# lunarlab-gatech/MorphSym-HGNN

Measured on AMD Instinct MI355X. Metric: graph-windows/sec fwd+bwd, A1-C2 GRF regression, higher is better.
Workload: dtype bf16; 1 GPU; A1-C2 GRF regression (3-D), h=128, L=3, T=150, 8192 windows/GPU, fwd+MSE+bwd, all parameter gradients; global_batch=8192, parallelism=dp1, rccl_ranks=0

## Files before the change

### morphsym_hgnn_amd/csrc/mshgnn.hip

```cpp
#include "mshgnn_slab.hpp"
extern "C" const char* mshgnn_last_error(void) { return g_err.c_str(); }
extern "C" const char* mshgnn_version(void) { return "mshgnn 0.5 (gfx950)"; }
extern "C" int mshgnn_abi_version(void) { return MSHGNN_ABI_VERSION; }
extern "C" size_t mshgnn_struct_size(int which) {
    switch (which) {
        case 0: return sizeof(mshgnn_desc);
        case 1: return sizeof(mshgnn_info);
        case 2: return sizeof(mshgnn_ws_layout);
        case 3: return sizeof(mshgnn_window_desc);
        case 4: return sizeof(mshgnn_kernel_stat);
        default: return 0;
    }
}


template <typename T> __device__ __forceinline__ void prep_one(const PrepArgs& a, int idx, bool with_bias) {
    constexpr int EPC = Prec<T>::EPC, NBV = Prec<T>::NBV;
    const int vec_per_pack = H * H / EPC;
    const int npk = a.pack_n < 0 ? a.n_packs : a.pack_n;
    const int total = npk * vec_per_pack;
    if (idx < total) {
        const int pack = a.pack0 + idx / vec_per_pack, r = idx % vec_per_pack;
        const int gid = pack * vec_per_pack + r;
        const int lane = r % 64, v = (r / 64) % NBV, wv = r / (64 * NBV);
        const PackDesc pd = a.packs[pack];
        T out[EPC];
        float g[8][EPC];
#pragma unroll
        for (int i = 0; i < 8; ++i)
#pragma unroll
            for (int x = 0; x < EPC; ++x) {
                int k, col;
                const int i16 = lane & 15;
                if constexpr (sizeof(T) == 4) { k = 32 * (lane >> 4) + 4 * (v & 7) + x; col = wv * 32 + 8 * (i16 >> 2) + 4 * (v >> 3) + (i16 & 3); }
                else { k = 32 * (lane >> 4) + 8 * (v & 3) + x; col = wv * 32 + 8 * (i16 >> 2) + 4 * (v >> 2) + (i16 & 3); }
                g[i][x] = 0.f;
                if (i < pd.n_src) {
                    if (pd.orient == 0) { if (k < pd.ncols) g[i][x] = a.params[pd.src[i] + (int64_t)col * pd.ld + pd.col0 + k]; }
                    else g[i][x] = a.params[pd.src[i] + (int64_t)k * pd.ld + col];
                }
            }
#pragma unroll
        for (int x = 0; x < EPC; ++x) {
            float sum = 0.f;
#pragma unroll
            for (int i = 0; i < 8; ++i) sum += g[i][x];
            out[x] = from_f32<T>(sum);
        }
        T* dst = reinterpret_cast<T*>(a.wpack) + (size_t)gid * EPC;
#pragma unroll
        for (int x = 0; x < EPC; ++x) dst[x] = out[x];
    } else if (with_bias) {
        const int b = idx - total;
        if (b < a.n_biases * H) {
            const BiasDesc bd = a.biases[b / H];
            float s = 0.f;
            for (int i = 0; i < bd.n_src; ++i) s += a.params[bd.src[i] + (b % H)];
            a.bias[b] = s;
        }
    }
}
template <typename T> __global__ void k_prep(PrepArgs a) { prep_one<T>(a, blockIdx.x * blockDim.x + threadIdx.x, true); }


__device__ __forceinline__ u32x4 splice8(u32x4 A, u32x4 B, int n0) {
    const unsigned __int128 a = ((unsigned __int128)(((unsigned long long)A[3] << 32) | A[2]) << 64) | (((unsigned long long)A[1] << 32) | A[0]);
    const unsigned __int128 b = ((unsigned __int128)(((unsigned long long)B[3] << 32) | B[2]) << 64) | (((unsigned long long)B[1] << 32) | B[0]);
    const int sh = 16 * n0;
    const unsigned __int128 r = (a & ((((unsigned __int128)1) << sh) - 1)) | (b << sh);
    return u32x4{(unsigned)r, (unsigned)(r >> 32), (unsigned)(r >> 64), (unsigned)(r >> 96)};
}
template <typename T, bool ALIGNED, bool SERIES = false, int SRC = 0, bool NORM = false> __global__ __launch_bounds__(256) void k_enc_fwd(EncArgs a, SeriesSrc ser, WideSrc wsrc) {
    using P = Prec<T>;
    static_assert(!NORM || SERIES, "standardisation is part of the series gather");
    static_assert(!SERIES || (sizeof(T) == 2 && ALIGNED), "the series gather is a bf16 path");
    static_assert(SRC == 0 || (sizeof(T) == 2 && ALIGNED && !SERIES), "wide source rows: bf16 plan, aligned destination rows");
    constexpr int MB = P::ENC_MB;
    constexpr int VPB = P::ROWS * P::CPR, NIT = VPB / 256 > 0 ? VPB / 256 : 1, BPP = 256 / VPB > 0 ? 256 / VPB : 1;
    extern __shared__ __attribute__((aligned(16))) char smem[];
    const int tid = threadIdx.x, lane = tid & 63, wv = __builtin_amdgcn_readfirstlane(tid >> 6);
    const int lab_blocks = SERIES ? (int)((ser.lab.B + 255) / 256) : 0;
    if constexpr (SERIES) {
        if ((int)blockIdx.x < lab_blocks) {
            const int64_t b = (int64_t)blockIdx.x * 256 + tid;
            if (b < ser.lab.B) window_labels_one(ser.lab, b);
            return;
        }
    }
    const int bid = (int)blockIdx.x - lab_blocks;
    if (bid >= a.wg_prefix[a.n_types]) {
        if constexpr (sizeof(T) == 2 && ALIGNED && !SERIES) prep_one<T>(a.prep, (bid - a.wg_prefix[a.n_types]) * 256 + tid, false);
        return;
    }
    int t = 0;
    while (t + 1 < a.n_types && bid >= a.wg_prefix[t + 1]) ++t;
    const int local = bid - a.wg_prefix[t];
    const int node = a.node_list[a.node_off[t] + (ENC_ORDER ? local % a.nodes[t] : local / a.tiles)], tile = ENC_ORDER ? local / a.nodes[t] : local % a.tiles;
    const bool skip = SERIES && ((a.skip_mask >> (a.tbase[t] + node)) & 1ull) != 0;
    const int w0 = tile * MB * P::ROWS;
    const T* x = reinterpret_cast<const T*>(a.x[t]);
    const int64_t pitch = a.pitch[t];
    const int F = a.width[t], nt = a.tbase[t + 1] - a.tbase[t], nkc = a.nkc[t], vb = a.vb[t];
    const uint8_t* sg = a.signs + a.sign_off[t] + (size_t)node * nkc * H;
    const T* wpack = reinterpret_cast<const T*>(a.wpack);
    const float* bias = a.bias + (size_t)max(a.bias_idx[t], 0) * H;

    typename P::Acc acc[MB];
#pragma unroll
    for (int m = 0; m < MB; ++m) acc_init_bias<T>(acc[m], bias, wv, lane);
    const int c = tid % P::CPR, r0 = (tid % VPB) / P::CPR, sub = tid / VPB;
    typename P::BFrag bf;
    typename P::AFrag af;
    const AOff<T> ao(lane);
    u32x4 v[MB / BPP][NIT];
    u32x4 rawv[(SERIES || SRC) ? MB / BPP : 1][NIT];
    u32x2 wv8[SRC ? MB / BPP : 1][SRC ? SRC : 1];
    const bool unit_ok = SRC == 8 || (F & 1) == 0;
    const int64_t spitch = SRC ? wsrc.pitch[t] : 0;
    int srow[SERIES ? MB / BPP : 1];
    u32x4 vn[NORM ? MB / BPP : 1][2];
    RunStats rsa[NORM ? MB / BPP : 1], rsb[NORM ? MB / BPP : 1];
    int n_n0 = 8; bool n_has_a = false, n_has_b = false;
    __shared__ unsigned long long rp_s[SERIES ? 16 : 1];
    int rfirst = 0, rend = 0;
    if constexpr (SERIES) {
#pragma unroll
        for (int mi = 0; mi < MB / BPP; ++mi) srow[mi] = (int)ser.starts[min(w0 + (mi * BPP + sub) * P::ROWS + r0, a.B - 1)];
        rfirst = ser.rows[2 * (ser.row0[t] + node)]; rend = ser.rows[2 * (ser.row0[t] + node) + 1];
        if (tid < 16) rp_s[tid] = rfirst + tid < rend ? ser.run_ptr[rfirst + tid] : 0ull;
        __syncthreads();
    }
    auto fetch = [&](int kc) {
        const int k0 = kc * H + c * P::EPC;
        const int nvalid = min(P::EPC, F - k0);
        if constexpr (SERIES) {
            const int j = k0 / ser.T, off = k0 - j * ser.T, n0 = min(P::EPC, ser.T - off);
            const bool second = nvalid > n0;
            auto run_ptr_of = [&](int jj) -> unsigned long long { return jj < 16 ? rp_s[jj] : (rfirst + jj < rend ? ser.run_ptr[rfirst + jj] : 0ull); };
            const unsigned long long pa = nvalid > 0 ? run_ptr_of(j) : 0ull, pb = second ? run_ptr_of(j + 1) : 0ull;
            if constexpr (NORM) {
                n_n0 = n0; n_has_a = pa != 0ull; n_has_b = pb != 0ull;
                const u32x4 ones32 = u32x4{0x3f800000u, 0x3f800000u, 0x3f800000u, 0x3f800000u};
#pragma unroll
                for (int mi = 0; mi < MB / BPP; ++mi) {
                    u32x4 a0 = nvalid > 0 ? ones32 : u32x4{0, 0, 0, 0}, a1 = a0;
                    const double* sp2 = ser.stats + ((size_t)min(w0 + (mi * BPP + sub) * P::ROWS + r0, a.B - 1) * ser.n_runs + rfirst + j) * 2;
                    rsa[mi] = RunStats{0.0, 1.0}; rsb[mi] = RunStats{0.0, 1.0};
                    if (pa) {
                        const float* sp = reinterpret_cast<const float*>(pa) + srow[mi] + off;
                        a0 = *reinterpret_cast<const u32x4*>(sp); a1 = *reinterpret_cast<const u32x4*>(sp + 4);
                        const f64x2 sv = *reinterpret_cast<const f64x2*>(sp2);
                        rsa[mi] = RunStats{sv[0], sv[1]};
                    }
                    if (second) {
                        u32x4 b0 = ones32, b1 = ones32;
                        if (pb) {
                            const float* sp = reinterpret_cast<const float*>(pb) + srow[mi];
                            b0 = *reinterpret_cast<const u32x4*>(sp); b1 = *reinterpret_cast<const u32x4*>(sp + 4);
                            const f64x2 sv = *reinterpret_cast<const f64x2*>(sp2 + 2);
                            rsb[mi] = RunStats{sv[0], sv[1]};
                        }
                        splice8f(a0, a1, b0, b1, n0);
                    }
                    vn[mi][0] = a0; vn[mi][1] = a1;
                }
                return;
            }
            const u32x4 ones = u32x4{0x3f803f80u, 0x3f803f80u, 0x3f803f80u, 0x3f803f80u};
#pragma unroll
            for (int mi = 0; mi < MB / BPP; ++mi) {
                u32x4 va = nvalid > 0 ? ones : u32x4{0, 0, 0, 0};
                if (pa) va = *reinterpret_cast<const u32x4*>(reinterpret_cast<const T*>(pa) + srow[mi] + off);
                if (second) {
                    u32x4 vb2 = ones;
                    if (pb) vb2 = *reinterpret_cast<const u32x4*>(reinterpret_cast<const T*>(pb) + srow[mi]);
                    va = splice8(va, vb2, n0);
                }
                v[mi][0] = va;
            }
            return;
        }
        if constexpr (SRC > 0) {
#pragma unroll
            for (int mi = 0; mi < MB / BPP; ++mi) {
                const int w = w0 + (mi * BPP + sub) * P::ROWS + r0;
                const char* row = reinterpret_cast<const char*>(wsrc.p[t]) + ((size_t)min(w, a.B - 1) * nt + node) * spitch * SRC;
                wide_fetch<SRC>(wv8[mi], row, k0, F, unit_ok, w < a.B);
            }
            return;
        }
#pragma unroll
        for (int mi = 0; mi < MB / BPP; ++mi)
#pragma unroll
            for (int it = 0; it < NIT; ++it) {
                const int m = mi * BPP + sub, row = r0 + it * (256 / P::CPR), w = w0 + m * P::ROWS + row;
                if constexpr (ALIGNED) {
                    const T* src = x + ((size_t)min(w, a.B - 1) * nt + node) * pitch + (nvalid > 0 ? k0 : kc * H);
                    v[mi][it] = ld16<ENC_NT>(src);
                } else {
                    v[mi][it] = u32x4{0, 0, 0, 0};
                    if (w < a.B) v[mi][it] = load_chunk<T>(x + ((size_t)w * nt + node) * pitch + k0, nvalid, vb);
                }
            }
    };
    fetch(0);
    for (int kc = 0; kc < nkc; ++kc) {
        const u32x4 sx = sign_xor<T>(sg + kc * H + c * P::EPC);
        const int nv = F - (kc * H + c * P::EPC);
        __syncthreads();
#pragma unroll
        for (int mi = 0; mi < MB / BPP; ++mi)
#pragma unroll
            for (int it = 0; it < NIT; ++it) {
                u32x4 raw;
                if constexpr (SRC > 0) {
// ... 951 lines not shown
            qstride[i] = H; qvalid[i] = 8; qvb[i] = 16;
        } else {
            const int t = im[3] - BUF_IN;
            qbase[i] = reinterpret_cast<const T*>(a.x[t]) + (size_t)im[5] * a.pitch[t] + im[6] + c * 8;
            qstride[i] = (int64_t)a.nodes[t] * a.pitch[t]; qvalid[i] = im[7] - c * 8; qvb[i] = a.vb[t];
            qsign[i] = sign_xor<T>(a.signs + im[8] + c * 8);
        }
    }
    f32x16 acc[2][2];
#pragma unroll
    for (int i = 0; i < 2; ++i)
#pragma unroll
        for (int j = 0; j < 2; ++j)
#pragma unroll
            for (int q = 0; q < 16; ++q) acc[i][j][q] = 0.f;
    float bsum[8];
#pragma unroll
    for (int e = 0; e < 8; ++e) bsum[e] = 0.f;

    struct Stage { u32x4 pv[4], qv[4]; unsigned mw[4]; };
    auto fetch = [&](Stage& st, int s) {
        const int w0 = (ch0 + (nit == 2 ? s >> 1 : s)) * GWB_KW;
        const int it = (nit == 2) ? (s & 1) : 0;
        const T* pb = it ? pbase[I1] : pbase[0];
        const T* qb = it ? qbase[I1] : qbase[0];
        const uint8_t* mb = it ? mbase[I1] : mbase[0];
        const int64_t qs = it ? qstride[I1] : qstride[0];
        const int qn = it ? qvalid[I1] : qvalid[0], vb = it ? qvb[I1] : qvb[0];
#pragma unroll
        for (int p = 0; p < 4; ++p) {
            const int w = w0 + r0 + 16 * p;
            st.pv[p] = u32x4{0, 0, 0, 0}; st.qv[p] = u32x4{0, 0, 0, 0}; st.mw[p] = 0xffffffffu;
            if (w < a.B && !ABL(a.dbg & 1)) {
                st.pv[p] = *reinterpret_cast<const u32x4*>(pb + (size_t)w * H);
                if (mb) st.mw[p] = mb[((size_t)(w >> 4) << 6) + (w & 15)];
                if (a.aligned) { if (qn > 0) st.qv[p] = *reinterpret_cast<const u32x4*>(qb + (size_t)w * qs); }
                else st.qv[p] = load_chunk<T>(qb + (size_t)w * qs, qn, vb);
            }
        }
    };
    const bool p_masked = mbase[0] != nullptr, q_raw_input = qvb[0] != 16 || qvalid[0] != 8 || (qsign[0][0] | qsign[0][1] | qsign[0][2] | qsign[0][3] | qsign[nit == 2 ? I1 : 0][0] | qsign[nit == 2 ? I1 : 0][1] | qsign[nit == 2 ? I1 : 0][2] | qsign[nit == 2 ? I1 : 0][3]) != 0 || qvalid[nit == 2 ? I1 : 0] != 8;
    auto stage_to_lds = [&](const Stage& st, const u32x4 sx, const int qn, __bf16* Ps, __bf16* Qs) {
        if ABL(a.dbg & 2) { asm volatile("" :: "v"(st.pv[0][0]), "v"(st.qv[3][3])); return; }
#pragma unroll
        for (int p = 0; p < 4; ++p) {
            const int row = r0 + 16 * p;
            u32x4 pm = st.pv[p];
            if (p_masked) pm &= mlut[st.mw[p] & 0xffu];
            *reinterpret_cast<u32x4*>(&Ps[gwb_elem(row, c * 8)]) = pm;
            u32x4 qm = st.qv[p];
            if (q_raw_input) qm = chunk_keep_first<T>(qm, qn) ^ sx;
            *reinterpret_cast<u32x4*>(&Qs[gwb_elem(row, c * 8)]) = qm;
            if (bias_flag) {
#pragma unroll
                for (int e = 0; e < 4; ++e) {
                    bsum[2 * e] += __builtin_bit_cast(float, pm[e] << 16);
                    bsum[2 * e + 1] += __builtin_bit_cast(float, pm[e] & 0xffff0000u);
                }
            }
        }
    };
    auto mfmas = [&](const __bf16* Ps, const __bf16* Qs) {
        if ABL(a.dbg & 4) return;
#pragma unroll
        for (int ks = 0; ks < GWB_KW / 16; ++ks) {
            bf16x8 af[2], bq[2];
#pragma unroll
            for (int i = 0; i < 2; ++i) {
                af[i] = tr_frag(Ps, ks * 16, wr * 64 + i * 32, lane);
                bq[i] = tr_frag(Qs, ks * 16, wc * 64 + i * 32, lane);
            }
#pragma unroll
            for (int i = 0; i < 2; ++i)
#pragma unroll
                for (int j = 0; j < 2; ++j) acc[i][j] = __builtin_amdgcn_mfma_f32_32x32x16_bf16(af[i], bq[j], acc[i][j], 0, 0, 0);
        }
    };
    const u32x4 sx1 = nit == 2 ? qsign[I1] : qsign[0];
    const int qn1 = nit == 2 ? qvalid[I1] : qvalid[0];
#if GW_DEEP
    Stage sa, sb;
    if (nsteps > 0) fetch(sa, 0);
    if (nsteps > 1) fetch(sb, 1);
    if (nsteps > 0) stage_to_lds(sa, qsign[0], qvalid[0], Pbuf[0], Qbuf[0]);
    if (nsteps > 2) fetch(sa, 2);
    __syncthreads();
    for (int s = 0; s < nsteps; s += 2) {
        if (s + 1 < nsteps) stage_to_lds(sb, sx1, qn1, Pbuf[1], Qbuf[1]);
        if (s + 3 < nsteps) fetch(sb, s + 3);
        mfmas(Pbuf[0], Qbuf[0]);
        __syncthreads();
        if (s + 1 < nsteps) {
            if (s + 2 < nsteps) stage_to_lds(sa, qsign[0], qvalid[0], Pbuf[0], Qbuf[0]);
            if (s + 4 < nsteps) fetch(sa, s + 4);
            mfmas(Pbuf[1], Qbuf[1]);
            __syncthreads();
        }
    }
#else
    Stage sa;
    if (nsteps > 0) fetch(sa, 0);
#ifndef MSHGNN_GW_STAMPS
#define MSHGNN_GW_STAMPS 0
#endif
#if MSHGNN_GW_STAMPS
    long long tph[5] = {0, 0, 0, 0, 0}, tprev = a.stamps ? clock64() : 0;
    auto lap = [&](int k) { if (a.stamps) { const long long t = clock64(); tph[k] += t - tprev; tprev = t; } };
#else
    auto lap = [](int) {};
#endif
    for (int s = 0; s < nsteps; ++s) {
        __syncthreads();
        lap(0);
        stage_to_lds(sa, (nit == 2 && (s & 1)) ? qsign[I1] : qsign[0], (nit == 2 && (s & 1)) ? qvalid[I1] : qvalid[0], Pbuf[0], Qbuf[0]);
        lap(1);
        __syncthreads();
        lap(2);
        if (s + 1 < nsteps) fetch(sa, s + 1);
        lap(3);
        mfmas(Pbuf[0], Qbuf[0]);
        lap(4);
    }
#if MSHGNN_GW_STAMPS
    if (a.stamps && tid == 0) { for (int k = 0; k < 5; ++k) a.stamps[(size_t)blockIdx.x * 8 + k] = tph[k]; a.stamps[(size_t)blockIdx.x * 8 + 5] = nsteps; }
#endif
    (void)sx1; (void)qn1;
#endif
    float* slab = a.slabs + (size_t)(part * a.n_lanes + ln) * SLAB_FLOATS;
    if (!ABL(a.dbg & 8))
#pragma unroll
    for (int i = 0; i < 2; ++i)
#pragma unroll
        for (int j = 0; j < 2; ++j)
#pragma unroll
            for (int q = 0; q < 16; ++q) {
                const int o = wr * 64 + i * 32 + (q & 3) + ((q >> 2) << 3) + ((lane >> 5) << 2), k = wc * 64 + j * 32 + (lane & 31);
                slab[o * H + k] = acc[i][j][q];
            }
    if (bias_flag) {
        float* red = reinterpret_cast<float*>(Pbuf[0]);
        __syncthreads();
#pragma unroll
        for (int e = 0; e < 8; ++e) red[r0 * H + c * 8 + e] = bsum[e];
        __syncthreads();
        if (tid < H) {
            float s2 = 0.f;
#pragma unroll
            for (int r = 0; r < 16; ++r) s2 += red[r * H + tid];
            slab[H * H + tid] = s2;
        }
    }
}

template <bool ALIGNED, bool SERIES = false> __global__ __launch_bounds__(256, GW_WPS) void k_gradw_bf16_lean(GradwArgs a) {
    static_assert(!SERIES || ALIGNED, "the series gather replaces the aligned raw loads");
    using T = __bf16;
    __shared__ __attribute__((aligned(16))) __bf16 Ps[GWB_KW * GWB_PITCH];
    __shared__ __attribute__((aligned(16))) __bf16 Qs[GWB_KW * GWB_PITCH];
    __shared__ __attribute__((aligned(16))) u32x4 mlut[256];
    __shared__ __attribute__((aligned(16))) u32x4 qkeep_t[16];
    __shared__ __attribute__((aligned(16))) u32x4 qsign_t[GW_IPL][16];
    __shared__ unsigned long long sbase[GW_IPL][4];
    __shared__ unsigned long long sser[SERIES ? GW_IPL : 1][16][2];
    const int tid = threadIdx.x, lane = tid & 63, wv = __builtin_amdgcn_readfirstlane(tid >> 6);
    mlut[tid] = chunk_mask_bits<__bf16>(u32x4{0xffffffffu, 0xffffffffu, 0xffffffffu, 0xffffffffu}, (unsigned)tid);
    const int wr = wv >> 1, wc = wv & 1;
    const int ln = a.lane_order[blockIdx.x % a.n_pad], part = blockIdx.x / a.n_pad;
    if (ln < 0) return;
    const int* lh = a.lanes + ln * LANE_INTS;
    const int it0 = lh[0], nit = lh[1] - lh[0], bias_flag = lh[3];
    const int* im0 = a.items + it0 * ITEM_INTS;
    const int nchunks = (a.B + GWB_KW - 1) / GWB_KW;
    const int ch0 = (int)((int64_t)part * nchunks / a.n_parts), ch1 = (int)((int64_t)(part + 1) * nchunks / a.n_parts);
    const int nsteps = ch1 - ch0, total = nsteps * nit;
    const int c = tid & 15, r4 = (tid >> 4) * 4;

    const bool p_masked = im0[9] >= 0, q_raw = im0[4] < 0;
    const int ntile = (a.B + 15) >> 4;
    const unsigned voffP = (unsigned)(r4 * H + c * 8) * (unsigned)sizeof(T);
    const unsigned voffM = (unsigned)(((c >> 2) * ntile + (r4 >> 4)) * 64 + (c & 3) * 16 + (r4 & 15));
    const int qt = q_raw ? im0[3] - BUF_IN : 0;
    const unsigned qsb = q_raw ? (unsigned)(a.nodes[qt] * a.pitch[qt]) * (unsigned)sizeof(T) : (unsigned)(H * sizeof(T));
    const int qn = q_raw ? im0[7] - c * 8 : 8, qvb = q_raw ? a.vb[qt] : 16;
    const unsigned voffQ0 = (unsigned)r4 * qsb + (unsigned)c * 16u;
    unsigned ldsw[4];
#pragma unroll
    for (int p = 0; p < 4; ++p) ldsw[p] = (unsigned)gwb_elem(r4 + p, c * 8);
    if (tid < 16) qkeep_t[tid] = chunk_keep_first<T>(u32x4{0xffffffffu, 0xffffffffu, 0xffffffffu, 0xffffffffu}, qn);
    if (tid < nit) {
        const int* im = a.items + (it0 + tid) * ITEM_INTS;
        sbase[tid][0] = (unsigned long long)(a.ws + a.buf_off[im[0]] + (act_idx(0, im[2], a.B) + (size_t)ch0 * GWB_KW * H) * sizeof(T));
        sbase[tid][1] = p_masked ? (unsigned long long)(a.ws + a.buf_off[im[9]] + relu_byte(im[2], a.B, 0, 0) + (size_t)ch0 * (GWB_KW / 16) * 64) : 0ull;
        sbase[tid][2] = q_raw ? (unsigned long long)(reinterpret_cast<const char*>(a.x[qt]) + ((size_t)im[5] * a.pitch[qt] + im[6]) * sizeof(T) + (size_t)ch0 * GWB_KW * qsb)
                              : (unsigned long long)(a.ws + a.buf_off[im[3]] + (act_idx(0, im[5], a.B) + (size_t)ch0 * GWB_KW * H) * sizeof(T));
    }
    if (q_raw && tid < nit * 16) {
        const int* im = a.items + (it0 + (tid >> 4)) * ITEM_INTS;
        qsign_t[tid >> 4][c] = sign_xor<T>(a.signs + im[8] + c * 8);
        if constexpr (SERIES) {
            const int k0 = im[6] + c * 8, j = k0 / a.ser.T, off = k0 - j * a.ser.T, n0 = min(8, a.ser.T - off);
            const int rfirst = a.ser.rows[2 * (a.ser.row0[qt] + im[5])];
            const unsigned long long pa = qn > 0 ? a.ser.run_ptr[rfirst + j] : 0ull, pb = min(qn, 8) > n0 ? a.ser.run_ptr[rfirst + j + 1] : 0ull;
            sser[tid >> 4][c][0] = pa ? pa + (unsigned long long)off * sizeof(T) : 0ull;
            sser[tid >> 4][c][1] = pb;
        }
    }
    int s_n0 = 8; bool s_two = false;
    if constexpr (SERIES) { if (q_raw) { const int k0 = im0[6] + c * 8, off = k0 % a.ser.T; s_n0 = min(8, a.ser.T - off); s_two = min(qn, 8) > s_n0; } }
    __syncthreads();
    const char* pS = a.ws; const char* mS = a.ws; const char* qS = a.ws;
    auto ubase = [&](int k, int j, size_t off) -> const char* {
        const unsigned long long v = sbase[k][j] + off;
        return reinterpret_cast<const char*>(((unsigned long long)(unsigned)__builtin_amdgcn_readfirstlane((int)(v >> 32)) << 32) |
                                             (unsigned)__builtin_amdgcn_readfirstlane((int)(unsigned)v));
    };
    f32x16 acc[2][2];
#pragma unroll
    for (int i = 0; i < 2; ++i)
#pragma unroll
        for (int j = 0; j < 2; ++j)
#pragma unroll
            for (int q = 0; q < 16; ++q) acc[i][j][q] = 0.f;
    float bsum[8];
#pragma unroll
    for (int e = 0; e < 8; ++e) bsum[e] = 0.f;

    u32x4 pv[4], qv[4]; unsigned mw = 0xffffffffu;
    int nk = 0, nc = 0;
    int wst[SERIES ? 4 : 1];
    auto load_starts = [&](int chunk) {
        if constexpr (SERIES) {
            if (q_raw) {
#pragma unroll
                for (int p = 0; p < 4; ++p) wst[p] = (int)a.ser.starts[min((ch0 + chunk) * GWB_KW + r4 + p, a.B - 1)];
            }
        }
    };
    auto load_q = [&](int p) -> u32x4 {
        if constexpr (SERIES) {
            if (q_raw) {
                const u32x4 ones = u32x4{0x3f803f80u, 0x3f803f80u, 0x3f803f80u, 0x3f803f80u};
                const unsigned long long pa = sser[nk][c][0];
                u32x4 va = ones;
                if (pa) va = *reinterpret_cast<const u32x4*>(reinterpret_cast<const T*>(pa) + wst[p]);
                if (s_two) {
                    const unsigned long long pb = sser[nk][c][1];
                    u32x4 vb2 = ones;
                    if (pb) vb2 = *reinterpret_cast<const u32x4*>(reinterpret_cast<const T*>(pb) + wst[p]);
                    va = splice8(va, vb2, s_n0);
                }
                return va;
            }
        }
        if constexpr (ALIGNED) return *reinterpret_cast<const u32x4*>(qS + voffQ0 + p * qsb);
        else return q_raw ? load_chunk<T>(reinterpret_cast<const T*>(qS + voffQ0 + p * qsb), qn, qvb) : *reinterpret_cast<const u32x4*>(qS + voffQ0 + p * qsb);
    };
    auto fetch = [&]() {
        pS = ubase(nk, 0, (size_t)nc * GWB_KW * H * sizeof(T));
        if (p_masked) mS = ubase(nk, 1, (size_t)nc * (GWB_KW / 16) * 64);
        qS = ubase(nk, 2, (size_t)nc * GWB_KW * qsb);
        const int w0 = (ch0 + nc) * GWB_KW;
        if (w0 + GWB_KW <= a.B) {
#pragma unroll
            for (int p = 0; p < 4; ++p) {
                pv[p] = *reinterpret_cast<const u32x4*>(pS + voffP + p * (int)(H * sizeof(T)));
                qv[p] = u32x4{0, 0, 0, 0};
                if (qn > 0) qv[p] = load_q(p);
            }
            if (p_masked) mw = *reinterpret_cast<const unsigned*>(mS + voffM);
        } else {
#pragma unroll
            for (int p = 0; p < 4; ++p) {
                pv[p] = u32x4{0, 0, 0, 0}; qv[p] = u32x4{0, 0, 0, 0};
                if (w0 + r4 + p < a.B) {
                    pv[p] = *reinterpret_cast<const u32x4*>(pS + voffP + p * (int)(H * sizeof(T)));
                    if (qn > 0) qv[p] = load_q(p);
                }
            }
            mw = 0xffffffffu;
            if (p_masked && w0 + r4 < a.B) mw = *reinterpret_cast<const unsigned*>(mS + voffM);
        }
        if (++nk == nit) { nk = 0; ++nc; if (nc < nsteps) load_starts(nc); }
    };
    int sk = 0;
    auto stage_to_lds = [&]() {
        u32x4 mk[4], qkeep, sx;
        if (q_raw) { qkeep = qkeep_t[c]; sx = qsign_t[sk][c]; }
        if (++sk == nit) sk = 0;
        if (p_masked) {
#pragma unroll
            for (int p = 0; p < 4; ++p) mk[p] = mlut[(mw >> (8 * p)) & 0xffu];
        }
#pragma unroll
        for (int p = 0; p < 4; ++p) {
            u32x4 pm = pv[p];
            if (p_masked) pm &= mk[p];
            *reinterpret_cast<u32x4*>(&Ps[ldsw[p]]) = pm;
            u32x4 qm = qv[p];
            if (q_raw) qm = (qm & qkeep) ^ sx;
            *reinterpret_cast<u32x4*>(&Qs[ldsw[p]]) = qm;
            if (bias_flag) {
#pragma unroll
                for (int e = 0; e < 4; ++e) {
                    bsum[2 * e] += __builtin_bit_cast(float, pm[e] << 16);
                    bsum[2 * e + 1] += __builtin_bit_cast(float, pm[e] & 0xffff0000u);
                }
            }
        }
    };
    if (total > 0) { load_starts(0); fetch(); }
    for (int s = 0; s < total; ++s) {
        __syncthreads();
        stage_to_lds();
        __syncthreads();
        if (s + 1 < total) fetch();
#pragma unroll
        for (int ks = 0; ks < GWB_KW / 16; ++ks) {
            bf16x8 af[2], bq[2];
#pragma unroll
            for (int i = 0; i < 2; ++i) {
                af[i] = tr_frag(Ps, ks * 16, wr * 64 + i * 32, lane);
                bq[i] = tr_frag(Qs, ks * 16, wc * 64 + i * 32, lane);
            }
#pragma unroll
            for (int i = 0; i < 2; ++i)
#pragma unroll
                for (int j = 0; j < 2; ++j) acc[i][j] = __builtin_amdgcn_mfma_f32_32x32x16_bf16(af[i], bq[j], acc[i][j], 0, 0, 0);
        }
    }
    float* slab = a.slabs + (size_t)(part * a.n_lanes + ln) * SLAB_FLOATS;
#pragma unroll
    for (int i = 0; i < 2; ++i)
#pragma unroll
        for (int j = 0; j < 2; ++j)
#pragma unroll
            for (int q = 0; q < 16; ++q) {
                const int o = wr * 64 + i * 32 + (q & 3) + ((q >> 2) << 3) + ((lane >> 5) << 2), k = wc * 64 + j * 32 + (lane & 31);
                slab[o * H + k] = acc[i][j][q];
            }
    if (bias_flag) {
        float* red = reinterpret_cast<float*>(Ps);
        __syncthreads();
#pragma unroll
        for (int e = 0; e < 8; ++e) red[(r4 >> 2) * H + c * 8 + e] = bsum[e];
        __syncthreads();
        if (tid < H) {
            float s2 = 0.f;
#pragma unroll
            for (int r = 0; r < 16; ++r) s2 += red[r * H + tid];
            slab[H * H + tid] = s2;
        }
    }
}


#ifndef FIN_LB
#define FIN_LB 4
#endif
__global__ __launch_bounds__(256) void k_finalize(FinArgs a) {
    const int* f = a.fin + blockIdx.x * FIN_INTS;
    const int64_t dst = (int64_t)(unsigned)f[0] | ((int64_t)f[1] << 32);
    const int rows = f[2], cols = f[3], ld = f[4], tg = f[5], kind = f[6];
    const int* more = f[7] ? a.fin0 + f[7] : nullptr;
    const int RPB = (rows + gridDim.y - 1) / gridDim.y;
    const int r0 = blockIdx.y * RPB, r1 = min(rows, r0 + RPB);
    const int n = (r1 - r0) * cols;
    if (a.loss && blockIdx.x == 0 && blockIdx.y == 0 && threadIdx.x < 64) {
        float l = 0.f;
        for (int b = threadIdx.x; b < a.n_dec; b += 64) l += a.dec_slabs[(size_t)b * DEC_SLAB_FLOATS + 8 * H + 8];
#pragma unroll
        for (int m = 32; m >= 1; m >>= 1) l += __shfl_xor(l, m, 64);
        if (threadIdx.x == 0) *a.loss = l * a.inv_n + (a.accumulate ? *a.loss : 0.f);
    }
    if (!a.grad) return;
    const bool is_mat = (kind == FIN_MATRIX || kind == FIN_DEC_W);
    if (kind == FIN_DEC_W || kind == FIN_DEC_B) {
        const int lane = threadIdx.x & 63, wave = blockIdx.y * 4 + (threadIdx.x >> 6), nwaves = gridDim.y * 4;
        for (int e = wave; e < rows * cols; e += nwaves) {
            const int r = e / cols, cidx = e % cols;
            const int src = is_mat ? r * H + cidx : 8 * H + cidx;
            float sum = 0.f;
            for (int b0 = 0; b0 < a.n_dec; b0 += 512) {
                float v[8];
#pragma unroll
                for (int u = 0; u < 8; ++u) { const int b = b0 + lane + 64 * u; v[u] = b < a.n_dec ? a.dec_slabs[(size_t)b * DEC_SLAB_FLOATS + src] : 0.f; }
                sum += ((v[0] + v[1]) + (v[2] + v[3])) + ((v[4] + v[5]) + (v[6] + v[7]));
            }
#pragma unroll
            for (int m = 32; m >= 1; m >>= 1) sum += __shfl_xor(sum, m, 64);
            if (lane == 0) { float* gp = a.grad + dst + (int64_t)r * ld + cidx; *gp = a.accumulate ? *gp + sum : sum; }
        }
        return;
    }
    if (n <= 0) return;
    for (int i = threadIdx.x; i < n; i += 256) {
        const int r = r0 + i / cols, cidx = i % cols;
        float s = 0.f;
        if (kind == FIN_MATRIX || kind == FIN_BIAS) {
            const int src = is_mat ? r * H + cidx : H * H + cidx;
            const int l0 = a.targets[tg * TGT_INTS], nl = a.targets[tg * TGT_INTS + 1] - l0;
            const float* sp = a.slabs + (size_t)l0 * SLAB_FLOATS + src;
            const size_t pstride = (size_t)a.n_lanes * SLAB_FLOATS;
            for (int j0 = 0; j0 < nl; j0 += FIN_LB)
                for (int p0 = 0; p0 < a.n_parts; p0 += 4) {
                    float v[FIN_LB][4];
#pragma unroll
                    for (int jj = 0; jj < FIN_LB; ++jj)
#pragma unroll
                        for (int pp = 0; pp < 4; ++pp)
                            v[jj][pp] = (j0 + jj < nl && p0 + pp < a.n_parts) ? sp[(size_t)(j0 + jj) * SLAB_FLOATS + (size_t)(p0 + pp) * pstride] : 0.f;
#pragma unroll
                    for (int jj = 0; jj < FIN_LB; ++jj) s += (v[jj][0] + v[jj][1]) + (v[jj][2] + v[jj][3]);
                }
        }
        if (a.accumulate) s += a.grad[dst + (int64_t)r * ld + cidx];
        a.grad[dst + (int64_t)r * ld + cidx] = s;
        if (more) {
            const int nm = more[0];
            for (int k = 0; k < nm; ++k) a.grad[((int64_t)(unsigned)more[1 + 2 * k] | ((int64_t)more[2 + 2 * k] << 32)) + (int64_t)r * ld + cidx] = s;
        }
    }
}

static StackKernel slab_fwd_kernel(const HostPlan& hp) {
    if (hp.sl_hb <= SL_HB) return hp.n_mlp <= 2 ? k_slab_fwd<__bf16, 2, SL_HB> : k_slab_fwd<__bf16, 4, SL_HB>;
    return hp.n_mlp <= 2 ? k_slab_fwd<__bf16, 2, SL_HB_MAX> : k_slab_fwd<__bf16, 4, SL_HB_MAX>;
}
using SpecSelector = StackKernel (*)(const HostPlan& hp, int kind, int tr, int nt, int full, const char** name);
static StackKernel spec_kernel(const HostPlan& hp, int kind, int tr, int nt, int full, const char** name = nullptr) {
    const char* nm = nullptr;
    if (hp.jit_prog) {
        StackKernel kk = reinterpret_cast<SpecSelector>(hp.jit_prog)(hp, kind, tr, nt, full, &nm);
        if (nm) { if (name) *name = nm; return kk; }
    }
#define SPEC_SHARD_TRY(k) { StackKernel kk = spec_shard##k(hp, kind, tr, nt, full, &nm); if (nm) { if (name) *name = nm; return kk; } }
    SPEC_SHARD_LIST(SPEC_SHARD_TRY)
#undef SPEC_SHARD_TRY
    return nullptr;
}
inline bool whole_tiles(int64_t B) { return B > 0 && B % TILE_ROWS == 0; }
static StackKernel slab_step_spec_kernel(const HostPlan& hp, int nt, const char** name = nullptr, bool full = true) { return spec_kernel(hp, 0, 1, nt, full, name); }
static StackKernel slab_fwd_spec_kernel(const HostPlan& hp, int training, int nt, bool full = true) { return spec_kernel(hp, 1, training, nt, full); }
static StackKernel slab_bwd_spec_kernel(const HostPlan& hp, int nt, bool full = true) { return spec_kernel(hp, 2, 1, nt, full); }
static StackKernel slab_step_kernel(const HostPlan& hp, int64_t B = -1, int nt = 0, bool use_spec = false) {
    if (use_spec && B > 0) if (StackKernel k = slab_step_spec_kernel(hp, nt, nullptr, whole_tiles(B))) return k;
    if (hp.sl_hb <= SL_HB) return hp.n_mlp <= 2 ? k_slab_step<__bf16, 2, SL_HB> : k_slab_step<__bf16, 4, SL_HB>;
    return hp.n_mlp <= 2 ? k_slab_step<__bf16, 2, SL_HB_MAX> : k_slab_step<__bf16, 4, SL_HB_MAX>;
}
static StackKernel slab_bwd_kernel(const HostPlan& hp) {
    if (hp.sl_hb <= SL_HB) return hp.n_mlp <= 2 ? k_slab_bwd<__bf16, 2, SL_HB> : k_slab_bwd<__bf16, 4, SL_HB>;
    return hp.n_mlp <= 2 ? k_slab_bwd<__bf16, 2, SL_HB_MAX> : k_slab_bwd<__bf16, 4, SL_HB_MAX>;
}


static int set_spec_attrs(mshgnn_plan* p, int flds) {
    const HostPlan& hp = p->hp;
    int rc;
    const char* nm = nullptr;
    for (int nt = 0; nt < 2; ++nt)
        if (StackKernel k = slab_step_spec_kernel(hp, nt, &nm)) if ((rc = set_lds_attr(k, flds))) return rc;
    if (!nm) { p->use_spec = false; return MSHGNN_OK; }
    p->spec_name_buf = strncmp(nm, "spec::", 6) == 0 ? nm + 6 : nm;
    p->spec_name = p->spec_name_buf.c_str();
    for (int v = 0; v < 3; ++v)
        if (StackKernel k = slab_fwd_spec_kernel(hp, v > 0, v - 1)) if ((rc = set_lds_attr(k, flds))) return rc;
    for (int nt = 0; nt < 2; ++nt)
        if (StackKernel k = slab_bwd_spec_kernel(hp, nt)) if ((rc = set_lds_attr(k, flds))) return rc;
    if (StackKernel k = slab_step_spec_kernel(hp, 0, nullptr, false)) if ((rc = set_lds_attr(k, flds))) return rc;
    if (StackKernel k = slab_fwd_spec_kernel(hp, 0, 0, false)) if ((rc = set_lds_attr(k, flds))) return rc;
    return MSHGNN_OK;
}

extern "C" int mshgnn_plan_attach_program(mshgnn_plan* p, void* selector) {
    if (!p || !selector) return set_err(MSHGNN_EINVAL, "plan or selector is null");
    if (!p->gen && p->hp.d.dtype == MSHGNN_BF16X3) return x3_attach_program(p, selector);
    if (p->gen || p->hp.d.dtype != MSHGNN_BF16 || !p->use_fused || !p->use_slab) return set_err(MSHGNN_EINVAL, "attached programs exist for LDS-resident bf16 / split-bf16 plans (bf16: on the slab kernels) only");
    void* const prev = p->hp.jit_prog;
    p->hp.jit_prog = selector;
    const char* nm = nullptr;
    if (!reinterpret_cast<SpecSelector>(selector)(p->hp, 0, 1, 0, 1, &nm) || !nm) {
        p->hp.jit_prog = prev;
        return set_err(MSHGNN_EINVAL, "the program's tables are not this plan's");
    }
    p->use_spec = true;
    const int rc = set_spec_attrs(p, (p->hp.fs_blk + FS_EXTRA_BLK) * Prec<__bf16>::BLK);
    if (rc || !p->use_spec) { p->hp.jit_prog = prev; p->use_spec = false; return rc ? rc : set_err(MSHGNN_EINVAL, "no kernel of the attached program could be used"); }
    return MSHGNN_OK;
}

extern "C" int mshgnn_plan_create(const mshgnn_desc* desc, mshgnn_plan** out) {
    if (!out) return set_err(MSHGNN_EINVAL, "plan_out is null");
    *out = nullptr;
    mshgnn_plan* p = new (std::nothrow) mshgnn_plan();
    if (!p) return set_err(MSHGNN_ENOMEM, "out of host memory");
    if (!desc) { delete p; return set_err(MSHGNN_EINVAL, "null descriptor"); }
    p->n_types = desc->n_types;
    if (const char* e = getenv("MSHGNN_STEP_CHUNK")) p->step_chunk = std::max<int64_t>(0, atoll(e));
    if (const char* e = getenv("MSHGNN_STASH_NT")) p->stash_nt_force = atoi(e);
    const char* eng_env = getenv("MSHGNN_ENGINE");
    bool want_gen = eng_env && std::string(eng_env) == "generic";
    std::string why;
    if (!want_gen && !compile_plan(desc, p->hp)) {
        why = p->hp.err;
        const bool unsup = why.find("supports") != std::string::npos || why.find("not supported") != std::string::npos || why.find("too many") != std::string::npos;
        if (!unsup) { delete p; return set_err(MSHGNN_EINVAL, why); }
        want_gen = true;
    }
    if (want_gen) {
        int ndev0 = 0;
        if (hipGetDeviceCount(&ndev0) != hipSuccess || ndev0 == 0) { delete p; return set_err(MSHGNN_EHIP, "no HIP device: the MS-HGNN engine has no CPU fallback"); }
        const int rc = gen_create(p, desc);
        if (rc) {
            const std::string m = g_err; gen_destroy(p); delete p;
            return set_err(rc, why.empty() ? m : why + "; generic-width engine: " + m);
        }
#ifdef MSHGNN_ABLATE
        { const char* e = getenv("MSHGNN_DBG"); p->dbg = e ? atoi(e) : 0; }
#endif
        if (!p->hp.d.n_types) {
            p->hp.d = *desc;
        }
        *out = p;
        return MSHGNN_OK;
    }
    int ndev = 0;
    if (hipGetDeviceCount(&ndev) != hipSuccess || ndev == 0) {
        delete p; return set_err(MSHGNN_EHIP, "no HIP device: the MS-HGNN engine has no CPU fallback");
    }
#ifdef MSHGNN_ABLATE
    { const char* e = getenv("MSHGNN_DBG"); p->dbg = e ? atoi(e) : 0; e = getenv("MSHGNN_DBG_GW"); p->dbg_gw = e ? atoi(e) : 0; }
#endif
    HostPlan& hp = p->hp;
    auto up = [&](void** dptr, const void* src, size_t bytes) -> int {
        HIPCHK(hipMalloc(dptr, std::max<size_t>(bytes, 16)));
        if (bytes) HIPCHK(hipMemcpy(*dptr, src, bytes, hipMemcpyHostToDevice));
        return MSHGNN_OK;
    };
    int rc;
    if ((rc = up((void**)&p->d_tables, hp.tables.data(), hp.tables.size() * 4)) != 0 ||
        (rc = up((void**)&p->d_signs, hp.signs.data(), hp.signs.size())) != 0 ||
        (rc = up((void**)&p->d_out_mask, hp.out_mask_f.data(), hp.out_mask_f.size() * 4)) != 0 ||
        (rc = up((void**)&p->d_packs, hp.packs.data(), hp.packs.size() * sizeof(PackDesc))) != 0 ||
        (rc = up((void**)&p->d_biases, hp.biases.data(), hp.biases.size() * sizeof(BiasDesc))) != 0) {
        mshgnn_plan_destroy(p); return rc;
    }
    const int lds = hp.n_blk * hp.blk_bytes;
    if (hp.d.dtype == MSHGNN_BF16X3) {
        p->use_fused = true;
        { const char* et = getenv("MSHGNN_STEP_KERNEL"); p->use_step = !(et && atoi(et) == 0); }
        if ((rc = x3_set_attrs(p))) { mshgnn_plan_destroy(p); return rc; }
    } else if (hp.d.dtype == MSHGNN_F32) {
        if ((rc = set_lds_attr(k_layer_fwd<float>, lds)) || (rc = set_lds_attr(k_layer_bwd<float>, lds)) ||
            (rc = set_lds_attr(k_enc_fwd<float, true>, Prec<float>::ENC_MB * Prec<float>::BLK)) || (rc = set_lds_attr(k_enc_fwd<float, false>, Prec<float>::ENC_MB * Prec<float>::BLK))) { mshgnn_plan_destroy(p); return rc; }
    } else {
        if ((rc = set_lds_attr(k_layer_fwd<__bf16>, lds)) || (rc = set_lds_attr(k_layer_bwd<__bf16>, lds)) ||
            (rc = set_lds_attr(k_enc_fwd<__bf16, true>, Prec<__bf16>::ENC_MB * Prec<__bf16>::BLK)) || (rc = set_lds_attr(k_enc_fwd<__bf16, true, true>, Prec<__bf16>::ENC_MB * Prec<__bf16>::BLK)) || (rc = set_lds_attr(k_enc_fwd<__bf16, true, false, 8>, Prec<__bf16>::ENC_MB * Prec<__bf16>::BLK)) || (rc = set_lds_attr(k_enc_fwd<__bf16, true, false, 4>, Prec<__bf16>::ENC_MB * Prec<__bf16>::BLK)) || (rc = set_lds_attr(k_enc_fwd<__bf16, false>, Prec<__bf16>::ENC_MB * Prec<__bf16>::BLK))) { mshgnn_plan_destroy(p); return rc; }
        const char* e = getenv("MSHGNN_FUSED");
        p->use_fused = hp.fused && !(e && atoi(e) == 0);
        if (p->use_fused) {
            const int flds = (hp.fs_blk + FS_EXTRA_BLK) * Prec<__bf16>::BLK;
            if ((rc = set_lds_attr(k_stack_fwd<__bf16>, flds)) || (rc = set_lds_attr(k_stack_bwd<__bf16>, flds)) || (rc = set_lds_attr(k_stack_step<__bf16>, flds))) { mshgnn_plan_destroy(p); return rc; }
            const char* es = getenv("MSHGNN_SLAB");
            p->use_slab = hp.slab && !(es && atoi(es) == 0);
            p->slab_force = es && atoi(es) == 2;
            { int dev = 0, cus = 256; if (hipGetDevice(&dev) == hipSuccess) (void)hipDeviceGetAttribute(&cus, hipDeviceAttributeMultiprocessorCount, dev); p->n_cu = cus > 0 ? cus : 256; }
            if (p->use_slab && ((rc = set_lds_attr(slab_fwd_kernel(hp), flds)) || (rc = set_lds_attr(slab_bwd_kernel(hp), flds)) ||
                                (rc = set_lds_attr(slab_step_kernel(hp), flds)))) { mshgnn_plan_destroy(p); return rc; }
            { const char* esp = getenv("MSHGNN_SPEC"); p->use_spec = p->use_slab && !(esp && atoi(esp) == 0); }
            if (p->use_spec && (rc = set_spec_attrs(p, flds))) { mshgnn_plan_destroy(p); return rc; }
            { const char* et = getenv("MSHGNN_STEP_KERNEL"); p->use_step = !(et && atoi(et) == 0); }

            { const char* eg = TUNE_ENV("MSHGNN_STAGGER"); p->stagger = eg ? atoi(eg) : 0; }
        }
    }
    *out = p;
    return MSHGNN_OK;
}

extern "C" void mshgnn_plan_destroy(mshgnn_plan* p) {
    if (!p) return;
    gen_destroy(p);
    if (p->d_tables) (void)hipFree(p->d_tables);
    if (p->d_signs) (void)hipFree(p->d_signs);
    if (p->d_out_mask) (void)hipFree(p->d_out_mask);
    if (p->d_packs) (void)hipFree(p->d_packs);
    if (p->d_biases) (void)hipFree(p->d_biases);
    if (p->d_ig_nodes) (void)hipFree(p->d_ig_nodes);
    for (ProfRec& r : p->recs) { (void)hipEventDestroy(r.a); (void)hipEventDestroy(r.b); }
    for (hipEvent_t e : p->free_events) (void)hipEventDestroy(e);
    delete p;
}

extern "C" int mshgnn_profile_enable(mshgnn_plan* p, int on) {
    if (!p) return set_err(MSHGNN_EINVAL, "null plan");
    p->prof = on != 0;
    return MSHGNN_OK;
}

extern "C" int mshgnn_profile_read(mshgnn_plan* p, mshgnn_kernel_stat* stats, int32_t* n_inout) {
    if (!p || !stats || !n_inout) return set_err(MSHGNN_EINVAL, "null argument");
    std::vector<mshgnn_kernel_stat> ks = p->gen ? *gen_kstats(p) : p->hp.kstats;
    for (const ProfRec& r : p->recs) {
        HIPCHK(hipEventSynchronize(r.b));
        float ms = 0.f;
        HIPCHK(hipEventElapsedTime(&ms, r.a, r.b));
        if (r.slot >= 0 && r.slot < (int)ks.size()) { ks[r.slot].total_ms += ms; ks[r.slot].launches += 1; }
        p->free_events.push_back(r.a); p->free_events.push_back(r.b);
    }
    p->recs.clear();
    const int n = std::min<int>(*n_inout, (int)ks.size());
    for (int i = 0; i < n; ++i) stats[i] = ks[i];
    *n_inout = n;
    return MSHGNN_OK;
}

extern "C" const char* mshgnn_plan_specialised(const mshgnn_plan* p) { return p && !p->gen && p->use_spec ? p->spec_name : ""; }
extern "C" int mshgnn_plan_info(const mshgnn_plan* p, mshgnn_info* info) {
    if (!p || !info) return set_err(MSHGNN_EINVAL, "null argument");
    *info = p->gen ? *gen_info(p) : p->hp.info;
    return MSHGNN_OK;
}

extern "C" int mshgnn_plan_compile_host(const mshgnn_desc* desc, mshgnn_info* info, int32_t* n_tables_out) {
    HostPlan hp;
    const char* eng_env = getenv("MSHGNN_ENGINE");
    if ((eng_env && std::string(eng_env) == "generic") || !compile_plan(desc, hp)) {
        const std::string why = hp.err;
        if (gen_host_compile(desc, info, n_tables_out) == MSHGNN_OK) return MSHGNN_OK;
        return set_err(MSHGNN_EINVAL, why.empty() ? g_err : why + "; generic-width engine: " + g_err);
    }
    if (info) *info = hp.info;
    if (n_tables_out) *n_tables_out = (int32_t)hp.tables.size();
    return MSHGNN_OK;
}

extern "C" int mshgnn_workspace_layout(const mshgnn_plan* p, int64_t batch, int training, mshgnn_ws_layout* out) {
    if (!p || !out || batch < 1) return set_err(MSHGNN_EINVAL, "bad argument to mshgnn_workspace_layout");
    if (p->gen) gen_layout(p, batch, training, out); else layout_workspace(p->hp, batch, training, out);
    return MSHGNN_OK;
}

int launch_prep(const PrepArgs& a, bool split, hipStream_t st) {
    if (split) return x3_launch_prep(a, st);
    const int64_t total = (int64_t)a.n_packs * (H * H / Prec<__bf16>::EPC) + (int64_t)a.n_biases * H;
    if (prep_use_tiled(a.n_packs)) hipLaunchKernelGGL((k_prep_tiled<__bf16, false>), dim3(prep_tiled_grid(a.n_packs, a.n_biases)), dim3(256), 0, st, a);
    else hipLaunchKernelGGL(k_prep<__bf16>, dim3((unsigned)((total + 255) / 256)), dim3(256), 0, st, a);
    return MSHGNN_OK;
}

int run_finalize(const mshgnn_plan* p, const StepCall& c, const mshgnn_ws_layout& lay, int gw_parts) {
    const HostPlan& hp = p->hp;
    const mshgnn_desc& d = hp.d;
    char* ws = c.ws; float* gparams = c.grad_params; hipStream_t st = c.stream;
    const int B = (int)c.batch, gw_phase = c.gw_phase;
    float* loss = c.loss != LossKind::NONE ? c.loss_out : nullptr;
    FinArgs a{p->d_tables + hp.fin_off, p->d_tables + hp.fin_off, p->d_tables + hp.tgt_off, reinterpret_cast<const float*>(ws + lay.slabs),
              reinterpret_cast<const float*>(ws + lay.dec_slabs), gparams, hp.n_lanes, gw_parts, loss,
              1.0f / (float)(c.total_windows() * d.type_nodes[d.out_type] * (c.loss == LossKind::CE ? 1 : d.out_channels)),
              c.dec_done ? (int)((B + TILE_ROWS - 1) / TILE_ROWS) : NWG_DEC, c.accumulates()};
    int f0 = 0, nf = hp.n_fin;
    if (gw_phase == 0) nf = hp.n_fin_ph0;
    if (gw_phase == 1) { f0 = hp.n_fin_ph0; nf = hp.n_fin - hp.n_fin_ph0; a.loss = nullptr; }
    a.fin += (size_t)f0 * FIN_INTS;
    if (!gparams) {
        if (loss) hipLaunchKernelGGL(k_finalize, dim3(1, 1), dim3(256), 0, st, a);
        HIPCHK(hipGetLastError());
        return MSHGNN_OK;
    }
    ProfScope ps(p, hp.ks_fin, st);
    if (nf > 0) hipLaunchKernelGGL(k_finalize, dim3(nf, 64), dim3(256), 0, st, a);
    HIPCHK(hipGetLastError());
    return MSHGNN_OK;
}

template <typename T>
static int forward_impl(const mshgnn_plan* p, StepCall& c) {
    const HostPlan& hp = p->hp;
    const mshgnn_desc& d = hp.d;
    const int training = c.training;
    mshgnn_ws_layout lay; layout_workspace(hp, c.batch, training, &lay);
    const int B = (int)c.batch;
    const void* const* x = c.x; const int64_t* x_pitch = c.x_pitch;
    const float* params = c.params; char* ws = c.ws; hipStream_t st = c.stream;
    const SeriesSrc* series = c.series; const WideSrc* wide = c.wide;
    const float* y_fused = c.y_fused(); const int32_t* labels_fused = c.labels_fused();
    PrepArgs pa{params, ws + lay.wpack, reinterpret_cast<float*>(ws + lay.bias), p->d_packs, p->d_biases, (int)hp.packs.size(), (int)hp.biases.size()};
    int enc_pack0 = (int)hp.packs.size();
    for (int t = 0; t < hp.NT; ++t) if (hp.pack_enc_base[t] >= 0) enc_pack0 = std::min(enc_pack0, hp.pack_enc_base[t]);
    static const bool embed_off = TUNE_ENV("MSHGNN_PREP_EMBED") && atoi(TUNE_ENV("MSHGNN_PREP_EMBED")) == 0;
    const bool embed = sizeof(T) == 2 && !series && !prep_use_tiled(pa.n_packs) && enc_pack0 > 0 && !embed_off;
    {
        PrepArgs a = pa;
        if (embed) { a.pack0 = enc_pack0; a.pack_n = pa.n_packs - enc_pack0; }
        const int64_t total = (int64_t)(embed ? a.pack_n : a.n_packs) * (H * H / Prec<T>::EPC) + (int64_t)hp.biases.size() * H;
        ProfScope ps(p, hp.ks_prep, st);
        if (prep_use_tiled(a.n_packs)) hipLaunchKernelGGL((k_prep_tiled<T, false>), dim3(prep_tiled_grid(a.n_packs, a.n_biases)), dim3(256), 0, st, a);
        else hipLaunchKernelGGL(k_prep<T>, dim3((unsigned)((total + 255) / 256)), dim3(256), 0, st, a);
    }
    {
        EncArgs a{};
        a.n_types = hp.NT; a.B = B; a.NN = hp.NN; a.tiles = (B + Prec<T>::ENC_MB * Prec<T>::ROWS - 1) / (Prec<T>::ENC_MB * Prec<T>::ROWS);
        a.wg_prefix[0] = 0;
        for (int t = 0; t < hp.NT; ++t) {
            a.x[t] = x ? x[t] : nullptr; a.pitch[t] = x_pitch ? x_pitch[t] : d.type_width[t];
            if (a.pitch[t] < d.type_width[t]) return set_err(MSHGNN_EINVAL, "x_pitch smaller than the feature width");
            a.vb[t] = vec_bytes(a.x[t], a.pitch[t], (int)sizeof(T));
            if (t == 0) a.aligned = 1;
            if (a.vb[t] != 16 || a.pitch[t] % Prec<T>::EPC) a.aligned = 0;
            a.width[t] = d.type_width[t]; a.tbase[t] = hp.type_base[t]; a.nkc[t] = hp.enc_nkc[t];
            a.pack0[t] = hp.pack_enc_base[t]; a.bias_idx[t] = hp.bias_enc[t]; a.sign_off[t] = hp.sign_off[t];
            a.node_off[t] = t == 0 ? 0 : a.node_off[t - 1] + a.nodes[t - 1];
            a.nodes[t] = 0;
            const bool all_rows = series != nullptr && x != nullptr;
            for (int i = 0; i < d.type_nodes[t]; ++i) {
                const bool need = hp.need_n[0][hp.type_base[t] + i];
                if (need || all_rows) a.node_list[a.node_off[t] + a.nodes[t]++] = (unsigned char)i;
                if (!need) a.skip_mask |= 1ull << (hp.type_base[t] + i);
            }
            a.wg_prefix[t + 1] = a.wg_prefix[t] + a.nodes[t] * a.tiles;
        }
        a.tbase[hp.NT] = hp.NN;
        a.wpack = ws + lay.wpack; a.bias = reinterpret_cast<const float*>(ws + lay.bias); a.signs = p->d_signs; a.x0 = ws + lay.x[0];
        a.mask0 = (training && lay.dd[0]) ? reinterpret_cast<uint8_t*>(ws + lay.dd[0]) : nullptr;
        unsigned enc_grid = (unsigned)a.wg_prefix[hp.NT];
        if (embed) {
            PrepArgs lp = pa; lp.pack0 = 0; lp.pack_n = enc_pack0;
            if (a.aligned) { a.prep = lp; a.prep_vecs = enc_pack0 * (H * H / Prec<T>::EPC); enc_grid += (unsigned)((a.prep_vecs + 255) / 256); }
            else {
                ProfScope ps(p, hp.ks_prep, st);
                hipLaunchKernelGGL(k_prep<T>, dim3((unsigned)(((int64_t)enc_pack0 * (H * H / Prec<T>::EPC) + 255) / 256)), dim3(256), 0, st, lp);
            }
        }
        ProfScope ps(p, hp.ks_enc, st);
        if constexpr (sizeof(T) == 2) {
            if (series) {
                if (x && !a.aligned) return set_err(MSHGNN_EINVAL, "the fused window assembly needs 16-byte aligned window rows (pitch a multiple of 8)");
                enc_grid += (unsigned)((series->lab.B + 255) / 256);
                if (series->stats) hipLaunchKernelGGL((k_enc_fwd<T, true, true, 0, true>), dim3(enc_grid), dim3(256), Prec<T>::ENC_MB * Prec<T>::BLK, st, a, *series, WideSrc{});
                else hipLaunchKernelGGL((k_enc_fwd<T, true, true>), dim3(enc_grid), dim3(256), Prec<T>::ENC_MB * Prec<T>::BLK, st, a, *series, WideSrc{});
            } else if (wide) {
                if (x && !a.aligned) return set_err(MSHGNN_EINVAL, "wide source rows: the plan-dtype rows need 16-byte alignment and a pitch that is a multiple of 8");
                if (wide->bytes == 8) hipLaunchKernelGGL((k_enc_fwd<T, true, false, 8>), dim3(enc_grid), dim3(256), Prec<T>::ENC_MB * Prec<T>::BLK, st, a, SeriesSrc{}, *wide);
                else hipLaunchKernelGGL((k_enc_fwd<T, true, false, 4>), dim3(enc_grid), dim3(256), Prec<T>::ENC_MB * Prec<T>::BLK, st, a, SeriesSrc{}, *wide);
            } else if (a.aligned) hipLaunchKernelGGL((k_enc_fwd<T, true>), dim3(enc_grid), dim3(256), Prec<T>::ENC_MB * Prec<T>::BLK, st, a, SeriesSrc{}, WideSrc{});
            else hipLaunchKernelGGL((k_enc_fwd<T, false>), dim3(enc_grid), dim3(256), Prec<T>::ENC_MB * Prec<T>::BLK, st, a, SeriesSrc{}, WideSrc{});
        } else {
            if (wide) return set_err(MSHGNN_EUNSUPPORTED, "wide source rows: not on the fp32 plan (cast the inputs)");
            if (a.aligned) hipLaunchKernelGGL((k_enc_fwd<T, true>), dim3(enc_grid), dim3(256), Prec<T>::ENC_MB * Prec<T>::BLK, st, a, SeriesSrc{}, WideSrc{});
            else hipLaunchKernelGGL((k_enc_fwd<T, false>), dim3(enc_grid), dim3(256), Prec<T>::ENC_MB * Prec<T>::BLK, st, a, SeriesSrc{}, WideSrc{});
        }
    }
    const int tiles = (B + Prec<T>::ROWS - 1) / Prec<T>::ROWS;
    if constexpr (sizeof(T) == 2) {
        if (p->use_fused) {
            StackArgs a{};
            a.tile_in = ws + lay.x[0]; a.ws = ws;
            for (int l = 0; l <= hp.L; ++l) a.x_off[l] = lay.x[l];
            for (int l = 0; l < hp.L; ++l) { a.mask_off[l] = lay.mask[l]; a.hb_off[l] = lay.hb[l]; a.t1_off[l] = lay.t1[l]; a.prog_off[l] = hp.fs_fwd_off[l]; }
            a.wpack = ws + lay.wpack; a.bias = reinterpret_cast<const float*>(ws + lay.bias); a.tables = p->d_tables;
            a.B = B; a.NN = hp.NN; a.L = hp.L; a.training = training;
            a.dbg = p->dbg;
            a.params = params; a.out_mask = p->d_out_mask; a.out = c.out; a.off_dec_w = d.off_dec_w; a.off_dec_b = d.off_dec_b;
            a.node0 = hp.type_base[d.out_type]; a.n_out = d.type_nodes[d.out_type]; a.dout = d.out_channels;
            if (y_fused) {
                a.y = y_fused; a.dec_slabs = reinterpret_cast<float*>(ws + lay.dec_slabs); a.dx_off[hp.L] = lay.dx[hp.L];
                a.inv_n = 1.0f / (float)(c.total_windows() * a.n_out * a.dout);
            } else if (labels_fused) {
                a.labels = labels_fused; a.dec_slabs = reinterpret_cast<float*>(ws + lay.dec_slabs); a.dx_off[hp.L] = lay.dx[hp.L];
                a.inv_n = 1.0f / (float)(c.total_windows() * a.n_out);
            }
            c.dec_done = y_fused || labels_fused;
            a.stamps = stamp_ptr("MSHGNN_STAMPS");
            a.stagger = p->slab_for(tiles) && tiles > p->n_cu ? p->stagger : 0;
            a.stash_nt = training ? stash_nt_for(p->stash_nt_force, B, stash_rows_of(hp), H * (int)sizeof(T)) : 0;
            const bool want_step = p->use_step && c.dec_done;
            bool step_slab = p->slab_for(tiles);
            const bool spec_small = !step_slab && want_step && p->use_slab && p->use_spec && slab_step_spec_kernel(hp, a.stash_nt, nullptr, whole_tiles(B)) != nullptr;
            bool red_front_ok = false, red_back_ok = false; size_t red_back = 0;
            auto red_fits = [&](bool slab) {
                const size_t red_need = (size_t)((slab ? SL_THREADS : LAYER_THREADS) / 64) * DEC_SLAB_FLOATS * sizeof(float);
                const size_t lds_launch = (size_t)((slab ? hp.sl_blk : hp.fs_blk) + FS_EXTRA_BLK) * Prec<T>::BLK;
                red_back = (size_t)(a.node0 + a.n_out) * Prec<T>::BLK;
                red_front_ok = (size_t)a.node0 * Prec<T>::BLK >= red_need; red_back_ok = red_back + red_need <= lds_launch;
                return red_front_ok || red_back_ok; };
            if (spec_small && red_fits(true)) step_slab = true;
            const bool step = want_step && red_fits(step_slab);
            if (step && !red_front_ok) a.red_off = (int)red_back;
            const StackKernel fwd_spec = (!step && p->use_slab && p->use_spec) ? slab_fwd_spec_kernel(hp, training, a.stash_nt, whole_tiles(B)) : nullptr;
            if (fwd_spec) step_slab = true;
            ProfScope ps(p, step ? hp.ks_stack_step : hp.ks_stack_fwd, st);
            if (step_slab) {
                for (int l = 0; l < hp.L; ++l) a.prog_off[l] = hp.sl_fwd_off[l];
                if (step) {
                    for (int l = 0; l <= hp.L; ++l) a.dx_off[l] = lay.dx[l];
                    for (int l = 0; l < hp.L; ++l) { a.dh_off[l] = lay.dh[l]; a.du_off[l] = lay.du[l]; a.prog_off_b[l] = hp.sl_bwd_off[l]; }
                    a.mask0_off = lay.dd[0];
                    hipLaunchKernelGGL(slab_step_kernel(hp, B, a.stash_nt, p->use_spec), dim3(tiles), dim3(SL_THREADS), (hp.sl_blk + FS_EXTRA_BLK) * Prec<T>::BLK, st, a);
                    c.stack_done = true;
                } else
                hipLaunchKernelGGL(fwd_spec ? fwd_spec : slab_fwd_kernel(hp), dim3(tiles), dim3(SL_THREADS), (hp.sl_blk + FS_EXTRA_BLK) * Prec<T>::BLK, st, a);
            } else if (step) {
                for (int l = 0; l <= hp.L; ++l) a.dx_off[l] = lay.dx[l];
                for (int l = 0; l < hp.L; ++l) { a.dh_off[l] = lay.dh[l]; a.du_off[l] = lay.du[l]; a.prog_off_b[l] = hp.fs_bwd_off[l]; }
                a.mask0_off = lay.dd[0];
                hipLaunchKernelGGL(k_stack_step<T>, dim3(tiles), dim3(LAYER_THREADS), (hp.fs_blk + FS_EXTRA_BLK) * Prec<T>::BLK, st, a);
                c.stack_done = true;
            } else
            hipLaunchKernelGGL(k_stack_fwd<T>, dim3(tiles), dim3(LAYER_THREADS), (hp.fs_blk + FS_EXTRA_BLK) * Prec<T>::BLK, st, a);
            HIPCHK(hipGetLastError());
            return MSHGNN_OK;
        }
    }
    for (int l = 0; l < hp.L; ++l) {
        LayerArgs a{};
        a.x_in = ws + lay.x[l]; a.x_out = ws + lay.x[l + 1]; a.maskbits = reinterpret_cast<unsigned*>(ws + lay.mask[l]);
        a.hb = ws + lay.hb[l]; a.t1 = ws + lay.t1[l]; a.wpack = ws + lay.wpack; a.bias = reinterpret_cast<const float*>(ws + lay.bias);
        a.prog = p->d_tables + hp.fwd_prog_off[l]; a.B = B; a.NN = hp.NN; a.n_mlp = std::max(1, hp.n_mlp);
        a.dbg = p->dbg;
        ProfScope ps(p, hp.ks_layer_fwd0 + l, st);
        hipLaunchKernelGGL(k_layer_fwd<T>, dim3(tiles), dim3(LAYER_THREADS), hp.n_blk * Prec<T>::BLK, st, a);
    }
    {
        DecArgs a{};
        a.xl = ws + lay.x[hp.L]; a.params = params; a.out_mask = p->d_out_mask; a.out = c.out; a.off_w = d.off_dec_w; a.off_b = d.off_dec_b;
        a.B = B; a.NN = hp.NN; a.node0 = hp.type_base[d.out_type]; a.n_out = d.type_nodes[d.out_type]; a.dout = d.out_channels;
        const int64_t rows = (int64_t)B * a.n_out;
        ProfScope ps(p, hp.ks_dec_fwd, st);
        hipLaunchKernelGGL(k_dec_fwd<T>, dim3((unsigned)((rows + 15) / 16)), dim3(256), 0, st, a);
    }
    HIPCHK(hipGetLastError());
    return MSHGNN_OK;
}

template <typename T>
static int backward_impl(const mshgnn_plan* p, const StepCall& c) {
    const HostPlan& hp = p->hp;
    const mshgnn_desc& d = hp.d;
    mshgnn_ws_layout lay; layout_workspace(hp, c.batch, 1, &lay);
    const int B = (int)c.batch;
    const void* const* x = c.x; const int64_t* x_pitch = c.x_pitch;
    char* ws = c.ws; hipStream_t st = c.stream;
    const int gw_phase = c.gw_phase;
    const bool stack_done = c.stack_done;
    const SeriesSrc* series = c.gradw_from_series ? c.series : nullptr;
    if (!c.dec_done && gw_phase != 1) {
        DecArgs a{};
        a.xl = ws + lay.x[hp.L]; a.dxl = ws + lay.dx[hp.L]; a.params = c.params; a.out_mask = p->d_out_mask; a.gout = c.grad_out;
        a.slabs = reinterpret_cast<float*>(ws + lay.dec_slabs); a.off_w = d.off_dec_w; a.off_b = d.off_dec_b;
        a.B = B; a.NN = hp.NN; a.node0 = hp.type_base[d.out_type]; a.n_out = d.type_nodes[d.out_type]; a.dout = d.out_channels; a.slab0 = 0;
        if (c.loss == LossKind::MSE) {
            a.y = c.y; a.out = c.out; a.loss = c.loss_out; a.inv_n = 1.0f / (float)(c.total_windows() * a.n_out * a.dout);
        }
        if (c.loss == LossKind::CE) {
            a.labels = c.labels; a.out = c.out; a.loss = c.loss_out; a.inv_n = 1.0f / (float)(c.total_windows() * a.n_out);
        }
        ProfScope ps(p, hp.ks_dec_bwd, st);
        hipLaunchKernelGGL(k_dec_bwd<T>, dim3(NWG_DEC), dim3(256), 0, st, a);
    }
    const int tiles = (B + Prec<T>::ROWS - 1) / Prec<T>::ROWS;
    bool fused_done = gw_phase == 1 || stack_done;
    if constexpr (sizeof(T) == 2) {
        if (p->use_fused && gw_phase != 1 && !stack_done) {
            StackArgs a{};
            a.tile_in = ws + lay.dx[hp.L]; a.ws = ws;
            for (int l = 0; l <= hp.L; ++l) { a.x_off[l] = lay.x[l]; a.dx_off[l] = lay.dx[l]; }
            for (int l = 0; l < hp.L; ++l) { a.mask_off[l] = lay.mask[l]; a.t1_off[l] = lay.t1[l]; a.dh_off[l] = lay.dh[l]; a.du_off[l] = lay.du[l]; a.prog_off[l] = hp.fs_bwd_off[l]; }
            a.wpack = ws + lay.wpack; a.bias = reinterpret_cast<const float*>(ws + lay.bias); a.tables = p->d_tables;
            a.B = B; a.NN = hp.NN; a.L = hp.L; a.training = 1;
            a.node0 = hp.type_base[d.out_type]; a.n_out = d.type_nodes[d.out_type];
            a.mask0_off = lay.dd[0];
            a.dbg = p->dbg;
            a.stamps = stamp_ptr("MSHGNN_STAMPS_BWD");
            a.stagger = p->slab_for(tiles) && tiles > p->n_cu ? p->stagger : 0;
            a.stash_nt = stash_nt_for(p->stash_nt_force, B, stash_rows_of(hp), H * (int)sizeof(T));
            ProfScope ps(p, hp.ks_stack_bwd, st);
            const StackKernel bwd_spec = (p->use_slab && p->use_spec) ? slab_bwd_spec_kernel(hp, a.stash_nt, whole_tiles(B)) : nullptr;
            if (bwd_spec || p->slab_for(tiles)) {
                for (int l = 0; l < hp.L; ++l) a.prog_off[l] = hp.sl_bwd_off[l];
                hipLaunchKernelGGL(bwd_spec ? bwd_spec : slab_bwd_kernel(hp), dim3(tiles), dim3(SL_THREADS), (hp.sl_blk + FS_EXTRA_BLK) * Prec<T>::BLK, st, a);
            } else
            hipLaunchKernelGGL(k_stack_bwd<T>, dim3(tiles), dim3(LAYER_THREADS), (hp.fs_blk + FS_EXTRA_BLK) * Prec<T>::BLK, st, a);
            fused_done = true;
        }
    }
    for (int l = hp.L - 1; l >= 0 && !fused_done; --l) {
        LayerArgs a{};
        a.x_in = ws + lay.dx[l + 1]; a.x_out = ws + lay.dx[l]; a.maskbits = reinterpret_cast<unsigned*>(ws + lay.mask[l]);
        a.hb = ws + lay.hb[l]; a.t1 = ws + lay.t1[l]; a.dh = ws + lay.dh[l]; a.du = ws + lay.du[l]; a.x_act = ws + lay.x[0];
        a.wpack = ws + lay.wpack; a.bias = reinterpret_cast<const float*>(ws + lay.bias);
        a.prog = p->d_tables + hp.bwd_prog_off[l]; a.B = B; a.NN = hp.NN; a.n_mlp = std::max(1, hp.n_mlp);
        a.dbg = p->dbg;
        ProfScope ps(p, hp.ks_layer_bwd0 + (hp.L - 1 - l), st);
        hipLaunchKernelGGL(k_layer_bwd<T>, dim3(tiles), dim3(LAYER_THREADS), hp.n_blk * Prec<T>::BLK, st, a);
    }
    const int gw_parts = gw_parts_for(hp.n_parts, hp.n_lanes, hp.gw_ipl, B, sizeof(T) == 4 ? GW_KW : GWB_KW, p->n_cu);
    if (c.grad_params) {
        GradwArgs a{};
        a.ws = ws;
        for (int l = 0; l <= hp.L; ++l) { a.buf_off[BUF_X + l] = lay.x[l]; a.buf_off[BUF_DX + l] = lay.dx[l]; }
        for (int l = 0; l < hp.L; ++l) a.buf_off[BUF_MASK + l] = lay.mask[l];
        for (int l = 0; l < hp.L; ++l) { a.buf_off[BUF_DH + l] = lay.dh[l]; a.buf_off[BUF_HB + l] = lay.hb[l]; a.buf_off[BUF_T1 + l] = lay.t1[l]; a.buf_off[BUF_DU + l] = lay.du[l]; }
        for (int t = 0; t < hp.NT; ++t) {
            a.x[t] = x ? x[t] : nullptr; a.pitch[t] = x_pitch ? x_pitch[t] : d.type_width[t]; a.nodes[t] = d.type_nodes[t];
            a.vb[t] = vec_bytes(a.x[t], a.pitch[t], (int)sizeof(T));
            if (t == 0) a.aligned = 1;
            if (a.vb[t] != 16 || a.pitch[t] % Prec<T>::EPC) a.aligned = 0;
        }
        if (series) a.ser = *series;
        a.items = p->d_tables + hp.item_off; a.lanes = p->d_tables + hp.lane_off; a.lane_order = p->d_tables + hp.lane_order_off; a.n_pad = hp.n_lanes_pad;
        if (gw_phase >= 0) { a.lane_order = p->d_tables + hp.order_ph_off[gw_phase]; a.n_pad = hp.npad_ph[gw_phase]; }
        a.signs = p->d_signs; a.slabs = reinterpret_cast<float*>(ws + lay.slabs); a.B = B; a.n_lanes = hp.n_lanes; a.n_parts = gw_parts;
        a.dbg = p->dbg_gw;
        a.stamps = stamp_ptr("MSHGNN_STAMPS_GW");
        ProfScope ps(p, hp.ks_gradw, st);
        auto launch_gradw = [&](const GradwArgs& ga, hipStream_t s_) {
            [[maybe_unused]] static const bool gw_general = TUNE_ENV("MSHGNN_GRADW") && std::string(TUNE_ENV("MSHGNN_GRADW")) == "general";
            if (ga.n_pad <= 0) return;
            if constexpr (sizeof(T) == 4) hipLaunchKernelGGL(k_gradw_f32, dim3(ga.n_pad * gw_parts), dim3(256), 0, s_, ga);
#ifdef MSHGNN_TUNING
            else if (gw_general && hp.gw_ipl == 1) hipLaunchKernelGGL(k_gradw_bf16<1>, dim3(ga.n_pad * gw_parts), dim3(256), 0, s_, ga);
            else if (gw_general && hp.gw_ipl == 2) hipLaunchKernelGGL(k_gradw_bf16<2>, dim3(ga.n_pad * gw_parts), dim3(256), 0, s_, ga);
#endif
            else if (series) hipLaunchKernelGGL((k_gradw_bf16_lean<true, true>), dim3(ga.n_pad * gw_parts), dim3(256), 0, s_, ga);
            else if (ga.aligned) hipLaunchKernelGGL(k_gradw_bf16_lean<true>, dim3(ga.n_pad * gw_parts), dim3(256), 0, s_, ga);
            else hipLaunchKernelGGL(k_gradw_bf16_lean<false>, dim3(ga.n_pad * gw_parts), dim3(256), 0, s_, ga);
        };
        launch_gradw(a, st);
    }
    return run_finalize(p, c, lay, gw_parts);
}

static int run_forward(const mshgnn_plan* p, StepCall& c) {
    if (c.wide && c.series) return set_err(MSHGNN_EINVAL, "a call takes its encoder rows from wide sources or from a series, not from both");
    if (p->gen) return gen_forward(p, c);
    if (p->hp.d.dtype == MSHGNN_BF16X3) return x3_forward(p, c);
    if (p->hp.d.dtype == MSHGNN_F32) return forward_impl<float>(p, c);
    return forward_impl<__bf16>(p, c);
}

static int run_backward(const mshgnn_plan* p, const StepCall& c) {
    if (p->gen) return gen_backward(p, c);
    if (p->hp.d.dtype == MSHGNN_BF16X3) return x3_backward(p, c);
    if (p->hp.d.dtype == MSHGNN_F32) return backward_impl<float>(p, c);
    return backward_impl<__bf16>(p, c);
}

static int64_t step_chunk_windows(const mshgnn_plan* p, const StepCall& c) {
    const int64_t limit = p->step_chunk;
    if (limit <= 0 || c.batch < 2 * limit || p->gen || c.wide || c.series) return 0;
    const int64_t n = c.batch / limit;
    return ((c.batch + n - 1) / n + TILE_ROWS - 1) / TILE_ROWS * TILE_ROWS;
}

static int run_step(const mshgnn_plan* p, StepCall& c) {
    auto whole = [p](StepCall& s) { const int rc = run_forward(p, s); return rc ? rc : run_backward(p, s); };
    const int64_t cw = step_chunk_windows(p, c);
    if (!cw) return whole(c);
    const mshgnn_desc& d = p->hp.d;
    const int64_t eb = d.dtype == MSHGNN_BF16 ? 2 : 4;
    const int64_t n_out = d.type_nodes[d.out_type], orow = n_out * d.out_channels;
    int idx = 0;
    for (int64_t w0 = 0; w0 < c.batch; w0 += cw, ++idx) {
        const void* xc[MSHGNN_MAX_TYPES] = {};
        for (int t = 0; t < p->n_types; ++t)
            xc[t] = static_cast<const char*>(c.x[t]) + w0 * d.type_nodes[t] * (c.x_pitch ? c.x_pitch[t] : (int64_t)d.type_width[t]) * eb;
        StepCall sub = c;
        sub.x = xc; sub.batch = std::min(cw, c.batch - w0); sub.chunk = StepChunk{c.batch, idx};
        sub.out = c.out + w0 * orow;
        if (c.loss == LossKind::MSE) sub.y = c.y + w0 * orow; else sub.labels = c.labels + w0 * n_out;
        if (const int rc = whole(sub)) return rc;
    }
    return MSHGNN_OK;
}

static int fill_wide_src(const mshgnn_plan* p, int src_bytes, const void* const* src, const int64_t* src_pitch, const char* who, WideSrc& w) {
    if (!p || !src) return set_err(MSHGNN_EINVAL, std::string("null argument to ") + who);
    if (src_bytes != 4 && src_bytes != 8) return set_err(MSHGNN_EINVAL, std::string(who) + ": src_bytes must be 4 (fp32) or 8 (fp64)");
    if (p->gen || p->hp.d.dtype == MSHGNN_F32) return set_err(MSHGNN_EUNSUPPORTED, std::string(who) + ": wide source rows run on the bf16 and split-bf16 plans of the LDS-resident kernels");
    w.bytes = src_bytes;
    for (int t = 0; t < p->n_types; ++t) {
        if (!src[t]) return set_err(MSHGNN_EINVAL, std::string(who) + ": null source tensor");
        w.p[t] = src[t]; w.pitch[t] = src_pitch ? src_pitch[t] : p->hp.d.type_width[t];
        if (w.pitch[t] < p->hp.d.type_width[t]) return set_err(MSHGNN_EINVAL, std::string(who) + ": src_pitch smaller than the feature width");
        if (((uintptr_t)src[t] % (src_bytes == 8 ? 8 : 4)) != 0) return set_err(MSHGNN_EINVAL, std::string(who) + ": source tensor not aligned to its element size");
        if (src_bytes == 4 && (p->hp.d.type_width[t] & 1) == 0 && ((((uintptr_t)src[t]) | (uintptr_t)(w.pitch[t] * 4)) & 7) != 0)
            return set_err(MSHGNN_EINVAL, std::string(who) + ": fp32 source rows of an even width must start 8-byte aligned (base and pitch)");
    }
    return MSHGNN_OK;
}

static int forward_entry(const mshgnn_plan* p, const WideSrc* wide, const void* const* x, const int64_t* x_pitch, const float* params, float* out,
                         void* workspace, int64_t batch, int training, void* stream) {
    if (!p || !x || !params || !out || !workspace) return set_err(MSHGNN_EINVAL, "null argument to mshgnn_forward");
    if (batch < 1 || batch > (1 << 24)) return set_err(MSHGNN_EINVAL, "batch must be in [1, 2^24]");
    for (int t = 0; t < p->n_types; ++t) if (!x[t]) return set_err(MSHGNN_EINVAL, "null input tensor");
    StepCall c;
    c.x = x; c.x_pitch = x_pitch; c.params = params; c.out = out; c.ws = (char*)workspace; c.batch = batch; c.training = training; c.stream = (hipStream_t)stream;
    c.wide = wide;
    return run_forward(p, c);
}

extern "C" int mshgnn_forward(const mshgnn_plan* p, const void* const* x, const int64_t* x_pitch, const float* params, float* out,
                              void* workspace, int64_t batch, int training, void* stream) {
    return forward_entry(p, nullptr, x, x_pitch, params, out, workspace, batch, training, stream);
}

extern "C" int mshgnn_forward_src(const mshgnn_plan* p, int src_bytes, const void* const* src, const int64_t* src_pitch, void* const* x_rows, const int64_t* x_pitch,
                                  const float* params, float* out, void* workspace, int64_t batch, int training, void* stream) {
    if (!x_rows) return set_err(MSHGNN_EINVAL, "mshgnn_forward_src: x_rows is null (the plan-dtype rows the encoder materialises)");
    WideSrc w{};
    if (const int rc = fill_wide_src(p, src_bytes, src, src_pitch, "mshgnn_forward_src", w)) return rc;
    return forward_entry(p, &w, x_rows, x_pitch, params, out, workspace, batch, training, stream);
}

static int backward_entry(const mshgnn_plan* p, const void* const* x, const int64_t* x_pitch, const float* params, float* grad_params, void* workspace,
                          int64_t batch, void* stream, StepCall& c) {
    if (batch < 1 || batch > (1 << 24)) return set_err(MSHGNN_EINVAL, "batch must be in [1, 2^24]");
    c.x = x; c.x_pitch = x_pitch; c.params = params; c.grad_params = grad_params; c.ws = (char*)workspace; c.batch = batch; c.stream = (hipStream_t)stream;
    return MSHGNN_OK;
}

extern "C" int mshgnn_backward(const mshgnn_plan* p, const void* const* x, const int64_t* x_pitch, const float* params, const float* grad_out,
                               float* grad_params, void* workspace, int64_t batch, void* stream) {
    if (!p || !x || !params || !grad_out || !workspace) return set_err(MSHGNN_EINVAL, "null argument to mshgnn_backward");
    StepCall c;
    if (const int rc = backward_entry(p, x, x_pitch, params, grad_params, workspace, batch, stream, c)) return rc;
    c.grad_out = grad_out;
    return run_backward(p, c);
}

extern "C" int mshgnn_backward_mse(const mshgnn_plan* p, const void* const* x, const int64_t* x_pitch, const float* params, const float* out,
                                   const float* y, float* loss_out, float* grad_params, void* workspace, int64_t batch, void* stream) {
    if (!p || !x || !params || !out || !y || !loss_out || !workspace) return set_err(MSHGNN_EINVAL, "null argument to mshgnn_backward_mse");
    StepCall c;
    if (const int rc = backward_entry(p, x, x_pitch, params, grad_params, workspace, batch, stream, c)) return rc;
    c.loss = LossKind::MSE; c.out = const_cast<float*>(out); c.y = y; c.loss_out = loss_out;
    return run_backward(p, c);
}

extern "C" int mshgnn_backward_ce(const mshgnn_plan* p, const void* const* x, const int64_t* x_pitch, const float* params, const float* out,
                                  const int32_t* labels, float* loss_out, float* grad_params, void* workspace, int64_t batch, void* stream) {
    if (!p || !x || !params || !out || !labels || !loss_out || !workspace) return set_err(MSHGNN_EINVAL, "null argument to mshgnn_backward_ce");
    StepCall c;
    if (const int rc = backward_entry(p, x, x_pitch, params, grad_params, workspace, batch, stream, c)) return rc;
    if (p->hp.d.out_channels != 2) return set_err(MSHGNN_EINVAL, "mshgnn_backward_ce needs a 2-logit (contact classification) plan");
    c.loss = LossKind::CE; c.out = const_cast<float*>(out); c.labels = labels; c.loss_out = loss_out;
    return run_backward(p, c);
}

static int step_call(const mshgnn_plan* p, const char* who, const void* const* x, const int64_t* x_pitch, const float* params, LossKind kind, const void* target,
                     float* out, float* loss_out, float* grad_params, void* workspace, int64_t batch, void* stream, StepCall& c) {
    if (!p || !x || !params || !target || !out || !loss_out || !grad_params || !workspace) return set_err(MSHGNN_EINVAL, std::string("null argument to ") + who);
    if (batch < 1 || batch > (1 << 24)) return set_err(MSHGNN_EINVAL, "batch must be in [1, 2^24]");
    c.x = x; c.x_pitch = x_pitch; c.params = params; c.out = out; c.ws = (char*)workspace; c.batch = batch; c.training = 1; c.stream = (hipStream_t)stream;
    c.loss = kind; c.loss_out = loss_out; c.grad_params = grad_params;
    if (kind == LossKind::MSE) c.y = static_cast<const float*>(target); else c.labels = static_cast<const int32_t*>(target);
    return MSHGNN_OK;
}
static int step_entry(const mshgnn_plan* p, const WideSrc* wide, const void* const* x, const int64_t* x_pitch, const float* params, LossKind kind, const void* target,
                      float* out, float* loss_out, float* grad_params, void* workspace, int64_t batch, void* stream) {
    StepCall c;
    if (const int rc = step_call(p, kind == LossKind::CE ? "mshgnn_step_ce" : "mshgnn_step_mse", x, x_pitch, params, kind, target, out, loss_out, grad_params, workspace, batch, stream, c)) return rc;
    for (int t = 0; t < p->n_types; ++t) if (!x[t]) return set_err(MSHGNN_EINVAL, "null input tensor");
    if (kind == LossKind::CE && p->hp.d.out_channels != 2) return set_err(MSHGNN_EINVAL, "mshgnn_step_ce: the classification wrappers have two logits per foot");
    c.wide = wide;
    return run_step(p, c);
}

extern "C" int mshgnn_step_mse(const mshgnn_plan* p, const void* const* x, const int64_t* x_pitch, const float* params, const float* y,
                               float* out, float* loss_out, float* grad_params, void* workspace, int64_t batch, void* stream) {
    return step_entry(p, nullptr, x, x_pitch, params, LossKind::MSE, y, out, loss_out, grad_params, workspace, batch, stream);
}

extern "C" int mshgnn_step_ce(const mshgnn_plan* p, const void* const* x, const int64_t* x_pitch, const float* params, const int32_t* labels,
                              float* out, float* loss_out, float* grad_params, void* workspace, int64_t batch, void* stream) {
    return step_entry(p, nullptr, x, x_pitch, params, LossKind::CE, labels, out, loss_out, grad_params, workspace, batch, stream);
}

extern "C" int mshgnn_step_mse_src(const mshgnn_plan* p, int src_bytes, const void* const* src, const int64_t* src_pitch, void* const* x_rows, const int64_t* x_pitch,
                                   const float* params, const float* y, float* out, float* loss_out, float* grad_params, void* workspace, int64_t batch, void* stream) {
    if (!x_rows) return set_err(MSHGNN_EINVAL, "mshgnn_step_mse_src: x_rows is null (the plan-dtype rows the encoder materialises)");
    WideSrc w{};
// ... 256 lines not shown
```

### morphsym_hgnn_amd/csrc/mshgnn_device.hpp

```cpp
#pragma once
#include <type_traits>
#include <hip/hip_runtime.h>

#include <cmath>
#include <cstdio>
#include <cstdlib>
#include <cstring>
#include <string>
#include <vector>

#include "mshgnn_plan.hpp"

using namespace mshgnn;

typedef float f32x4 __attribute__((ext_vector_type(4)));
typedef float f32x2 __attribute__((ext_vector_type(2)));
typedef float f32x16 __attribute__((ext_vector_type(16)));
typedef __bf16 bf16x8 __attribute__((ext_vector_type(8)));
typedef unsigned int u32x4 __attribute__((ext_vector_type(4)));
typedef double f64x2 __attribute__((ext_vector_type(2)));
typedef unsigned int u32x2 __attribute__((ext_vector_type(2)));

#ifndef ENC_NT
#define ENC_NT 0
// ... 129 lines not shown
__device__ __forceinline__ int lds_swz(int row) { return (row & 15) ^ ((row & 4) << 1); }
template <typename T> __device__ __forceinline__ int lds_chunk(int blk, int row, int c) {
    return blk * Prec<T>::BLK + row * Prec<T>::RB + ((c ^ lds_swz(row)) << 4);
}
template <typename T> __device__ __forceinline__ int lds_elem(int blk, int row, int col) {
    return lds_chunk<T>(blk, row, col / Prec<T>::EPC) + (col % Prec<T>::EPC) * (int)sizeof(T);
}

template <typename T> __device__ __forceinline__ void lds_load_oct(const char* smem, int blk, int row, int col, f32x4& lo, f32x4& hi) {
    if constexpr (sizeof(T) == 4) {
        lo = *reinterpret_cast<const f32x4*>(smem + lds_chunk<T>(blk, row, col / 4));
        hi = *reinterpret_cast<const f32x4*>(smem + lds_chunk<T>(blk, row, col / 4 + 1));
    } else load_oct(reinterpret_cast<const T*>(smem + lds_chunk<T>(blk, row, col / 8)), lo, hi);
}
template <typename T> __device__ __forceinline__ void lds_store_oct(char* smem, int blk, int row, int col, f32x4 lo, f32x4 hi) {
    if constexpr (sizeof(T) == 4) {
        *reinterpret_cast<f32x4*>(smem + lds_chunk<T>(blk, row, col / 4)) = lo;
        *reinterpret_cast<f32x4*>(smem + lds_chunk<T>(blk, row, col / 4 + 1)) = hi;
    } else store_oct(reinterpret_cast<T*>(smem + lds_chunk<T>(blk, row, col / 8)), lo, hi);
}

template <typename T> __device__ __forceinline__ void load_afrag(typename Prec<T>::AFrag& a, const char* smem, int blk, int lane_) {
    const int lane = opaque(lane_);
    const int row = lane & 15, g = lane >> 4;
#pragma unroll
    for (int t = 0; t < Prec<T>::NAV; ++t) {
        const u32x4 v = *reinterpret_cast<const u32x4*>(smem + lds_chunk<T>(blk, row, g * Prec<T>::NAV + t));
        a.v[t] = __builtin_bit_cast(typename Prec<T>::Vec, v);
    }
}
template <typename T> struct AOff {
    int o[Prec<T>::NAV];
    __device__ __forceinline__ explicit AOff(int lane) {
        const int row = lane & 15, g = lane >> 4;
#pragma unroll
        for (int t = 0; t < Prec<T>::NAV; ++t) o[t] = opaque(lds_chunk<T>(0, row, g * Prec<T>::NAV + t));
    }
};
template <typename T> __device__ __forceinline__ void load_afrag(typename Prec<T>::AFrag& a, const char* smem, int blk, const AOff<T>& ao) {
    const int base = blk * Prec<T>::BLK;
#pragma unroll
    for (int t = 0; t < Prec<T>::NAV; ++t) {
        const u32x4 v = *reinterpret_cast<const u32x4*>(smem + base + ao.o[t]);
        a.v[t] = __builtin_bit_cast(typename Prec<T>::Vec, v);
    }
}
template <typename T> __device__ __forceinline__ void load_bfrag(typename Prec<T>::BFrag& b, const T* wpack, int pack, int wv, int lane) {
    constexpr int NBV = Prec<T>::NBV;
    const u32x4* base = reinterpret_cast<const u32x4*>(wpack + (size_t)pack * H * H) + (size_t)wv * NBV * 64 + lane;
#pragma unroll
    for (int v = 0; v < NBV; ++v) {
        const u32x4 x = base[v * 64];
        b.v[v] = __builtin_bit_cast(typename Prec<T>::Vec, x);
    }
}

template <typename T> __device__ __forceinline__ void load_bfrag_u(typename Prec<T>::BFrag& b, const T* wpack, int pack, int wv, unsigned lane16) {
    constexpr int NBV = Prec<T>::NBV;
    gchar* base = uniform_ptr(reinterpret_cast<const char*>(wpack) + ((size_t)pack * H * H * sizeof(T)) + (size_t)wv * NBV * 64 * 16);
#pragma unroll
    for (int v = 0; v < NBV; ++v) b.v[v] = __builtin_bit_cast(typename Prec<T>::Vec, gload16(base + v * 1024, lane16));
}

__device__ __forceinline__ void mac(Prec<float>::Acc& acc, const Prec<float>::AFrag& x, const Prec<float>::BFrag& w) {
#pragma unroll
    for (int t4 = 0; t4 < 8; ++t4)
#pragma unroll
        for (int e = 0; e < 4; ++e) {
            acc.c[0] = __builtin_amdgcn_mfma_f32_16x16x4f32(w.v[t4][e], x.v[t4][e], acc.c[0], 0, 0, 0);
            acc.c[1] = __builtin_amdgcn_mfma_f32_16x16x4f32(w.v[8 + t4][e], x.v[t4][e], acc.c[1], 0, 0, 0);
        }
}
__device__ __forceinline__ void mac(Prec<__bf16>::Acc& acc, const Prec<__bf16>::AFrag& x, const Prec<__bf16>::BFrag& w) {
#pragma unroll
    for (int t = 0; t < 4; ++t) {
        acc.c[0] = __builtin_amdgcn_mfma_f32_16x16x32_bf16(w.v[t], x.v[t], acc.c[0], 0, 0, 0);
        acc.c[1] = __builtin_amdgcn_mfma_f32_16x16x32_bf16(w.v[4 + t], x.v[t], acc.c[1], 0, 0, 0);
    }
}

template <typename T> __device__ __forceinline__ void acc_init_bias(typename Prec<T>::Acc& a, const float* bias, int wv, int lane) {
    if (bias == nullptr) { acc_fill(a, 0.f); return; }
    a.c[0] = *reinterpret_cast<const f32x4*>(bias + wv * 32 + c_feat(0, lane));
    a.c[1] = *reinterpret_cast<const f32x4*>(bias + wv * 32 + c_feat(1, lane));
}
template <typename T> __device__ __forceinline__ void acc_init_bias_u(typename Prec<T>::Acc& a, const float* bias_row, int wv, unsigned loff) {
    gchar* base = uniform_ptr(reinterpret_cast<const char*>(bias_row + wv * 32));
    a.c[0] = __builtin_bit_cast(f32x4, gload16(base, loff));
    a.c[1] = __builtin_bit_cast(f32x4, gload16(base + 16, loff));
}
struct BiasQ { f32x4 b[2]; };
__device__ __forceinline__ BiasQ load_bias(const float* bias, int wv, int lane) {
    BiasQ q;
    q.b[0] = *reinterpret_cast<const f32x4*>(bias + wv * 32 + c_feat(0, lane));
    q.b[1] = *reinterpret_cast<const f32x4*>(bias + wv * 32 + c_feat(1, lane));
    return q;
}

constexpr int LAYER_THREADS = 512;

template <typename T> struct RowMap {
    static constexpr int VPB = Prec<T>::ROWS * Prec<T>::CPR, NPB = LAYER_THREADS / VPB;
    int sub, row, c;
    __device__ __forceinline__ explicit RowMap(int tid) : sub(tid / VPB), row((tid % VPB) / Prec<T>::CPR), c(tid % Prec<T>::CPR) {}
};

template <typename T>
__device__ __forceinline__ void stage_nodes(char* smem, const T* src, int NN, int w0, int B, int tid) {
    constexpr int EPC = Prec<T>::EPC, NPB = RowMap<T>::NPB, BATCH = 6;
    const RowMap<T> m(tid);
    for (int nb = m.sub; nb < NN; nb += NPB * BATCH) {
        u32x4 v[BATCH];
#pragma unroll
        for (int i = 0; i < BATCH; ++i) {
            const int n = nb + i * NPB;
            v[i] = u32x4{0, 0, 0, 0};
            if (n < NN && w0 + m.row < B) v[i] = *reinterpret_cast<const u32x4*>(src + act_idx(w0 + m.row, n, B) + m.c * EPC);
        }
#pragma unroll
        for (int i = 0; i < BATCH; ++i) {
            const int n = nb + i * NPB;
            if (n < NN) *reinterpret_cast<u32x4*>(smem + lds_chunk<T>(n, m.row, m.c)) = v[i];
        }
    }
}

__device__ __forceinline__ size_t relu_byte(int n, int B, int w, int f) {
    return ((((size_t)n * 4 + (f >> 5)) * ((B + 15) >> 4) + (w >> 4)) << 6) + (((f >> 3) & 3) << 4) + (w & 15);
}
__device__ __forceinline__ size_t relu_tile_base(int n, int B, int tile, int wn) { return (((size_t)n * 4 + wn) * ((B + 15) >> 4) + tile) << 6; }
__device__ __forceinline__ void unpack_oct(u32x4 r, f32x4& lo, f32x4& hi) {
    lo = f32x4{__builtin_bit_cast(float, r[0] << 16), __builtin_bit_cast(float, r[0] & 0xffff0000u),
               __builtin_bit_cast(float, r[1] << 16), __builtin_bit_cast(float, r[1] & 0xffff0000u)};
    hi = f32x4{__builtin_bit_cast(float, r[2] << 16), __builtin_bit_cast(float, r[2] & 0xffff0000u),
               __builtin_bit_cast(float, r[3] << 16), __builtin_bit_cast(float, r[3] & 0xffff0000u)};
}
template <typename T>
__device__ __forceinline__ unsigned relu_with_bits(typename Prec<T>::Acc& acc) {
    unsigned bits = 0;
#pragma unroll
    for (int fb = 1; fb >= 0; --fb)
#pragma unroll
        for (int j = 3; j >= 0; --j) {
            const float xf = acc.c[fb][j];
            const int y = max(__float_as_int(xf), 0);
            acc.c[fb][j] = __int_as_float(y);
            bits = __builtin_amdgcn_alignbit(bits, (unsigned)y + 0x7fffffffu, 31);
        }
    return bits;
}
struct PrepArgs {
    const float* params; void* wpack; float* bias; const PackDesc* packs; const BiasDesc* biases; int n_packs; int n_biases;
    int pack0 = 0, pack_n = -1;
};

struct EncArgs {
    const void* x[MSHGNN_MAX_TYPES]; int64_t pitch[MSHGNN_MAX_TYPES]; int vb[MSHGNN_MAX_TYPES];
    int width[MSHGNN_MAX_TYPES], nodes[MSHGNN_MAX_TYPES], tbase[MSHGNN_MAX_TYPES + 1], nkc[MSHGNN_MAX_TYPES];
    int pack0[MSHGNN_MAX_TYPES], bias_idx[MSHGNN_MAX_TYPES], sign_off[MSHGNN_MAX_TYPES], wg_prefix[MSHGNN_MAX_TYPES + 1];
    int n_types, tiles, B, NN;
    unsigned char node_list[64]; int node_off[MSHGNN_MAX_TYPES]; unsigned long long skip_mask;
    int aligned;
    const void* wpack; const float* bias; const uint8_t* signs; void* x0;
    uint8_t* mask0;
    PrepArgs prep; int prep_vecs;
};

struct LabelArgs {
    const float* lab; int64_t lab_cs;
    const float* quat_src; int64_t quat_cs;
    const int64_t* starts; int64_t B; int T;
    const int* label_cols; int n_label, label_rotate;
    float* y; float* quat; int32_t* labels_int;
};

__device__ __forceinline__ void window_labels_one(const LabelArgs& a, int64_t b) {
    const int64_t row = a.starts[b] + a.T - 1;
    const float* lab = a.lab + row;
    const int64_t lcs = a.lab_cs;
    double R[3][3] = {{1, 0, 0}, {0, 1, 0}, {0, 0, 1}};
    float qv[4] = {0.f, 0.f, 0.f, 1.f};
    if (a.quat_src) {
        const float* qp = a.quat_src + row;
        const int64_t qcs = a.quat_cs;
        const float q0 = qp[0], q1 = qp[qcs], q2 = qp[2 * qcs], q3 = qp[3 * qcs];
        qv[0] = q0; qv[1] = q1; qv[2] = q2; qv[3] = q3;
        if (a.label_rotate) {
            double x = q0, yq = q1, z = q2, s = q3;
            const double nrm = sqrt(x * x + yq * yq + z * z + s * s);
            x /= nrm; yq /= nrm; z /= nrm; s /= nrm;
            R[0][0] = 1 - 2 * (yq * yq + z * z); R[0][1] = 2 * (x * yq - z * s); R[0][2] = 2 * (x * z + yq * s);
            R[1][0] = 2 * (x * yq + z * s); R[1][1] = 1 - 2 * (x * x + z * z); R[1][2] = 2 * (yq * z - x * s);
            R[2][0] = 2 * (x * z - yq * s); R[2][1] = 2 * (yq * z + x * s); R[2][2] = 1 - 2 * (x * x + yq * yq);
        }
    }
    constexpr int LMAX = 24;
    for (int k0 = 0; k0 < a.n_label; k0 += LMAX) {
        float v[LMAX];
#pragma unroll
        for (int j = 0; j < LMAX; ++j) v[j] = k0 + j < a.n_label ? lab[a.label_cols[k0 + j] * lcs] : 0.f;
        if (a.label_rotate) {
#pragma unroll
            for (int j = 0; j + 2 < LMAX; j += 3) {
                if (k0 + j + 2 >= a.n_label) break;
#pragma unroll
                for (int i = 0; i < 3; ++i)
                    a.y[b * a.n_label + k0 + j + i] = (float)(R[i][0] * (double)v[j] + R[i][1] * (double)v[j + 1] + R[i][2] * (double)v[j + 2]);
            }
        } else {
#pragma unroll
            for (int j = 0; j < LMAX; ++j) {
                if (k0 + j >= a.n_label) break;
                a.y[b * a.n_label + k0 + j] = v[j];
                if (a.labels_int) a.labels_int[b * a.n_label + k0 + j] = v[j] != 0.f;
            }
        }
    }
    if (a.quat_src && a.quat) { a.quat[b * 4] = qv[0]; a.quat[b * 4 + 1] = qv[1]; a.quat[b * 4 + 2] = qv[2]; a.quat[b * 4 + 3] = qv[3]; }
}

struct SeriesSrc {
    const unsigned long long* run_ptr;
    const int* rows;
    const int64_t* starts;
    int row0[MSHGNN_MAX_TYPES];
    int T;
    LabelArgs lab;
    const double* stats;
    int n_runs;
};

constexpr int WIN_MAX_SRC = 12;
constexpr int WIN_MAX_RUNS = 128;
struct WindowArgs {
    const float* src[WIN_MAX_SRC]; int64_t src_cstride[WIN_MAX_SRC];
    void* x[MSHGNN_MAX_TYPES]; int64_t x_pitch[MSHGNN_MAX_TYPES]; int nodes[MSHGNN_MAX_TYPES];
    const int* runs; int n_runs;
    const int* rows; int n_rows;
    const int64_t* starts; int64_t B; int T, normalize;
    const int* label_cols; int n_label, label_src, label_rotate, quat_src;
    float* y; float* quat;
};

struct RunStats { double mean, sd; };
__device__ __forceinline__ double wave_sum_f64(double v) {
#pragma unroll
    for (int m = 32; m >= 1; m >>= 1) v += __shfl_xor(v, m, 64);
    return v;
}
__device__ __forceinline__ RunStats run_stats(const float (&v)[4], int len, int lane) {
#pragma clang fp contract(off)
    double s1 = 0.0;
#pragma unroll
    for (int q = 0; q < 4; ++q) if (2 * lane + 128 * (q >> 1) + (q & 1) < len) s1 += (double)v[q];
    RunStats r;
    r.mean = wave_sum_f64(s1) / (double)len;
    double qs = 0.0;
#pragma unroll
    for (int q = 0; q < 4; ++q) if (2 * lane + 128 * (q >> 1) + (q & 1) < len) { const double dlt = (double)v[q] - r.mean; qs = fma(dlt, dlt, qs); }
    r.sd = sqrt(wave_sum_f64(qs) / (double)(len - 1));
    return r;
}
__device__ __forceinline__ float standardise_one(float x, double mean, double sd) {
#pragma clang fp contract(off)
    const double z = ((double)x - mean) / sd;
    float f = z == z ? (float)z : 0.0f;
    asm volatile("" : "+v"(f));
    return f;
}

__device__ __forceinline__ void splice8f(u32x4& a0, u32x4& a1, const u32x4 b0, const u32x4 b1, int n0) {
    unsigned sft[8] = {b0[0], b0[1], b0[2], b0[3], b1[0], b1[1], b1[2], b1[3]};
    if (n0 & 4) {
#pragma unroll
        for (int e = 7; e >= 4; --e) sft[e] = sft[e - 4];
    }
    if (n0 & 2) {
#pragma unroll
        for (int e = 7; e >= 2; --e) sft[e] = sft[e - 2];
    }
    if (n0 & 1) {
#pragma unroll
        for (int e = 7; e >= 1; --e) sft[e] = sft[e - 1];
    }
#pragma unroll
    for (int e = 0; e < 4; ++e) {
        a0[e] = e < n0 ? a0[e] : sft[e];
        a1[e] = e + 4 < n0 ? a1[e] : sft[e + 4];
    }
}
__device__ __forceinline__ void standardise_oct(u32x4& a0, u32x4& a1, int n0, bool has_a, bool has_b, RunStats sa, RunStats sb) {
#pragma unroll
    for (int e = 0; e < 8; ++e) {
        const bool first = e < n0;
        const float x = __builtin_bit_cast(float, e < 4 ? a0[e & 3] : a1[e & 3]);
        const float z = standardise_one(x, first ? sa.mean : sb.mean, first ? sa.sd : sb.sd);
        const unsigned r = __builtin_bit_cast(unsigned, (first ? has_a : has_b) ? z : x);
        if (e < 4) a0[e & 3] = r; else a1[e & 3] = r;
    }
}

struct WideSrc {
    int bytes;
    const void* p[MSHGNN_MAX_TYPES];
    int64_t pitch[MSHGNN_MAX_TYPES];
};
struct StepChunk { int64_t total_windows; int index; };
// ... 62 lines not shown
template <typename T> __device__ __forceinline__ u32x4 chunk_keep_first(u32x4 v, int nv) {
    if constexpr (sizeof(T) == 4) {
#pragma unroll
        for (int e = 0; e < 4; ++e) if (e >= nv) v[e] = 0u;
    } else {
#pragma unroll
        for (int e = 0; e < 4; ++e) {
            const unsigned m = (2 * e < nv ? 0x0000ffffu : 0u) | (2 * e + 1 < nv ? 0xffff0000u : 0u);
            v[e] &= m;
        }
    }
    return v;
}
template <typename T> __device__ __forceinline__ u32x4 sign_xor(const uint8_t* s) {
    if constexpr (sizeof(T) == 4) {
        const unsigned w = *reinterpret_cast<const unsigned*>(s);
        return u32x4{(w & 1u) << 31, ((w >> 8) & 1u) << 31, ((w >> 16) & 1u) << 31, ((w >> 24) & 1u) << 31};
    } else {
        const unsigned w0 = reinterpret_cast<const unsigned*>(s)[0], w1 = reinterpret_cast<const unsigned*>(s)[1];
        return u32x4{((w0 & 1u) << 15) | (((w0 >> 8) & 1u) << 31), (((w0 >> 16) & 1u) << 15) | (((w0 >> 24) & 1u) << 31),
                     ((w1 & 1u) << 15) | (((w1 >> 8) & 1u) << 31), (((w1 >> 16) & 1u) << 15) | (((w1 >> 24) & 1u) << 31)};
    }
}

template <typename T> __device__ __forceinline__ u32x4 chunk_add(u32x4 a, u32x4 b) {
    union U { u32x4 v; T e[Prec<T>::EPC]; } x, y, r;
    x.v = a; y.v = b;
#pragma unroll
    for (int e = 0; e < Prec<T>::EPC; ++e) r.e[e] = from_f32<T>(to_f32(x.e[e]) + to_f32(y.e[e]));
    return r.v;
}
template <typename T> __device__ __forceinline__ u32x4 chunk_mask_pos(u32x4 v, u32x4 act) {
    union U { u32x4 v; T e[Prec<T>::EPC]; } x, y;
    x.v = v; y.v = act;
#pragma unroll
    for (int e = 0; e < Prec<T>::EPC; ++e) if (!(to_f32(y.e[e]) > 0.f)) x.e[e] = from_f32<T>(0.f);
    return x.v;
}
template <typename T> __device__ __forceinline__ u32x4 chunk_mask_bits(u32x4 v, unsigned bits) {
    if constexpr (sizeof(T) == 4) {
#pragma unroll
        for (int e = 0; e < 4; ++e) if (!((bits >> e) & 1u)) v[e] = 0u;
    } else {
#pragma unroll
        for (int e = 0; e < 4; ++e) {
            const int lo = __builtin_amdgcn_sbfe((int)bits, 2 * e, 1), hi = __builtin_amdgcn_sbfe((int)bits, 2 * e + 1, 1);
            v[e] &= (unsigned)((lo & 0xffff) | (hi & (int)0xffff0000));
        }
    }
    return v;
}


template <typename T> __device__ __forceinline__ void load8(const T* p, float (&v)[8]) {
    if constexpr (sizeof(T) == 4) {
        const f32x4 a = reinterpret_cast<const f32x4*>(p)[0], b = reinterpret_cast<const f32x4*>(p)[1];
        v[0] = a[0]; v[1] = a[1]; v[2] = a[2]; v[3] = a[3]; v[4] = b[0]; v[5] = b[1]; v[6] = b[2]; v[7] = b[3];
    } else {
        const u32x4 r = *reinterpret_cast<const u32x4*>(p);
#pragma unroll
        for (int e = 0; e < 4; ++e) { v[2 * e] = __builtin_bit_cast(float, r[e] << 16); v[2 * e + 1] = __builtin_bit_cast(float, r[e] & 0xffff0000u); }
    }
}
template <typename T> __device__ __forceinline__ void store8(T* p, const float (&v)[8]) {
    if constexpr (sizeof(T) == 4) {
        reinterpret_cast<f32x4*>(p)[0] = f32x4{v[0], v[1], v[2], v[3]};
        reinterpret_cast<f32x4*>(p)[1] = f32x4{v[4], v[5], v[6], v[7]};
    } else {
        union { u32x4 r; __bf16 e[8]; } u;
#pragma unroll
        for (int e = 0; e < 8; ++e) u.e[e] = (__bf16)v[e];
        *reinterpret_cast<u32x4*>(p) = u.r;
    }
}


__device__ __forceinline__ void split_oct(f32x4 a, f32x4 b, u32x4& hi, u32x4& lo) {
    hi = pack_oct(a, b);
    f32x4 ha, hb; unpack_oct(hi, ha, hb);
    lo = pack_oct(a - ha, b - hb);
}
__device__ __forceinline__ void join_oct(u32x4 hi, u32x4 lo, f32x4& a, f32x4& b) {
    f32x4 la, lb; unpack_oct(hi, a, b); unpack_oct(lo, la, lb);
    a += la; b += lb;
}

constexpr int PREP_PITCH0 = 132, PREP_PITCH1 = 68, PREP_TILE_FLOATS = 64 * PREP_PITCH0 > 128 * PREP_PITCH1 ? 64 * PREP_PITCH0 : 128 * PREP_PITCH1;
template <typename T, bool SPLIT_OUT>
__device__ __forceinline__ void prep_pack_half(const PrepArgs& a, int pack, int h, float* tile, int tid) {
    constexpr int EPC = Prec<T>::EPC, NBV = Prec<T>::NBV;
    const PackDesc* pdp = a.packs + pack;
    struct { int orient, n_src, ld, col0, ncols; } pd{pdp->orient, pdp->n_src, pdp->ld, pdp->col0, pdp->ncols};
    const bool o0 = pd.orient == 0;
    const int pitch = o0 ? PREP_PITCH0 : PREP_PITCH1;
    {
        const int nb4 = o0 ? 32 : 16;
        const int b4 = (tid % nb4) * 4, a0 = tid / nb4, apass = 256 / nb4, npass = (o0 ? 64 : 128) / apass;
        f32x4 sum[8];
#pragma unroll
        for (int ps = 0; ps < 8; ++ps) sum[ps] = f32x4{0.f, 0.f, 0.f, 0.f};
        for (int i = 0; i < pd.n_src; ++i) {
            const int64_t src_i = pdp->src[i];
            const float* base = a.params + src_i;
            const bool al = ((src_i + (o0 ? pd.col0 : 0)) % 4 == 0) && pd.ld % 4 == 0;
            f32x4 g[8];
#pragma unroll
            for (int ps = 0; ps < 8; ++ps) {
                const int ar = a0 + ps * apass;
                const float* q = o0 ? base + (int64_t)(64 * h + ar) * pd.ld + pd.col0 + b4 : base + (int64_t)ar * pd.ld + 64 * h + b4;
                const int nvalid = o0 ? pd.ncols - b4 : 4;
                g[ps] = f32x4{0.f, 0.f, 0.f, 0.f};
                if (ps < npass) {
                    if (al && nvalid >= 4) g[ps] = *reinterpret_cast<const f32x4*>(q);
                    else {
#pragma unroll
                        for (int e = 0; e < 4; ++e) if (e < nvalid) g[ps][e] = q[e];
                    }
                }
            }
#pragma unroll
            for (int ps = 0; ps < 8; ++ps) sum[ps] += g[ps];
        }
#pragma unroll
        for (int ps = 0; ps < 8; ++ps) if (ps < npass) *reinterpret_cast<f32x4*>(&tile[(a0 + ps * apass) * pitch + b4]) = sum[ps];
    }
    __syncthreads();
    constexpr int VPH = 2 * NBV * 64;
    const size_t vec0 = (size_t)pack * (H * H / EPC) + (size_t)(2 * h) * NBV * 64;
    for (int r = tid; r < VPH; r += 256) {
        const int lane = r % 64, v = (r / 64) % NBV, wl = r / (64 * NBV);
        const int i16 = lane & 15;
        int k, cl;
        if constexpr (sizeof(T) == 4) { k = 32 * (lane >> 4) + 4 * (v & 7); cl = wl * 32 + 8 * (i16 >> 2) + 4 * (v >> 3) + (i16 & 3); }
        else { k = 32 * (lane >> 4) + 8 * (v & 3); cl = wl * 32 + 8 * (i16 >> 2) + 4 * (v >> 2) + (i16 & 3); }
        float s[EPC];
#pragma unroll
        for (int x = 0; x < EPC; ++x) s[x] = o0 ? tile[cl * PREP_PITCH0 + k + x] : tile[(k + x) * PREP_PITCH1 + cl];
        if constexpr (SPLIT_OUT) {
            u32x4 hi, lo;
            split_oct(f32x4{s[0], s[1], s[2], s[3]}, f32x4{s[4], s[5], s[6], s[7]}, hi, lo);
            u32x4* dst = reinterpret_cast<u32x4*>(a.wpack);
            dst[vec0 + r] = hi;
            dst[(size_t)a.n_packs * (H * H / EPC) + vec0 + r] = lo;
        } else {
            T* dst = reinterpret_cast<T*>(a.wpack) + (vec0 + r) * EPC;
            if constexpr (sizeof(T) == 4) *reinterpret_cast<f32x4*>(dst) = f32x4{s[0], s[1], s[2], s[3]};
            else *reinterpret_cast<u32x4*>(dst) = pack_oct(f32x4{s[0], s[1], s[2], s[3]}, f32x4{s[4], s[5], s[6], s[7]});
        }
    }
}
template <typename T, bool SPLIT_OUT> __global__ __launch_bounds__(256) void k_prep_tiled(PrepArgs a) {
    __shared__ __attribute__((aligned(16))) float tile[PREP_TILE_FLOATS];
    const int tid = threadIdx.x;
    if ((int)blockIdx.x < 2 * a.n_packs) { prep_pack_half<T, SPLIT_OUT>(a, blockIdx.x >> 1, blockIdx.x & 1, tile, tid); return; }
    const int b = ((int)blockIdx.x - 2 * a.n_packs) * 256 + tid;
    if (b < a.n_biases * H) {
        const BiasDesc* bd = a.biases + b / H;
        const int ns = bd->n_src;
        float s = 0.f;
        for (int i = 0; i < ns; ++i) s += a.params[bd->src[i] + (b % H)];
        a.bias[b] = s;
    }
}
constexpr int PREP_TILED_MIN = 200;
inline bool prep_use_tiled(int n_packs) {
    static const int forced = [] { const char* e = TUNE_ENV("MSHGNN_PREP_TILED"); return e ? atoi(e) : -1; }();
    return forced >= 0 ? forced != 0 : n_packs >= PREP_TILED_MIN;
}
inline unsigned prep_tiled_grid(int n_packs, int n_biases) { return (unsigned)(2 * n_packs + (n_biases * H + 255) / 256); }

struct StackArgs {
    static constexpr bool full = false;
    static constexpr int nt_mode = -1;
    const void* tile_in;
    char* ws;
    size_t x_off[MAX_L + 1], dx_off[MAX_L + 1];
    size_t mask_off[MAX_L], hb_off[MAX_L], t1_off[MAX_L], dh_off[MAX_L], du_off[MAX_L];
    const void* wpack; const float* bias; const int* tables; int prog_off[MAX_L];
    int prog_off_b[MAX_L];
    int B, NN, L, training, dbg;
    const float* params; const float* out_mask; float* out; int64_t off_dec_w, off_dec_b; int node0, n_out, dout;
    const float* y; float* dec_slabs; float inv_n;
    const int32_t* labels;
    size_t mask0_off;
    long long* stamps;
    int lo_blk, n_img;
    int scr0;
    int red_off;
    int stash_nt;
    int stagger;
};
template <int NT, bool FULL = true> struct StackView {
    static constexpr bool full = FULL;
    static constexpr int nt_mode = NT;
    const StackArgs& s;
    const void* const& tile_in; char* const& ws;
    const size_t (&x_off)[MAX_L + 1]; const size_t (&dx_off)[MAX_L + 1];
    const size_t (&mask_off)[MAX_L]; const size_t (&hb_off)[MAX_L]; const size_t (&t1_off)[MAX_L]; const size_t (&dh_off)[MAX_L]; const size_t (&du_off)[MAX_L];
    const void* const& wpack; const float* const& bias; const int* const& tables; const int (&prog_off)[MAX_L]; const int (&prog_off_b)[MAX_L];
    const int& NN; const int& L; const int& dbg; const int& node0; const int& n_out; const size_t& mask0_off; long long* const& stamps; const int& stagger;
    int B, training, stash_nt;
    __device__ __forceinline__ StackView(const StackArgs& a, bool step)
        : s(a), tile_in(a.tile_in), ws(a.ws), x_off(a.x_off), dx_off(a.dx_off), mask_off(a.mask_off), hb_off(a.hb_off), t1_off(a.t1_off), dh_off(a.dh_off), du_off(a.du_off),
          wpack(a.wpack), bias(a.bias), tables(a.tables), prog_off(a.prog_off), prog_off_b(a.prog_off_b), NN(a.NN), L(a.L), dbg(a.dbg), node0(a.node0), n_out(a.n_out),
          mask0_off(a.mask0_off), stamps(a.stamps), stagger(a.stagger), B(a.B), training(step ? 1 : a.training), stash_nt(a.stash_nt) {
        asm volatile("" : "+s"(B));
    }
};
__device__ __forceinline__ const StackArgs& args_of(const StackArgs& a) { return a; }
template <int NT, bool FULL> __device__ __forceinline__ const StackArgs& args_of(const StackView<NT, FULL>& v) { return v.s; }

__device__ __forceinline__ void stash_store(void* p, u32x4 v, bool nt) {
    if (nt) asm volatile("global_store_dwordx4 %0, %1, off nt" :: "v"(p), "v"(v) : "memory");
    else *reinterpret_cast<u32x4*>(p) = v;
}
template <class A> __device__ __forceinline__ void stash_store_a(const A& a, void* p, u32x4 v) {
    if constexpr (A::nt_mode == 1) __builtin_nontemporal_store(v, reinterpret_cast<u32x4*>(p));
    else if constexpr (A::nt_mode == 0) *reinterpret_cast<u32x4*>(p) = v;
    else stash_store(p, v, a.stash_nt != 0);
}
template <class A> __device__ __forceinline__ void stash_store_u(const A& a, gwchar* base, unsigned off, u32x4 v) {
    static_assert(A::nt_mode >= 0, "compile-time store policy");
    if constexpr (A::nt_mode == 1) gstore16_nt(base, off, v); else gstore16(base, off, v);
}
inline int stash_nt_for(int force, int64_t B, int stash_rows, int row_bytes) {
    static const int64_t limit_mb = []() { const char* e = TUNE_ENV("MSHGNN_STASH_NT_MB"); return (int64_t)(e ? atoi(e) : 200); }();
    if (force == 0 || force == 1) return force;
    return (int64_t)stash_rows * B * row_bytes > (limit_mb << 20) ? 1 : 0;
}
template <typename HP> inline int stash_rows_of(const HP& hp) {
    int rows = 0;
    for (int l = 0; l < hp.L; ++l)
        for (int n = 0; n < hp.NN; ++n) rows += (hp.live_n[l][n] && l + 1 < hp.L ? 1 : 0) + (hp.need_n[l][n] ? 1 : 0);
    return rows;
}
template <class A> __device__ __forceinline__ void stack_stagger(const A& a) {
    if (a.stagger > 0 && blockIdx.x >= (gridDim.x + 1) / 2)
        for (int i = 0; i < a.stagger; i += 1024) __builtin_amdgcn_s_sleep(16);
}
#ifdef MSHGNN_SEG_STAMPS
constexpr int FS_EXTRA_BLK = 6;
#else
constexpr int FS_EXTRA_BLK = 0;
#endif
#if defined(MSHGNN_FS_STAMPS) || defined(MSHGNN_SEG_STAMPS)
#define FS_STAMP(k) do { if (a.stamps && tid == 0) a.stamps[(size_t)blockIdx.x * 32 + (k)] = clock64(); } while (0)
#define FS_STAMP2(k) do { if (a.stamps && tid == 0) a.stamps[(size_t)gridDim.x * 32 + (size_t)blockIdx.x * 32 + (k)] = clock64(); } while (0)
#else
#define FS_STAMP(k) do { } while (0)
#define FS_STAMP2(k) do { } while (0)
#endif

#ifdef MSHGNN_PAD_VALU
__device__ __forceinline__ void pad_valu() {
    int d0 = 0, d1 = 0;
#pragma unroll
    for (int i = 0; i < MSHGNN_PAD_VALU; i += 2) { asm volatile("v_add_u32 %0, %0, 1" : "+v"(d0)); asm volatile("v_add_u32 %0, %0, 1" : "+v"(d1)); }
}
#else
__device__ __forceinline__ void pad_valu() {}
#endif
#ifdef MSHGNN_PAD_SALU
__device__ __forceinline__ void pad_salu() {
    int d0 = 0;
#pragma unroll
    for (int i = 0; i < MSHGNN_PAD_SALU; ++i) asm volatile("s_add_u32 %0, %0, 1" : "+s"(d0) :: "scc");
}
#else
__device__ __forceinline__ void pad_salu() {}
#endif

struct FProg {
    static constexpr bool is_static = false;
    int pk, pcnt, pb;
    __device__ __forceinline__ FProg() : pk(0), pcnt(0), pb(0) {}
    __device__ __forceinline__ FProg(const int* prog, int lane) : pk(prog[lane]), pcnt(prog[64 + lane]), pb(prog[128 + lane]) {}
    __device__ __forceinline__ int pack(int sgi) const { return __builtin_amdgcn_readlane(pk, sgi); }
    __device__ __forceinline__ int counts(int sgi) const { return __builtin_amdgcn_readlane(pcnt, sgi); }
    __device__ __forceinline__ int at(int i) const { return (__builtin_amdgcn_readlane(pb, i >> 2) >> ((i & 3) << 3)) & 0xff; }
    __device__ __forceinline__ void settle() { asm volatile("" : "+v"(pk), "+v"(pcnt), "+v"(pb)); }
};

struct FHdr {
    static constexpr bool is_static = false;
    int h0, h1;
    __device__ __forceinline__ FHdr() : h0(0), h1(0) {}
    __device__ __forceinline__ FHdr(const int* hdr, int lane) : h0(hdr[lane]), h1(lane < FH_SIZE - 64 ? hdr[64 + lane] : 0) {}
    __device__ __forceinline__ int operator[](int i) const { return i < 64 ? __builtin_amdgcn_readlane(h0, i & 63) : __builtin_amdgcn_readlane(h1, i & 63); }
    __device__ __forceinline__ void settle() { asm volatile("" : "+v"(h0), "+v"(h1)); }
};

template <class SP, int DIR, int LL> struct SHdr {
    static constexpr bool is_static = true;
    __device__ __forceinline__ constexpr int operator[](int i) const { return DIR ? SP::bwd[LL][i] : SP::fwd[LL][i]; }
    __device__ __forceinline__ void settle() const {}
};
template <class SP, int DIR, int LL, int G> struct SProg {
    static constexpr bool is_static = true;
    static constexpr int BASE = FH_SIZE + G * FPROG_LEN;
    __device__ __forceinline__ constexpr int raw(int i) const { return DIR ? SP::bwd[LL][BASE + i] : SP::fwd[LL][BASE + i]; }
    __device__ __forceinline__ constexpr int pack(int sgi) const { return raw(sgi); }
    __device__ __forceinline__ constexpr int counts(int sgi) const { return raw(64 + sgi); }
    __device__ __forceinline__ constexpr int at(int i) const { return (raw(128 + (i >> 2)) >> ((i & 3) << 3)) & 0xff; }
    __device__ __forceinline__ void settle() const {}
};

// ... 170 lines not shown
        const float* W = a.params + a.off_dec_w;
        const bool ce = a.labels != nullptr, fuse = a.y != nullptr || ce;
        T* dxl = reinterpret_cast<T*>(a.ws + a.dx_off[a.L]);
        float accw[DMAX][8], accb[DMAX], lsum = 0.f;
        if (fuse) {
#pragma unroll
            for (int dd = 0; dd < DMAX; ++dd) { accb[dd] = 0.f;
#pragma unroll
                for (int e = 0; e < 8; ++e) accw[dd][e] = 0.f; }
        }
        DecOps<DMAX, NPP> ops;
        if constexpr (PRE) ops = *pre; else decoder_ops_load_w<DMAX, NPP>(a, tid, ops);
        auto& Wv = ops.Wv; auto& bv = ops.bv; auto& mk = ops.mk; auto& yv = ops.yv; auto& labv = ops.labv;
        FS_STAMP(24);
        for (int f0 = tid >> 8; f0 < a.n_out; f0 += NPP * (THREADS / 256)) {
            float ov[NPP][DMAX], dxv[NPP][8];
            if (!(PRE && f0 == (tid >> 8))) decoder_ops_load<THREADS, DMAX, NPP>(a, tid, w0, B, f0, false, ops);
#pragma unroll
            for (int i = 0; i < NPP; ++i) {
                const int f = f0 + i * (THREADS / 256);
                const bool live = f < a.n_out;
                f32x4 x0, x1;
                lds_load_oct<T>(smem, a.node0 + (live ? f : f0), row, c * 8, x0, x1);
                if constexpr (SPLIT) {
                    f32x4 l0, l1;
                    lds_load_oct<T>(smem, a.lo_blk + a.node0 + (live ? f : f0), row, c * 8, l0, l1);
                    x0 += l0; x1 += l1;
                }
                const float x[8] = {x0[0], x0[1], x0[2], x0[3], x1[0], x1[1], x1[2], x1[3]};
#pragma unroll
                for (int e = 0; e < 8; ++e) dxv[i][e] = 0.f;
                const bool ok = live && w0 + row < B;
#pragma unroll
                for (int dd = 0; dd < DMAX; ++dd) {
                    ov[i][dd] = 0.f;
                    if (dd < a.dout && live) {
                        float sum = 0.f;
#pragma unroll
                        for (int e = 0; e < 8; ++e) sum = __builtin_fmaf(x[e], Wv[dd][e], sum);
                        sum = row16_sum(sum);
                        ov[i][dd] = (sum + bv[dd]) * mk[i][dd];
                    }
                }
                if (fuse && ok) {
                    float ce_g[2] = {0.f, 0.f};
                    if (ce) {
                        const float l0 = ov[i][0], l1 = ov[i][1];
                        const float m = fmaxf(l0, l1), e0 = expf(l0 - m), e1 = expf(l1 - m), se = e0 + e1;
                        ce_g[0] = (e0 / se - (labv[i] ? 0.f : 1.f)) * a.inv_n; ce_g[1] = (e1 / se - (labv[i] ? 1.f : 0.f)) * a.inv_n;
                        if (c == 0) lsum += (m + logf(se)) - (labv[i] ? l1 : l0);
                    }
#pragma unroll
                    for (int dd = 0; dd < DMAX; ++dd) {
                        if (dd < a.dout) {
                            float g;
                            if (ce) g = ce_g[dd & 1] * mk[i][dd];
                            else {
                                const float dlt = ov[i][dd] - yv[i][dd];
                                g = 2.0f * dlt * a.inv_n * mk[i][dd];
                                if (c == 0) lsum = __builtin_fmaf(dlt, dlt, lsum);
                            }
                            accb[dd] += g;
#pragma unroll
                            for (int e = 0; e < 8; ++e) { accw[dd][e] = __builtin_fmaf(g, x[e], accw[dd][e]); dxv[i][e] = __builtin_fmaf(g, Wv[dd][e], dxv[i][e]); }
                        }
                    }
                }
            }
#pragma unroll
            for (int i = 0; i < NPP; ++i) {
                const int f = f0 + i * (THREADS / 256);
                const bool ok = f < a.n_out && w0 + row < B;
                const size_t r = (size_t)(w0 + row) * a.n_out + f;
                if (c == 0 && ok) {
#pragma unroll
                    for (int dd = 0; dd < DMAX; ++dd) if (dd < a.dout) a.out[r * a.dout + dd] = ov[i][dd];
                }
                if (fuse && ok) {
                    if constexpr (SPLIT) {
                        u32x4 hi, lo;
                        split_oct(f32x4{dxv[i][0], dxv[i][1], dxv[i][2], dxv[i][3]}, f32x4{dxv[i][4], dxv[i][5], dxv[i][6], dxv[i][7]}, hi, lo);
                        T* q = dxl + 2 * act_idx(w0 + row, a.node0 + f, B) + c * 8;
                        *reinterpret_cast<u32x4*>(q) = hi; *reinterpret_cast<u32x4*>(q + H) = lo;
                    } else store8<T>(dxl + act_idx(w0 + row, a.node0 + f, B) + c * 8, dxv[i]);
                }
                if constexpr (TOLDS) {
                    if (f < a.n_out) {
                        if (!ok) {
#pragma unroll
                            for (int e = 0; e < 8; ++e) dxv[i][e] = 0.f;
                        }
                        if constexpr (SPLIT) {
                            u32x4 hi, lo;
                            split_oct(f32x4{dxv[i][0], dxv[i][1], dxv[i][2], dxv[i][3]}, f32x4{dxv[i][4], dxv[i][5], dxv[i][6], dxv[i][7]}, hi, lo);
                            *reinterpret_cast<u32x4*>(smem + lds_chunk<T>(a.node0 + f, row, c)) = hi;
                            *reinterpret_cast<u32x4*>(smem + lds_chunk<T>(a.lo_blk + a.node0 + f, row, c)) = lo;
                        } else store8<T>(reinterpret_cast<T*>(smem + lds_chunk<T>(a.node0 + f, row, c)), dxv[i]);
                    }
                }
            }
        }
        FS_STAMP(25);
        if (fuse) {
#pragma unroll
            for (int dd = 0; dd < DMAX; ++dd) {
                if (dd < a.dout) {
#pragma unroll
                    for (int e = 0; e < 8; ++e) { accw[dd][e] += __shfl_xor(accw[dd][e], 16, 64); accw[dd][e] += __shfl_xor(accw[dd][e], 32, 64); }
                    accb[dd] += __shfl_xor(accb[dd], 16, 64); accb[dd] += __shfl_xor(accb[dd], 32, 64);
                }
            }
            lsum += __shfl_xor(lsum, 16, 64); lsum += __shfl_xor(lsum, 32, 64);
            FS_STAMP(26);
            __syncthreads();
            float* red = reinterpret_cast<float*>(smem + a.red_off);
            if (lane < 16) {
#pragma unroll
                for (int dd = 0; dd < DMAX; ++dd) {
#pragma unroll
                    for (int e = 0; e < 8; ++e) red[wv * DEC_SLAB_FLOATS + dd * H + lane * 8 + e] = accw[dd][e];
                    if (lane == 0) red[wv * DEC_SLAB_FLOATS + 8 * H + dd] = accb[dd];
                }
                if (lane == 0) red[wv * DEC_SLAB_FLOATS + 8 * H + 8] = lsum;
            }
            __syncthreads();
            FS_STAMP(27);
            float* slab = a.dec_slabs + (size_t)blockIdx.x * DEC_SLAB_FLOATS;
            for (int i = tid; i < 8 * H + 9; i += THREADS) {
                if (i >= a.dout * H && i < 8 * H) continue;
                float s2 = 0.f;
#pragma unroll
                for (int k = 0; k < THREADS / 64; ++k) s2 += red[k * DEC_SLAB_FLOATS + i];
                slab[i] = s2;
            }
        }
    }
}

template <typename T, int THREADS, bool SPLIT = false, bool TOLDS = false>
__device__ __forceinline__ void decoder_tail(const StackArgs& a, char* smem, int tid, int lane, int wv, int w0, int B) {
    if (a.dout <= 4) decoder_tail_impl<T, THREADS, 4, SPLIT, TOLDS>(a, smem, tid, lane, wv, w0, B);
    else decoder_tail_impl<T, THREADS, 8, SPLIT, TOLDS>(a, smem, tid, lane, wv, w0, B);
}
constexpr int DEC_NPP_STATIC = 4;

struct DecArgs {
    const void* xl; void* dxl; const float* params; const float* out_mask; float* out; const float* gout; float* slabs;
    int64_t off_w, off_b; int B, NN, node0, n_out, dout, slab0;
    const float* y; float* loss; float inv_n;
    const int32_t* labels;
};


struct GradwArgs {
    const char* ws; size_t buf_off[BUF_COUNT];
    const void* x[MSHGNN_MAX_TYPES]; int64_t pitch[MSHGNN_MAX_TYPES]; int nodes[MSHGNN_MAX_TYPES]; int vb[MSHGNN_MAX_TYPES];
    const int* items; const int* lanes; const int* lane_order; const uint8_t* signs; float* slabs; int B, n_lanes, n_parts, n_pad;
    int aligned;
    int dbg;
    long long* stamps;
    SeriesSrc ser;
};

constexpr int GWB_KW = 64;
constexpr int GWB_PITCH = 128;
__device__ __forceinline__ int gwb_elem(int row, int col) { return row * GWB_PITCH + ((((col >> 3) ^ ((row & 3) << 2)) << 3) | (col & 7)); }
typedef short s16x4 __attribute__((ext_vector_type(4)));

__device__ __forceinline__ bf16x8 tr_frag(const __bf16* tile, int w_base, int col_base, int lane) {
    const int g = lane >> 4, q = (lane >> 2) & 3, pp = lane & 3;
    const __bf16* p0 = tile + gwb_elem(w_base + 8 * (g >> 1) + q, col_base + 16 * (g & 1) + 4 * pp);
    const s16x4 lo = __builtin_amdgcn_ds_read_tr16_b64_v4i16((__attribute__((address_space(3))) s16x4*)(p0));
    const s16x4 hi = __builtin_amdgcn_ds_read_tr16_b64_v4i16((__attribute__((address_space(3))) s16x4*)(p0 + 4 * GWB_PITCH));
    typedef short s16x8 __attribute__((ext_vector_type(8)));
    const s16x8 v = {lo[0], lo[1], lo[2], lo[3], hi[0], hi[1], hi[2], hi[3]};
    return __builtin_bit_cast(bf16x8, v);
}


struct FinArgs { const int* fin; const int* fin0; const int* targets; const float* slabs; const float* dec_slabs; float* grad; int n_lanes, n_parts; float* loss; float inv_n;
                 int n_dec; int accumulate; };

struct mshgnn_gen_state;
struct ProfRec { int slot; hipEvent_t a, b; };
struct mshgnn_plan {
    HostPlan hp;
    bool prof = false;
    std::vector<ProfRec> recs;
    std::vector<hipEvent_t> free_events;
    int* d_tables = nullptr; uint8_t* d_signs = nullptr; float* d_out_mask = nullptr;
    PackDesc* d_packs = nullptr; BiasDesc* d_biases = nullptr;
    int* d_ig_nodes = nullptr;
    bool attr_set = false;
    bool use_fused = false;
    bool use_slab = false;
    bool slab_force = false; int n_cu = 256;
    int stash_nt_force = -1;
    int64_t step_chunk = 32768;
    bool use_step = false;
    bool use_spec = true;
    const char* spec_name = "";
    std::string spec_name_buf;
    int stagger = 0;
    int n_types = 0;
    mshgnn_gen_state* gen = nullptr;
    int dbg = 0, dbg_gw = 0;
    bool slab_for(int tiles) const { return use_slab && (slab_force || tiles > n_cu); }
};

inline long long* stamp_ptr(const char* name) {
#if defined(MSHGNN_FS_STAMPS) || defined(MSHGNN_SEG_STAMPS) || MSHGNN_GW_STAMPS_BUILD
    const char* e = getenv(name);
    return e ? reinterpret_cast<long long*>((uintptr_t)strtoull(e, nullptr, 0)) : nullptr;
#else
    (void)name; return nullptr;
#endif
}

struct ProfScope {
    mshgnn_plan* p; hipStream_t st; ProfRec r{}; bool on;
    ProfScope(const mshgnn_plan* pc, int slot, hipStream_t s) : p(const_cast<mshgnn_plan*>(pc)), st(s), on(pc->prof) {
        if (!on) return;
        auto get = [&]() { hipEvent_t e; if (!p->free_events.empty()) { e = p->free_events.back(); p->free_events.pop_back(); } else (void)hipEventCreate(&e); return e; };
        r.slot = slot; r.a = get(); r.b = get();
        (void)hipEventRecord(r.a, st);
    }
    ~ProfScope() { if (on) { (void)hipEventRecord(r.b, st); p->recs.push_back(r); } }
};

template <typename K> inline int set_lds_attr(K kernel, int bytes) {
    HIPCHK(hipFuncSetAttribute(reinterpret_cast<const void*>(kernel), hipFuncAttributeMaxDynamicSharedMemorySize, bytes));
    return MSHGNN_OK;
}

inline int vec_bytes(const void* base, int64_t pitch_elems, int esize) {
    const uint64_t a = (uint64_t)(uintptr_t)base | (uint64_t)(pitch_elems * esize);
    if ((a & 15) == 0) return 16;
    if ((a & 7) == 0) return 8;
    if ((a & 3) == 0) return 4;
    return esize;
}



inline int gw_parts_for(int plan_parts, int lanes, int ipl, int64_t B, int chunk_windows, int n_cu) {
    static const int forced = [] { const char* e = TUNE_ENV("MSHGNN_GW_PARTS"); return e ? atoi(e) : 0; }();
    if (forced > 0) return std::min(forced, plan_parts);
    const int64_t nchunks = (B + chunk_windows - 1) / chunk_windows;
    const double cu_scale = 256.0 / (double)std::max(1, n_cu);
    const int cap_wg = 45 * std::max(1, n_cu) / 16;
    const int qmax = std::max(1, std::min(plan_parts, cap_wg / std::max(1, lanes)));
    auto cost = [&](int q) {
        const double W = (double)lanes * q * cu_scale;
        const double t = 1.1 + (W <= 480.0 ? 0.0024 : 0.0032) * W;
        return (double)((nchunks + q - 1) / q) * std::max(1, ipl) * t + 0.012 * W; };
    int best = qmax; double best_cost = cost(qmax);
    for (int q = 1; q < qmax; ++q) if (cost(q) < best_cost) { best_cost = cost(q); best = q; }
    return best_cost < 0.97 * cost(qmax) ? best : qmax;
}

enum class LossKind { NONE, MSE, CE };
struct StepCall {
    const void* const* x = nullptr;
    const int64_t* x_pitch = nullptr;
    const float* params = nullptr;
    float* out = nullptr;
    char* ws = nullptr;
    int64_t batch = 0;
    int training = 1;
    hipStream_t stream = nullptr;
    const float* grad_out = nullptr;
    LossKind loss = LossKind::NONE;
    const float* y = nullptr;
    const int32_t* labels = nullptr;
    float* loss_out = nullptr;
    float* grad_params = nullptr;
    const WideSrc* wide = nullptr;
    const SeriesSrc* series = nullptr;
    bool gradw_from_series = false;
    int gw_phase = -1;
    StepChunk chunk{0, 0};
    bool dec_done = false;
    bool stack_done = false;

    const float* y_fused() const { return loss == LossKind::MSE ? y : nullptr; }
    const int32_t* labels_fused() const { return loss == LossKind::CE ? labels : nullptr; }
    int64_t total_windows() const { return chunk.total_windows ? chunk.total_windows : batch; }
    int accumulates() const { return chunk.index > 0 ? 1 : 0; }
};

#define SPEC_SHARD_LIST(X) X(1) X(2) X(3) X(4) X(5) X(6) X(7)
#define SPEC_CAT2(a, b) a##b
#define SPEC_CAT(a, b) SPEC_CAT2(a, b)

int run_finalize(const mshgnn_plan* p, const StepCall& c, const mshgnn_ws_layout& lay, int gw_parts);
int x3_set_attrs(mshgnn_plan* p);
int x3_attach_program(mshgnn_plan* p, void* selector);
int x3_forward(const mshgnn_plan* p, StepCall& c);
int x3_backward(const mshgnn_plan* p, const StepCall& c);
int x3_launch_prep(const PrepArgs& a, hipStream_t st);
int launch_prep(const PrepArgs& a, bool split, hipStream_t st);
int gen_create(mshgnn_plan* p, const mshgnn_desc* desc);
void gen_destroy(mshgnn_plan* p);
const mshgnn_info* gen_info(const mshgnn_plan* p);
namespace mshgnn { namespace gen { struct GenPlan; } }
const mshgnn::gen::GenPlan* gen_plan(const mshgnn_plan* p);
const uint8_t* gen_signs(const mshgnn_plan* p);
const std::vector<mshgnn_kernel_stat>* gen_kstats(const mshgnn_plan* p);
void gen_layout(const mshgnn_plan* p, int64_t batch, int training, mshgnn_ws_layout* out);
int gen_host_compile(const mshgnn_desc* desc, mshgnn_info* info, int32_t* n_tables);
int gen_forward(const mshgnn_plan* p, StepCall& c);
int gen_backward(const mshgnn_plan* p, const StepCall& c);
```

### morphsym_hgnn_amd/csrc/mshgnn_plan.hpp

```cpp
#pragma once
#include <algorithm>
#include <array>
#include <cmath>
#include <cstdint>
#include <cstdio>
#include <cstring>
#include <string>
#include <vector>

#include "../../include/mshgnn.h"

#ifdef MSHGNN_TUNING
#define TUNE_ENV(name) std::getenv(name)
#else
#define TUNE_ENV(name) (static_cast<const char*>(nullptr))
#endif

namespace mshgnn {

constexpr int H = 128;
constexpr int GMAX = 12;
constexpr int TILE_ROWS = 16;
constexpr int MAX_L = 16;
#ifndef LDS_LIMIT_KB
#define LDS_LIMIT_KB 160
#endif
constexpr int LDS_LIMIT = LDS_LIMIT_KB * 1024;
constexpr int SLAB_FLOATS = H * H + H;
constexpr int NWG_DEC = 512;
constexpr int DEC_SLAB_FLOATS = 8 * H + 16;
#ifndef GW_IPL_MAX
#define GW_IPL_MAX 2
#endif
constexpr int GW_IPL = GW_IPL_MAX;
#ifndef GW_TARGET_WGS
#define GW_TARGET_WGS 768.0
#endif

#ifndef GW_XCD_SLACK
#define GW_XCD_SLACK 1
#endif

enum { OP_LOADW = 0, OP_MAC = 1 };
enum { KIND_RELU = 0, KIND_MLP = 1 };
enum { NK_DEAD = 0, NK_RELU = 1, NK_MLP = 2 };
enum { GF_RESIDUAL = 1, GF_ENC_MASK = 2, GF_STORE_MASK = 4, GF_LDS_EPI = 8 };

enum { GH_KIND = 0, GH_NSLOTS, GH_BIAS, GH_NSEG, GH_W1, GH_W2, GH_B1, GH_B2, GH_FLAGS, GH_PC0, GH_PC1, GH_PAD2,
       GH_NODES = 12, GH_MLPIDX = 12 + GMAX, GH_SCR = 12 + 2 * GMAX, GH_SIZE = 12 + 3 * GMAX };
constexpr int WPROG_LEN = 128;
enum { BH_NGROUPS = 0, BH_NMLP, BH_W2, BH_W1, BH_KIND = 8, BH_MLPNODES = 8 + 128, BH_SIZE = 8 + 128 + GMAX };

constexpr int FS_HS = 10;
constexpr int FS_MAXN = 2 * FS_HS;
constexpr int FPROG_LEN = 192;
enum { FH_NSEG = 0, FH_NMLP, FH_W1, FH_W2, FH_B1, FH_B2, FH_FLAGS, FH_MLP0,
       FH_KIND = 8,
       FH_BIAS = 8 + FS_MAXN,
       FH_OUT = 8 + 2 * FS_MAXN,
       FH_RES = 8 + 3 * FS_MAXN,
       FH_SLOTA = 8 + 4 * FS_MAXN,
       FH_SLOTB = FH_SLOTA + 16,
       FH_SIZE = FH_SLOTB + 16,
       FH_NEXT = FH_SLOTA };
static_assert(FH_NEXT + 8 + 20 <= FH_SIZE && MSHGNN_MAX_TYPES <= 4, "header: next-layer array");
constexpr int SL_HA = 12, SL_HB = 6, SL_HB_MAX = 8, SL_THREADS = 256;
constexpr int SL_CBA = 2, SL_CBB = 3;
enum { FF_RESIDUAL = 1, FF_ENC_MASK = 2, FF_SCR_ALIAS = 4, FF_A_EMPTY = 8, FF_B_EMPTY = 16 };

enum { BUF_X = 0, BUF_DX = 17, BUF_DH = 34, BUF_HB = 50, BUF_T1 = 66, BUF_DU = 82, BUF_IN = 98, BUF_MASK = 102, BUF_COUNT = 118 };
constexpr int ITEM_INTS = 10;
constexpr int TGT_INTS = 8;
constexpr int LANE_INTS = 4;
constexpr int FIN_INTS = 8;
enum { FIN_MATRIX = 0, FIN_BIAS = 1, FIN_ZERO = 2, FIN_DEC_W = 3, FIN_DEC_B = 4 };

struct PackDesc {
    int orient;
    int n_src;
    int64_t src[8];
    int ld;
    int col0;
    int ncols;
};
struct BiasDesc { int n_src; int64_t src[8]; };

struct HostPlan {
    mshgnn_desc d{};
    void* jit_prog = nullptr;
    std::vector<int32_t> rel_src, rel_dst, rel_mean, rel_edge_off, edges;
    std::vector<float> in_mask[MSHGNN_MAX_TYPES], out_mask;
    std::vector<int64_t> off_enc_w, off_enc_b, off_rel_w, off_rel_b, off_root_w;
    int L = 0, NT = 0, NR = 0, NN = 0;
    int type_base[MSHGNN_MAX_TYPES + 1]{};
    int node_type[64]{};
    int n_mlp = 0;
    int n_blk = 0;
    bool mlp_scratch = false;
    int rows = TILE_ROWS;
    int blk_bytes = 8192;
    int gmax = GMAX;
    int esize = 4;
    bool split = false;
    int planes = 1;
    int n_img = 0;
    int lo_blk = 0;
    int gw_target = (int)GW_TARGET_WGS;
    bool live[MAX_L][MSHGNN_MAX_TYPES]{};
    bool need_dx[MAX_L][MSHGNN_MAX_TYPES]{};
    bool live_n[MAX_L][64]{}, need_n[MAX_L][64]{};
    bool prune_nodes = true;
    int enc_live_nodes = 0;
    std::vector<PackDesc> packs;
    std::vector<BiasDesc> biases;
    std::vector<int> pack_root[2], pack_rel[2];
    int pack_mlp[2][2]{};
    std::vector<int> pack_enc_base; std::vector<int> enc_nkc;
    std::vector<int> bias_layer;
    int bias_mlp[2]{}; std::vector<int> bias_enc;
    std::vector<uint8_t> signs; std::vector<int> sign_off;
    std::vector<int32_t> tables;
    int fwd_prog_off[MAX_L]{}, bwd_prog_off[MAX_L]{};
    bool fused = false;
    int fs_fwd_off[MAX_L]{}, fs_bwd_off[MAX_L]{};
    bool slab = false;
    int sl_fwd_off[MAX_L]{}, sl_bwd_off[MAX_L]{}, sl_ta = -1, sl_hb = SL_HB, sl_blk = 0;
    bool sl_alias = false;
    int fs_blk = 0;
    bool x3_alias = false;
    int ks_stack_fwd = -1, ks_stack_bwd = -1;
    int item_off = 0, n_items = 0, tgt_off = 0, n_targets = 0, lane_off = 0, n_lanes = 0, n_parts = 1, n_wg_gradw = 0;
    int lane_order_off = 0, n_lanes_pad = 0, gw_ipl = 1;
    int order_ph_off[2]{}, npad_ph[2]{}, n_fin_ph0 = 0;
    int64_t grad_split = -1;
    int fin_off = 0, n_fin = 0;
    int enc_tile_mb = 4;
    int n_slabs = 0;
    std::vector<float> out_mask_f;
    std::vector<mshgnn_kernel_stat> kstats;
    int ks_prep = 0, ks_enc = 0, ks_layer_fwd0 = 0, ks_dec_fwd = 0, ks_dec_bwd = 0, ks_layer_bwd0 = 0, ks_gradw = 0, ks_fin = 0, ks_stack_step = 0;
    mshgnn_info info{};
    std::string err;
};

inline bool fail(HostPlan& p, const std::string& m) { p.err = m; return false; }

inline int add_pack(HostPlan& p, int orient, const std::vector<int64_t>& src, int ld, int col0, int ncols) {
    PackDesc q{}; q.orient = orient; q.n_src = (int)src.size(); q.ld = ld; q.col0 = col0; q.ncols = ncols;
    for (size_t i = 0; i < src.size(); ++i) q.src[i] = src[i];
    p.packs.push_back(q); return (int)p.packs.size() - 1;
}
inline int add_bias(HostPlan& p, const std::vector<int64_t>& src) {
    BiasDesc b{}; b.n_src = (int)src.size(); for (size_t i = 0; i < src.size(); ++i) b.src[i] = src[i];
    p.biases.push_back(b); return (int)p.biases.size() - 1;
}

inline bool compile_plan(const mshgnn_desc* din, HostPlan& p) {
    if (!din) return fail(p, "null descriptor");
    p.d = *din;
    const mshgnn_desc& d = p.d;
    if (d.n_types < 1 || d.n_types > MSHGNN_MAX_TYPES) return fail(p, "n_types must be 1..4");
    if (d.hidden != H) return fail(p, "this build supports hidden_channels == 128 only");
    if (d.num_layers < 1 || d.num_layers > MAX_L) return fail(p, "num_layers must be 1..16");
    if (d.n_rel < 1 || d.n_rel > 64) return fail(p, "n_rel must be 1..64");
    if (d.dtype != MSHGNN_F32 && d.dtype != MSHGNN_BF16 && d.dtype != MSHGNN_BF16X3) return fail(p, "dtype must be MSHGNN_F32, MSHGNN_BF16 or MSHGNN_BF16X3");
    if (d.out_type < 0 || d.out_type >= d.n_types) return fail(p, "out_type out of range");
    if (d.out_channels < 1 || d.out_channels > 8) return fail(p, "out_channels must be 1..8");
    if (!d.rel_src || !d.rel_dst || !d.rel_mean || !d.rel_edge_off || !d.edges) return fail(p, "null relation arrays");
    if (!d.off_enc_w || !d.off_enc_b || !d.off_rel_w || !d.off_rel_b || !d.off_root_w) return fail(p, "null offset arrays");
    p.L = d.num_layers; p.NT = d.n_types; p.NR = d.n_rel;
    const int L = p.L, NT = p.NT, NR = p.NR;
    const bool has_mlp = (d.flags & MSHGNN_FLAG_BASE_MLP) != 0;
    const bool residual = (d.flags & MSHGNN_FLAG_RESIDUAL) != 0;
    if (has_mlp && (d.mlp_type < 0 || d.mlp_type >= NT)) return fail(p, "mlp_type out of range");
    p.type_base[0] = 0;
    {
        int64_t total = 0;
        for (int t = 0; t < NT; ++t) total += std::max(0, d.type_nodes[t]);
        if (total > 64) return fail(p, "topology has too many nodes per window for the LDS-resident layer kernel (max 20 fp32 / 40 bf16)");
    }
    for (int t = 0; t < NT; ++t) {
        if (d.type_nodes[t] < 1) return fail(p, "every node type needs >= 1 node");
        if (d.type_width[t] < 1) return fail(p, "every node type needs input width >= 1");
        p.type_base[t + 1] = p.type_base[t] + d.type_nodes[t];
        for (int i = 0; i < d.type_nodes[t]; ++i) p.node_type[p.type_base[t] + i] = t;
    }
    p.NN = p.type_base[NT];
    p.esize = d.dtype == MSHGNN_F32 ? 4 : 2;
    p.split = d.dtype == MSHGNN_BF16X3; p.planes = p.split ? 2 : 1;
#ifndef GWX3_TARGET_WGS
#define GWX3_TARGET_WGS 768
#endif
    p.gw_target = p.split ? GWX3_TARGET_WGS : (int)GW_TARGET_WGS;
    { const char* e = TUNE_ENV("MSHGNN_GW_TARGET"); if (e && std::atoi(e) >= 64) p.gw_target = std::atoi(e); }
    p.blk_bytes = TILE_ROWS * H * p.esize;
    if (!p.split && (int64_t)p.NN * p.blk_bytes > LDS_LIMIT)
        return fail(p, "topology has too many nodes per window for the LDS-resident layer kernel (max 20 fp32 / 40 bf16)");
    p.rows = TILE_ROWS;
    p.gmax = d.dtype == MSHGNN_F32 ? GMAX : 8;
    p.n_mlp = has_mlp ? d.type_nodes[d.mlp_type] : 0;
    if (p.n_mlp > p.gmax) return fail(p, "base_transform type has too many nodes for one accumulator group");

    p.rel_src.assign(d.rel_src, d.rel_src + NR); p.rel_dst.assign(d.rel_dst, d.rel_dst + NR);
    p.rel_mean.assign(d.rel_mean, d.rel_mean + NR); p.rel_edge_off.assign(d.rel_edge_off, d.rel_edge_off + NR + 1);
    const int E = p.rel_edge_off[NR];
    if (p.rel_edge_off[0] != 0 || E < 0) return fail(p, "bad rel_edge_off");
    p.edges.assign(d.edges, d.edges + 2 * (size_t)E);
    p.off_enc_w.assign(d.off_enc_w, d.off_enc_w + NT); p.off_enc_b.assign(d.off_enc_b, d.off_enc_b + NT);
    p.off_rel_w.assign(d.off_rel_w, d.off_rel_w + (size_t)L * NR); p.off_rel_b.assign(d.off_rel_b, d.off_rel_b + (size_t)L * NR);
    p.off_root_w.assign(d.off_root_w, d.off_root_w + (size_t)L * NR);
    std::vector<bool> has_in(NT, false);
    for (int r = 0; r < NR; ++r) {
        const int s = p.rel_src[r], t = p.rel_dst[r];
        if (s < 0 || s >= NT || t < 0 || t >= NT) return fail(p, "relation type index out of range");
        if (p.rel_edge_off[r + 1] < p.rel_edge_off[r]) return fail(p, "rel_edge_off must be non-decreasing");
        has_in[t] = true;
        std::vector<int> deg(d.type_nodes[t], 0);
        for (int e = p.rel_edge_off[r]; e < p.rel_edge_off[r + 1]; ++e) {
            const int j = p.edges[2 * e], i = p.edges[2 * e + 1];
            if (j < 0 || j >= d.type_nodes[s] || i < 0 || i >= d.type_nodes[t]) return fail(p, "edge endpoint out of range");
            deg[i]++;
        }
        if (p.rel_mean[r]) for (int i = 0; i < d.type_nodes[t]; ++i)
            if (deg[i] > 1) return fail(p, "mean aggregation with in-degree > 1 is not supported by this build "
                                           "(all reference topologies have degree 1 on mean relations)");
    }
    for (int t = 0; t < NT; ++t)
        if (!has_in[t]) return fail(p, "every node type must be the destination of at least one relation "
                                       "(HeteroConv drops types without incoming relations)");
    p.sign_off.assign(NT, 0); p.enc_nkc.assign(NT, 0);
    for (int t = 0; t < NT; ++t) {
        const int F = d.type_width[t], n = d.type_nodes[t];
        const int nkc = (F + H - 1) / H; p.enc_nkc[t] = nkc;
        p.sign_off[t] = (int)p.signs.size();
        p.signs.resize(p.signs.size() + (size_t)n * nkc * H, 0);
        if (d.in_mask[t]) {
            for (int i = 0; i < n; ++i) for (int k = 0; k < F; ++k) {
                const float m = d.in_mask[t][(size_t)i * F + k];
                if (m != 1.0f && m != -1.0f) return fail(p, "symmetry masks must be +1 or -1");
                p.signs[p.sign_off[t] + (size_t)i * nkc * H + k] = m < 0 ? 1 : 0;
            }
        }
    }
    const int n_out = d.type_nodes[d.out_type];
    p.out_mask_f.assign((size_t)n_out * d.out_channels, 1.0f);
    if (d.out_mask) for (size_t i = 0; i < p.out_mask_f.size(); ++i) {
        if (d.out_mask[i] != 1.0f && d.out_mask[i] != -1.0f) return fail(p, "output mask must be +1 or -1");
        p.out_mask_f[i] = d.out_mask[i];
    }

    { const char* e = std::getenv("MSHGNN_PRUNE"); p.prune_nodes = !(e && std::atoi(e) == 0); }
    auto widen = [&](bool (&v)[64]) {
        for (int t = 0; t < NT; ++t) {
            if (p.prune_nodes && !(has_mlp && t == d.mlp_type)) continue;
            bool any = false;
            for (int i = 0; i < d.type_nodes[t]; ++i) any = any || v[p.type_base[t] + i];
            if (any) for (int i = 0; i < d.type_nodes[t]; ++i) v[p.type_base[t] + i] = true;
        }
    };
    auto inputs_of = [&](const bool (&out)[64], bool (&in)[64]) {
        for (int n = 0; n < p.NN; ++n) in[n] = out[n];
        for (int r = 0; r < NR; ++r)
            for (int e = p.rel_edge_off[r]; e < p.rel_edge_off[r + 1]; ++e)
                if (out[p.type_base[p.rel_dst[r]] + p.edges[2 * e + 1]]) in[p.type_base[p.rel_src[r]] + p.edges[2 * e]] = true;
        if (!p.prune_nodes)
            for (int r = 0; r < NR; ++r) {
                bool dl = false;
                for (int i = 0; i < d.type_nodes[p.rel_dst[r]]; ++i) dl = dl || out[p.type_base[p.rel_dst[r]] + i];
                if (dl) for (int j = 0; j < d.type_nodes[p.rel_src[r]]; ++j) in[p.type_base[p.rel_src[r]] + j] = true;
            }
    };
    for (int n = 0; n < p.NN; ++n) p.live_n[L - 1][n] = (p.node_type[n] == d.out_type);
    for (int l = L - 1; l >= 0; --l) {
        widen(p.live_n[l]);
        inputs_of(p.live_n[l], p.need_n[l]);
        if (l == 0) widen(p.need_n[0]);
        if (l > 0) for (int n = 0; n < p.NN; ++n) p.live_n[l - 1][n] = p.need_n[l][n];
    }
    for (int l = 1; l < L; ++l) for (int n = 0; n < p.NN; ++n) p.need_n[l][n] = p.live_n[l - 1][n];
    p.enc_live_nodes = 0;
    for (int n = 0; n < p.NN; ++n) p.enc_live_nodes += p.need_n[0][n] ? 1 : 0;
    for (int l = 0; l < L; ++l)
        for (int t = 0; t < NT; ++t) {
            p.live[l][t] = p.need_dx[l][t] = false;
            for (int i = 0; i < d.type_nodes[t]; ++i) { p.live[l][t] = p.live[l][t] || p.live_n[l][p.type_base[t] + i]; p.need_dx[l][t] = p.need_dx[l][t] || p.need_n[l][p.type_base[t] + i]; }
        }
    auto rel_live = [&](int l, int r) {
        for (int e = p.rel_edge_off[r]; e < p.rel_edge_off[r + 1]; ++e) if (p.live_n[l][p.type_base[p.rel_dst[r]] + p.edges[2 * e + 1]]) return true;
// ... 567 lines not shown
                    const int after = [&] { int c = add_cost(a, xb); put_in(a, xb); const int c2 = add_cost(b, xa); take_out(a, xb); return c + c2; }();
                    const int before = [&] { put_in(a, xa); const int c2 = add_cost(b, xb); take_out(a, xa); return before_a + c2; }();
                    (void)before_b;
                    put_in(a, xa); put_in(b, xb);
                    if (after - before < best_d) { best_d = after - before; best_b = b; }
                }
                if (best_b >= 0) { const int xb = where[best_b]; take_out(a, xa); take_out(best_b, xb); put_in(a, xb); put_in(best_b, xa); improved = true; }
            }
            if (!improved) break;
        }
        for (auto& q : xq) q.clear();
        for (int ln = 0; ln < p.n_lanes; ++ln) if (where[ln] >= 0) xq[where[ln]].push_back(ln);
    };
    auto queue_cost = [&](const std::vector<std::vector<int>>& xq) {
        long c = 0;
        for (auto& q : xq) { std::vector<char> seen(n_streams, 0); for (int ln : q) for (auto& s2 : lane_streams[ln]) if (!seen[s2.first]) { seen[s2.first] = 1; c += s2.second; } }
        return c; };
    auto build_queues = [&](const std::vector<bool>& take, std::vector<std::vector<int>>& xq) {
        xq.assign(8, {});
        for (auto& cs : cl_size) {
            int best = 0; for (int x = 1; x < 8; ++x) if (xq[x].size() < xq[best].size()) best = x;
            for (int ln = 0; ln < p.n_lanes; ++ln) if (take[ln] && lane_cluster[ln] == cs.second) xq[best].push_back(ln);
        }
        for (;;) {
            int lo = 0, hi = 0; for (int x = 1; x < 8; ++x) { if (xq[x].size() < xq[lo].size()) lo = x; if (xq[x].size() > xq[hi].size()) hi = x; }
            if (xq[hi].size() <= xq[lo].size() + 1) break;
            xq[lo].push_back(xq[hi].back()); xq[hi].pop_back();
        }
        refine_queues(xq);
        {
            std::vector<std::vector<int>> gq(8);
            std::vector<int> todo; for (int ln = 0; ln < p.n_lanes; ++ln) if (take[ln]) todo.push_back(ln);
            const int n = (int)todo.size();
            std::vector<bool> used(p.n_lanes, false);
            int left = n;
            for (int x = 0; x < 8 && left > 0; ++x) {
                const int want = (left + (8 - x) - 1) / (8 - x);
                std::vector<int> cnt(n_streams, 0);
                for (int k = 0; k < want; ++k) {
                    int best = -1, best_add = 0, best_share = 0;
                    for (int ln : todo) {
                        if (used[ln]) continue;
                        int add = 0, share = 0;
                        for (auto& s2 : lane_streams[ln]) { if (cnt[s2.first]) share += s2.second; else add += s2.second; }
                        if (best < 0 || (k > 0 && (add < best_add || (add == best_add && share > best_share)))) { best = ln; best_add = add; best_share = share; }
                        if (k == 0) break;
                    }
                    used[best] = true; gq[x].push_back(best); --left;
                    for (auto& s2 : lane_streams[best]) ++cnt[s2.first];
                }
            }
            refine_queues(gq);
            if (queue_cost(gq) < queue_cost(xq)) xq = gq;
        }
        size_t m = 0; for (auto& q : xq) m = std::max(m, q.size());
        return m; };
    std::vector<std::vector<int>> xq;
    size_t qmax = build_queues(std::vector<bool>(p.n_lanes, true), xq);
    p.n_lanes_pad = (int)qmax * 8;
    p.n_wg_gradw = p.n_lanes * p.n_parts;
    p.tgt_off = (int)T.size(); p.n_targets = (int)tgts.size();
    for (size_t g = 0; g < tgts.size(); ++g) {
        T.push_back(tgt_lane_begin[g]); T.push_back(tgt_lane_end[g]); T.push_back(tgts[g].bias_flag);
        for (int k = 3; k < TGT_INTS; ++k) T.push_back(0);
    }
    p.lane_off = (int)T.size();
    for (auto& ln : lanes) for (int k = 0; k < LANE_INTS; ++k) T.push_back(ln[k]);
    p.lane_order_off = (int)T.size();
    for (int k = 0; k < (int)qmax; ++k) for (int x = 0; x < 8; ++x) T.push_back(k < (int)xq[x].size() ? xq[x][k] : -1);
    p.n_slabs = p.n_wg_gradw;
    int lane_split = p.n_lanes;
    std::vector<bool> tgt_is_enc(tgts.size(), false);
    for (int t = 0; t < NT; ++t) for (int g : tgt_enc[t]) { tgt_is_enc[g] = true; lane_split = std::min(lane_split, tgt_lane_begin[g]); }
    for (int ph = 0; ph < 2; ++ph) {
        std::vector<bool> take(p.n_lanes);
        for (int ln = 0; ln < p.n_lanes; ++ln) take[ln] = (ln >= lane_split) == (ph == 1);
        std::vector<std::vector<int>> q2;
        const size_t m = build_queues(take, q2);
        p.order_ph_off[ph] = (int)T.size(); p.npad_ph[ph] = (int)m * 8;
        for (int k = 0; k < (int)m; ++k) for (int x = 0; x < 8; ++x) T.push_back(k < (int)q2[x].size() ? q2[x][k] : -1);
    }

    struct FinRec { int64_t dst; int rows, cols, ld, target, kind; std::vector<int64_t> more; };
    std::vector<FinRec> fins;
    auto add_fin = [&](int64_t dst, int rows, int cols, int ld, int target, int kind) {
        if (target >= 0 && (kind == FIN_MATRIX || kind == FIN_BIAS))
            for (auto& f : fins)
                if (f.target == target && f.kind == kind && f.rows == rows && f.cols == cols && f.ld == ld) { f.more.push_back(dst); return; }
        fins.push_back({dst, rows, cols, ld, target, kind, {}}); };
    for (int t = 0; t < NT; ++t) {
        const int F = d.type_width[t];
        for (int kc = 0; kc < p.enc_nkc[t]; ++kc) {
            const int nc = std::min(H, F - kc * H);
            const int tg = tgt_enc[t].empty() ? -1 : tgt_enc[t][kc];
            add_fin(p.off_enc_w[t] + kc * H, H, nc, F, tg, tg < 0 ? FIN_ZERO : FIN_MATRIX);
        }
        const int tg0 = tgt_enc[t].empty() ? -1 : tgt_enc[t][0];
        add_fin(p.off_enc_b[t], 1, H, H, tg0, tg0 < 0 ? FIN_ZERO : FIN_BIAS);
    }
    for (int l = 0; l < L; ++l)
        for (int r = 0; r < NR; ++r) {
            const int tr = tgt_rel[l * NR + r], to = tgt_root[l * NT + p.rel_dst[r]];
            add_fin(p.off_rel_w[l * NR + r], H, H, H, tr, tr < 0 ? FIN_ZERO : FIN_MATRIX);
            add_fin(p.off_rel_b[l * NR + r], 1, H, H, to, to < 0 ? FIN_ZERO : FIN_BIAS);
            add_fin(p.off_root_w[l * NR + r], H, H, H, to, to < 0 ? FIN_ZERO : FIN_MATRIX);
        }
    if (has_mlp) {
        for (int k = 0; k < 2; ++k) {
            add_fin(d.off_mlp[2 * k], H, H, H, tgt_mlp[k], tgt_mlp[k] < 0 ? FIN_ZERO : FIN_MATRIX);
            add_fin(d.off_mlp[2 * k + 1], 1, H, H, tgt_mlp[k], tgt_mlp[k] < 0 ? FIN_ZERO : FIN_BIAS);
        }
    }
    add_fin(d.off_dec_w, d.out_channels, H, H, -2, FIN_DEC_W);
    add_fin(d.off_dec_b, 1, d.out_channels, d.out_channels, -2, FIN_DEC_B);
    {
        std::vector<std::pair<int64_t, int64_t>> spans;
        for (int t = 0; t < NT; ++t) { spans.push_back({p.off_enc_w[t], (int64_t)H * d.type_width[t]}); spans.push_back({p.off_enc_b[t], H}); }
        for (int i = 0; i < L * NR; ++i) { spans.push_back({p.off_rel_w[i], (int64_t)H * H}); spans.push_back({p.off_rel_b[i], H}); spans.push_back({p.off_root_w[i], (int64_t)H * H}); }
        if (has_mlp) for (int k = 0; k < 2; ++k) { spans.push_back({d.off_mlp[2 * k], (int64_t)H * H}); spans.push_back({d.off_mlp[2 * k + 1], H}); }
        spans.push_back({d.off_dec_w, (int64_t)d.out_channels * H}); spans.push_back({d.off_dec_b, d.out_channels});
        std::sort(spans.begin(), spans.end());
        int64_t pos = 0;
        for (auto& sp : spans) {
            if (sp.first > pos && sp.first - pos < 4096) add_fin(pos, 1, (int)(sp.first - pos), (int)(sp.first - pos), -1, FIN_ZERO);
            pos = std::max(pos, sp.first + sp.second);
        }
        if (d.n_flat > pos && d.n_flat - pos < 4096) add_fin(pos, 1, (int)(d.n_flat - pos), (int)(d.n_flat - pos), -1, FIN_ZERO);
    }
    {
        int64_t enc_end = 0, rest_begin = d.n_flat;
        for (int t = 0; t < NT; ++t) { enc_end = std::max(enc_end, p.off_enc_w[t] + (int64_t)H * d.type_width[t]); enc_end = std::max(enc_end, p.off_enc_b[t] + (int64_t)H); }
        for (int i = 0; i < L * NR; ++i) { rest_begin = std::min(rest_begin, std::min(p.off_rel_w[i], std::min(p.off_rel_b[i], p.off_root_w[i]))); }
        if (has_mlp) for (int k = 0; k < 4; ++k) rest_begin = std::min<int64_t>(rest_begin, d.off_mlp[k]);
        rest_begin = std::min<int64_t>(rest_begin, std::min(d.off_dec_w, d.off_dec_b));
        p.grad_split = (enc_end <= rest_begin && lane_split < p.n_lanes) ? rest_begin : -1;
        auto is_ph1 = [&](const FinRec& f) { return p.grad_split >= 0 && f.dst < p.grad_split; };
        std::stable_sort(fins.begin(), fins.end(), [&](const FinRec& x, const FinRec& y) { return is_ph1(x) < is_ph1(y); });
        p.fin_off = (int)T.size(); p.n_fin = (int)fins.size(); p.n_fin_ph0 = 0;
        std::vector<int32_t> extra;
        for (auto& f : fins) {
            if (!is_ph1(f)) ++p.n_fin_ph0;
            if (is_ph1(f) && f.target >= 0 && !tgt_is_enc[f.target]) p.grad_split = -1;
            for (int64_t m : f.more) if ((p.grad_split >= 0 && m < p.grad_split) != is_ph1(f)) p.grad_split = -1;
            T.push_back((int32_t)(f.dst & 0xffffffff)); T.push_back((int32_t)(f.dst >> 32)); T.push_back(f.rows); T.push_back(f.cols);
            T.push_back(f.ld); T.push_back(f.target); T.push_back(f.kind);
            T.push_back(f.more.empty() ? 0 : (int32_t)(fins.size() * FIN_INTS + extra.size()));
            if (!f.more.empty()) {
                extra.push_back((int32_t)f.more.size());
                for (int64_t m : f.more) { extra.push_back((int32_t)(m & 0xffffffff)); extra.push_back((int32_t)(m >> 32)); }
            }
        }
        T.insert(T.end(), extra.begin(), extra.end());
        if (p.grad_split < 0) p.n_fin_ph0 = p.n_fin;
    }

    p.info.rows_per_tile = p.rows; p.info.total_nodes = p.NN; p.info.lds_bytes = (int64_t)p.n_blk * p.blk_bytes;
    p.info.flops_fwd = alg_fwd; p.info.flops_bwd = alg_bwd; p.info.flops_exec_fwd = exec_fwd; p.info.flops_exec_bwd = exec_bwd;
    double bytes = 0, bytes_all = 0;
    for (int t = 0; t < NT; ++t) { bytes += (double)enc_n[t] * d.type_width[t] * (p.split ? 4 : p.esize); bytes_all += (double)d.type_nodes[t] * d.type_width[t] * (p.split ? 4 : p.esize); }
    p.info.bytes_in = bytes_all; p.info.bytes_in_live = bytes; p.info.n_gradw_workgroups = p.n_wg_gradw;
    p.info.n_launches_fwd = 3 + L; p.info.n_launches_bwd = 3 + L;
    p.info.grad_split = p.grad_split;
    p.info.kernel_sets = (p.fused ? 1 : 0) | (p.slab ? 2 : 0);

    {
        const double es = p.esize * p.planes, act = (double)p.enc_live_nodes * H * es;
        auto add = [&](const std::string& name, int bound, double fa, double fe, double by) {
            mshgnn_kernel_stat k{}; std::snprintf(k.name, sizeof(k.name), "%s", name.c_str());
            k.bound = bound; k.flops_per_window = fa; k.flops_exec_per_window = fe; k.bytes_per_window = by;
            p.kstats.push_back(k); return (int)p.kstats.size() - 1; };
        auto live_nodes = [&](int l) { int n = 0; for (int i = 0; i < p.NN; ++i) n += p.live_n[l][i] ? 1 : 0; return n; };
        auto need_nodes = [&](int l) { int n = 0; for (int i = 0; i < p.NN; ++i) n += p.need_n[l][i] ? 1 : 0; return n; };
        p.ks_prep = add("prep", MSHGNN_BOUND_HBM, 0, 0, 0);
        p.ks_enc = add("enc_fwd", d.dtype == MSHGNN_F32 ? MSHGNN_BOUND_MFMA : MSHGNN_BOUND_HBM, enc_alg, enc_exec, bytes + act);
        for (int l = 0; l < L; ++l) {
            const int idx = add("layer_fwd" + std::to_string(l), MSHGNN_BOUND_MFMA, lf_alg[l], lf_exec[l],
                                act + live_nodes(l) * (double)H * es + live_nodes(l) * 16.0);
            if (l == 0) p.ks_layer_fwd0 = idx;
        }
        p.ks_dec_fwd = add("dec_fwd", MSHGNN_BOUND_HBM, 2.0 * n_out * d.out_channels * H, 2.0 * n_out * d.out_channels * H, n_out * (double)H * es);
        p.ks_dec_bwd = add("dec_bwd", MSHGNN_BOUND_HBM, 4.0 * n_out * d.out_channels * H, 4.0 * n_out * d.out_channels * H, 2.0 * n_out * (double)H * es);
        for (int l = L - 1; l >= 0; --l) {
            const int idx = add("layer_bwd" + std::to_string(l), MSHGNN_BOUND_MFMA, lb_alg[l], lb_exec[l],
                                live_nodes(l) * (double)H * es * 2 + need_nodes(l) * (double)H * es + live_nodes(l) * 16.0);
            if (l == L - 1) p.ks_layer_bwd0 = idx;
        }
        p.ks_gradw = add("gradw", d.dtype == MSHGNN_F32 ? MSHGNN_BOUND_MFMA : MSHGNN_BOUND_HBM, gw_alg, gw_exec, bytes + (double)L * 2 * act + act);
        p.ks_fin = add("finalize", MSHGNN_BOUND_HBM, 0, 0, 0);
        if (p.fused) {
            double fa = 0, fe = 0, fb = act, ba = 0, be = 0, bb = act;
            for (int l = 0; l < L; ++l) {
                fa += lf_alg[l]; fe += lf_exec[l]; fb += live_nodes(l) * (double)H * es + live_nodes(l) * 16.0;
                ba += lb_alg[l]; be += lb_exec[l]; bb += need_nodes(l) * (double)H * es + live_nodes(l) * 16.0;
            }
            fa += 2.0 * n_out * d.out_channels * H; fe += 2.0 * n_out * d.out_channels * H;
            p.ks_stack_fwd = add("stack_fwd", MSHGNN_BOUND_MFMA, fa, fe, fb);
            p.ks_stack_bwd = add("stack_bwd", MSHGNN_BOUND_MFMA, ba, be, bb);
            p.ks_stack_step = add("stack_step", MSHGNN_BOUND_MFMA, fa + ba, fe + be, fb + bb);
        }
    }
    return true;
}

inline size_t align_up(size_t v, size_t a) { return (v + a - 1) / a * a; }

inline void layout_workspace(const HostPlan& p, int64_t B, int training, mshgnn_ws_layout* o) {
    std::memset(o, 0, sizeof(*o));
    size_t off = 0;
    const size_t act = (size_t)B * p.NN * H * p.esize * p.planes, mlp = (size_t)B * std::max(1, p.n_mlp) * H * p.esize * p.planes;
    auto take = [&](size_t bytes) { size_t r = off; off = align_up(off + bytes, 256); return r; };
    for (int l = 0; l <= p.L; ++l) o->x[l] = take(act);
    for (int l = 0; l < p.L; ++l) { o->mask[l] = take((size_t)((B + 15) / 16 * 16) * p.NN * 4 * 4); o->hb[l] = take(mlp); o->t1[l] = take(mlp); }
    if (training) {
        o->dd[0] = take((size_t)((B + 15) / 16 * 16) * p.NN * 4 * 4);
        for (int l = 0; l <= p.L; ++l) o->dx[l] = take(act);
        for (int l = 0; l < p.L; ++l) { o->dh[l] = take(act); o->du[l] = take(mlp); }
        o->slabs = take((size_t)p.n_slabs * SLAB_FLOATS * 4);
        o->dec_slabs = take((size_t)std::max<int64_t>(NWG_DEC, (B + TILE_ROWS - 1) / TILE_ROWS) * DEC_SLAB_FLOATS * 4);
    }
    o->wpack = take(p.packs.size() * (size_t)H * H * p.esize * p.planes);
    o->bias = take(p.biases.size() * (size_t)H * 4);
    o->loss = take(64);
    o->total = off;
}

}
```

Baseline: 45.46 million windows/s.

## Fuse gradient finalize into gradw kernel via tail workgroups and completion tickets

Adds extra tail workgroups to the bf16 gradw grid. They compute the loss sum and the decoder weight and bias reductions that k_finalize used to do after gradw. Per-target atomic ticket counters, zeroed in the prep kernel, let the last-arriving gradw block reduce that target's slabs in place. A size cap decides which targets qualify, and the trimmed k_finalize handles only the remaining ops. The aim is to overlap finalize work with the gradw tail and shrink the separate finalize kernel. The cost is extra fences and atomics, and with the default cap of zero no target takes the in-block path, so finalize still launches for all slab ops.

```diff
diff --git a/morphsym_hgnn_amd/csrc/mshgnn.hip b/morphsym_hgnn_amd/csrc/mshgnn.hip
--- a/morphsym_hgnn_amd/csrc/mshgnn.hip
+++ b/morphsym_hgnn_amd/csrc/mshgnn.hip
@@ -60,7 +60,7 @@
         }
     }
 }
-template <typename T> __global__ void k_prep(PrepArgs a) { prep_one<T>(a, blockIdx.x * blockDim.x + threadIdx.x, true); }
+template <typename T> __global__ void k_prep(PrepArgs a) { prep_zero_counters(a); prep_one<T>(a, blockIdx.x * blockDim.x + threadIdx.x, true); }
 
 
 __device__ __forceinline__ u32x4 splice8(u32x4 A, u32x4 B, int n0) {
@@ -1318,6 +1318,106 @@
     }
 }
 
+
+#ifndef FIN_LB
+#define FIN_LB 4
+#endif
+__device__ __forceinline__ void fin_loss_sum(const FinArgs& a, int lane) {
+    float l = 0.f;
+    for (int b = lane; b < a.n_dec; b += 64) l += a.dec_slabs[(size_t)b * DEC_SLAB_FLOATS + 8 * H + 8];
+#pragma unroll
+    for (int m = 32; m >= 1; m >>= 1) l += __shfl_xor(l, m, 64);
+    if (lane == 0) *a.loss = l * a.inv_n + (a.accumulate ? *a.loss : 0.f);
+}
+__device__ __forceinline__ void fin_dec_op(const FinArgs& a, const int* f, int wave, int nwaves) {
+    const int64_t dst = (int64_t)(unsigned)f[0] | ((int64_t)f[1] << 32);
+    const int rows = f[2], cols = f[3], ld = f[4];
+    const bool is_mat = f[6] == FIN_DEC_W;
+    const int lane = threadIdx.x & 63;
+    for (int e = wave; e < rows * cols; e += nwaves) {
+        const int r = e / cols, cidx = e % cols;
+        const int src = is_mat ? r * H + cidx : 8 * H + cidx;
+        float sum = 0.f;
+        for (int b0 = 0; b0 < a.n_dec; b0 += 512) {
+            float v[8];
+#pragma unroll
+            for (int u = 0; u < 8; ++u) { const int b = b0 + lane + 64 * u; v[u] = b < a.n_dec ? a.dec_slabs[(size_t)b * DEC_SLAB_FLOATS + src] : 0.f; }
+            sum += ((v[0] + v[1]) + (v[2] + v[3])) + ((v[4] + v[5]) + (v[6] + v[7]));
+        }
+#pragma unroll
+        for (int m = 32; m >= 1; m >>= 1) sum += __shfl_xor(sum, m, 64);
+        if (lane == 0) { float* gp = a.grad + dst + (int64_t)r * ld + cidx; *gp = a.accumulate ? *gp + sum : sum; }
+    }
+}
+template <int VEC> __device__ __forceinline__ void fin_slab_op(const FinArgs& a, const int* f, int r0, int r1) {
+    typedef float fvec4 __attribute__((ext_vector_type(4)));
+    using fvec = std::conditional_t<VEC == 1, float, fvec4>;
+    static_assert(VEC == 1 || VEC == 4, "one element or one 16-byte group per load");
+    const int64_t dst = (int64_t)(unsigned)f[0] | ((int64_t)f[1] << 32);
+    const int cols = f[3], ld = f[4], tg = f[5], kind = f[6];
+    const int* more = f[7] ? a.fin0 + f[7] : nullptr;
+    const int cv = cols / VEC, n = (r1 - r0) * cv;
+    const bool is_mat = kind == FIN_MATRIX;
+    for (int i = threadIdx.x; i < n; i += 256) {
+        const int r = r0 + i / cv, cidx = (i % cv) * VEC;
+        fvec s = 0.f;
+        if (kind == FIN_MATRIX || kind == FIN_BIAS) {
+            const int src = is_mat ? r * H + cidx : H * H + cidx;
+            const int l0 = a.targets[tg * TGT_INTS], nl = a.targets[tg * TGT_INTS + 1] - l0;
+            const float* sp = a.slabs + (size_t)l0 * SLAB_FLOATS + src;
+            const size_t pstride = (size_t)a.n_lanes * SLAB_FLOATS;
+            for (int j0 = 0; j0 < nl; j0 += FIN_LB)
+                for (int p0 = 0; p0 < a.n_parts; p0 += 4) {
+                    fvec v[FIN_LB][4];
+#pragma unroll
+                    for (int jj = 0; jj < FIN_LB; ++jj)
+#pragma unroll
+                        for (int pp = 0; pp < 4; ++pp) {
+                            v[jj][pp] = 0.f;
+                            if (j0 + jj < nl && p0 + pp < a.n_parts) v[jj][pp] = *reinterpret_cast<const fvec*>(sp + (size_t)(j0 + jj) * SLAB_FLOATS + (size_t)(p0 + pp) * pstride);
+                        }
+#pragma unroll
+                    for (int jj = 0; jj < FIN_LB; ++jj) s += (v[jj][0] + v[jj][1]) + (v[jj][2] + v[jj][3]);
+                }
+        }
+        float* gp = a.grad + dst + (int64_t)r * ld + cidx;
+#pragma unroll
+        for (int e = 0; e < VEC; ++e) {
+            float se; if constexpr (VEC == 1) se = s; else se = s[e];
+            if (a.accumulate) se += gp[e];
+            gp[e] = se;
+            if (more) {
+                const int nm = more[0];
+                for (int k = 0; k < nm; ++k) a.grad[((int64_t)(unsigned)more[1 + 2 * k] | ((int64_t)more[2 + 2 * k] << 32)) + (int64_t)r * ld + cidx + e] = se;
+            }
+        }
+    }
+}
+__device__ __forceinline__ void fin_slab_op_alone(const FinArgs& a, const int* f) {
+    if (f[3] % 4) fin_slab_op<1>(a, f, 0, f[2]);
+    else fin_slab_op<4>(a, f, 0, f[2]);
+}
+__device__ __forceinline__ void fin_tail(const GradwArgs& g, int w) {
+    const FinArgs& a = g.fin;
+    if (a.loss && w == 0 && threadIdx.x < 64) fin_loss_sum(a, threadIdx.x);
+    for (int k = 0; k < g.n_tail_ops; ++k) {
+        const int* f = a.fin0 + g.tail_ops[k] * FIN_INTS;
+        if (f[6] == FIN_DEC_W || f[6] == FIN_DEC_B) fin_dec_op(a, f, w * 4 + (threadIdx.x >> 6), g.n_tail_wg * 4);
+        else if (k % g.n_tail_wg == w) fin_slab_op_alone(a, f);
+    }
+}
+
+__global__ __launch_bounds__(256) void k_finalize(FinArgs a) {
+    const int* f = a.ops ? a.fin0 + a.ops[blockIdx.x] * FIN_INTS : a.fin + blockIdx.x * FIN_INTS;
+    const int rows = f[2], kind = f[6];
+    const int RPB = (rows + gridDim.y - 1) / gridDim.y;
+    const int r0 = blockIdx.y * RPB, r1 = min(rows, r0 + RPB);
+    if (a.loss && blockIdx.x == 0 && blockIdx.y == 0 && threadIdx.x < 64) fin_loss_sum(a, threadIdx.x);
+    if (!a.grad) return;
+    if (kind == FIN_DEC_W || kind == FIN_DEC_B) { fin_dec_op(a, f, blockIdx.y * 4 + (threadIdx.x >> 6), gridDim.y * 4); return; }
+    fin_slab_op<1>(a, f, r0, r1);
+}
+
 template <bool ALIGNED, bool SERIES = false> __global__ __launch_bounds__(256, GW_WPS) void k_gradw_bf16_lean(GradwArgs a) {
     static_assert(!SERIES || ALIGNED, "the series gather replaces the aligned raw loads");
     using T = __bf16;
@@ -1329,6 +1429,7 @@
     __shared__ unsigned long long sbase[GW_IPL][4];
     __shared__ unsigned long long sser[SERIES ? GW_IPL : 1][16][2];
     const int tid = threadIdx.x, lane = tid & 63, wv = __builtin_amdgcn_readfirstlane(tid >> 6);
+    if ((int)blockIdx.x >= a.n_pad * a.n_parts) { fin_tail(a, (int)blockIdx.x - a.n_pad * a.n_parts); return; }
     mlut[tid] = chunk_mask_bits<__bf16>(u32x4{0xffffffffu, 0xffffffffu, 0xffffffffu, 0xffffffffu}, (unsigned)tid);
     const int wr = wv >> 1, wc = wv & 1;
     const int ln = a.lane_order[blockIdx.x % a.n_pad], part = blockIdx.x / a.n_pad;
@@ -1517,75 +1618,26 @@
             slab[H * H + tid] = s2;
         }
     }
-}
-
-
-#ifndef FIN_LB
-#define FIN_LB 4
-#endif
-__global__ __launch_bounds__(256) void k_finalize(FinArgs a) {
-    const int* f = a.fin + blockIdx.x * FIN_INTS;
-    const int64_t dst = (int64_t)(unsigned)f[0] | ((int64_t)f[1] << 32);
-    const int rows = f[2], cols = f[3], ld = f[4], tg = f[5], kind = f[6];
-    const int* more = f[7] ? a.fin0 + f[7] : nullptr;
-    const int RPB = (rows + gridDim.y - 1) / gridDim.y;
-    const int r0 = blockIdx.y * RPB, r1 = min(rows, r0 + RPB);
-    const int n = (r1 - r0) * cols;
-    if (a.loss && blockIdx.x == 0 && blockIdx.y == 0 && threadIdx.x < 64) {
-        float l = 0.f;
-        for (int b = threadIdx.x; b < a.n_dec; b += 64) l += a.dec_slabs[(size_t)b * DEC_SLAB_FLOATS + 8 * H + 8];
-#pragma unroll
-        for (int m = 32; m >= 1; m >>= 1) l += __shfl_xor(l, m, 64);
-        if (threadIdx.x == 0) *a.loss = l * a.inv_n + (a.accumulate ? *a.loss : 0.f);
-    }
-    if (!a.grad) return;
-    const bool is_mat = (kind == FIN_MATRIX || kind == FIN_DEC_W);
-    if (kind == FIN_DEC_W || kind == FIN_DEC_B) {
-        const int lane = threadIdx.x & 63, wave = blockIdx.y * 4 + (threadIdx.x >> 6), nwaves = gridDim.y * 4;
-        for (int e = wave; e < rows * cols; e += nwaves) {
-            const int r = e / cols, cidx = e % cols;
-            const int src = is_mat ? r * H + cidx : 8 * H + cidx;
-            float sum = 0.f;
-            for (int b0 = 0; b0 < a.n_dec; b0 += 512) {
-                float v[8];
-#pragma unroll
-                for (int u = 0; u < 8; ++u) { const int b = b0 + lane + 64 * u; v[u] = b < a.n_dec ? a.dec_slabs[(size_t)b * DEC_SLAB_FLOATS + src] : 0.f; }
-                sum += ((v[0] + v[1]) + (v[2] + v[3])) + ((v[4] + v[5]) + (v[6] + v[7]));
-            }
-#pragma unroll
-            for (int m = 32; m >= 1; m >>= 1) sum += __shfl_xor(sum, m, 64);
-            if (lane == 0) { float* gp = a.grad + dst + (int64_t)r * ld + cidx; *gp = a.accumulate ? *gp + sum : sum; }
-        }
-        return;
-    }
-    if (n <= 0) return;
-    for (int i = threadIdx.x; i < n; i += 256) {
-        const int r = r0 + i / cols, cidx = i % cols;
-        float s = 0.f;
-        if (kind == FIN_MATRIX || kind == FIN_BIAS) {
-            const int src = is_mat ? r * H + cidx : H * H + cidx;
-            const int l0 = a.targets[tg * TGT_INTS], nl = a.targets[tg * TGT_INTS + 1] - l0;
-            const float* sp = a.slabs + (size_t)l0 * SLAB_FLOATS + src;
-            const size_t pstride = (size_t)a.n_lanes * SLAB_FLOATS;
-            for (int j0 = 0; j0 < nl; j0 += FIN_LB)
-                for (int p0 = 0; p0 < a.n_parts; p0 += 4) {
-                    float v[FIN_LB][4];
-#pragma unroll
-                    for (int jj = 0; jj < FIN_LB; ++jj)
-#pragma unroll
-                        for (int pp = 0; pp < 4; ++pp)
-                            v[jj][pp] = (j0 + jj < nl && p0 + pp < a.n_parts) ? sp[(size_t)(j0 + jj) * SLAB_FLOATS + (size_t)(p0 + pp) * pstride] : 0.f;
-#pragma unroll
-                    for (int jj = 0; jj < FIN_LB; ++jj) s += (v[jj][0] + v[jj][1]) + (v[jj][2] + v[jj][3]);
-                }
-        }
-        if (a.accumulate) s += a.grad[dst + (int64_t)r * ld + cidx];
-        a.grad[dst + (int64_t)r * ld + cidx] = s;
-        if (more) {
-            const int nm = more[0];
-            for (int k = 0; k < nm; ++k) a.grad[((int64_t)(unsigned)more[1 + 2 * k] | ((int64_t)more[2 + 2 * k] << 32)) + (int64_t)r * ld + cidx] = s;
-        }
-    }
+    if (!a.fin.grad) return;
+    const int* tt = a.fin.targets + lh[2] * TGT_INTS;
+    if (tt[1] - tt[0] > a.fuse_lanes || tt[3] == 0) return;
+    asm volatile("s_waitcnt vmcnt(0)" ::: "memory");
+    __syncthreads();
+    if (tid == 0) {
+        __builtin_amdgcn_fence(__ATOMIC_RELEASE, "agent");
+        asm volatile("s_waitcnt vmcnt(0)" ::: "memory");
+        const unsigned ticket = atomicAdd(a.fin_cnt + lh[2], 1u);
+        const bool last = ticket + 1u == (unsigned)((tt[1] - tt[0]) * a.n_parts);
+        if (last) {
+            __builtin_amdgcn_fence(__ATOMIC_ACQUIRE, "agent");
+            asm volatile("s_waitcnt vmcnt(0)" ::: "memory");
+            __hip_atomic_store(a.fin_cnt + lh[2], 0u, __ATOMIC_RELAXED, __HIP_MEMORY_SCOPE_AGENT);
+        }
+        sbase[0][3] = last ? 1ull : 0ull;
+    }
+    __syncthreads();
+    if (!sbase[0][3]) return;
+    for (int k = 0; k < tt[3]; ++k) fin_slab_op_alone(a.fin, a.fin.fin0 + tt[4 + k] * FIN_INTS);
 }
 
 static StackKernel slab_fwd_kernel(const HostPlan& hp) {
@@ -1735,6 +1787,8 @@
             { const char* esp = getenv("MSHGNN_SPEC"); p->use_spec = p->use_slab && !(esp && atoi(esp) == 0); }
             if (p->use_spec && (rc = set_spec_attrs(p, flds))) { mshgnn_plan_destroy(p); return rc; }
             { const char* et = getenv("MSHGNN_STEP_KERNEL"); p->use_step = !(et && atoi(et) == 0); }
+            { const char* ef = getenv("MSHGNN_FUSED_FINALIZE"); p->fuse_fin = hp.fin_fusable && !(ef && atoi(ef) == 0); }
+            { const char* ef = getenv("MSHGNN_FUSE_MAX_SLABS"); if (ef) p->fuse_max_slabs = atoi(ef); }
 
             { const char* eg = TUNE_ENV("MSHGNN_STAGGER"); p->stagger = eg ? atoi(eg) : 0; }
         }
@@ -1814,16 +1868,31 @@
     return MSHGNN_OK;
 }
 
-int run_finalize(const mshgnn_plan* p, const StepCall& c, const mshgnn_ws_layout& lay, int gw_parts) {
+FinArgs finalize_args(const mshgnn_plan* p, const StepCall& c, const mshgnn_ws_layout& lay, int gw_parts) {
     const HostPlan& hp = p->hp;
     const mshgnn_desc& d = hp.d;
-    char* ws = c.ws; float* gparams = c.grad_params; hipStream_t st = c.stream;
-    const int B = (int)c.batch, gw_phase = c.gw_phase;
-    float* loss = c.loss != LossKind::NONE ? c.loss_out : nullptr;
-    FinArgs a{p->d_tables + hp.fin_off, p->d_tables + hp.fin_off, p->d_tables + hp.tgt_off, reinterpret_cast<const float*>(ws + lay.slabs),
-              reinterpret_cast<const float*>(ws + lay.dec_slabs), gparams, hp.n_lanes, gw_parts, loss,
-              1.0f / (float)(c.total_windows() * d.type_nodes[d.out_type] * (c.loss == LossKind::CE ? 1 : d.out_channels)),
-              c.dec_done ? (int)((B + TILE_ROWS - 1) / TILE_ROWS) : NWG_DEC, c.accumulates()};
+    return FinArgs{p->d_tables + hp.fin_off, p->d_tables + hp.fin_off, p->d_tables + hp.tgt_off, reinterpret_cast<const float*>(c.ws + lay.slabs),
+                   reinterpret_cast<const float*>(c.ws + lay.dec_slabs), c.grad_params, hp.n_lanes, gw_parts, c.loss != LossKind::NONE ? c.loss_out : nullptr,
+                   1.0f / (float)(c.total_windows() * d.type_nodes[d.out_type] * (c.loss == LossKind::CE ? 1 : d.out_channels)),
+                   c.dec_done ? (int)((c.batch + TILE_ROWS - 1) / TILE_ROWS) : NWG_DEC, c.accumulates(), nullptr};
+}
+
+int run_finalize(const mshgnn_plan* p, const StepCall& c, const mshgnn_ws_layout& lay, int gw_parts, int fuse_lanes) {
+    const HostPlan& hp = p->hp;
+    float* gparams = c.grad_params; hipStream_t st = c.stream;
+    const int gw_phase = c.gw_phase;
+    FinArgs a = finalize_args(p, c, lay, gw_parts);
+    float* loss = a.loss;
+    if (fuse_lanes >= 0) {
+        int nrem = 0;
+        while (nrem < (int)hp.fin_rem_lanes.size() && hp.fin_rem_lanes[nrem] > fuse_lanes) ++nrem;
+        if (nrem == 0) return MSHGNN_OK;
+        a.loss = nullptr; a.ops = p->d_tables + hp.fin_rem_off;
+        ProfScope ps(p, hp.ks_fin, st);
+        hipLaunchKernelGGL(k_finalize, dim3(nrem, 64), dim3(256), 0, st, a);
+        HIPCHK(hipGetLastError());
+        return MSHGNN_OK;
+    }
     int f0 = 0, nf = hp.n_fin;
     if (gw_phase == 0) nf = hp.n_fin_ph0;
     if (gw_phase == 1) { f0 = hp.n_fin_ph0; nf = hp.n_fin - hp.n_fin_ph0; a.loss = nullptr; }
@@ -1851,6 +1920,7 @@
     const SeriesSrc* series = c.series; const WideSrc* wide = c.wide;
     const float* y_fused = c.y_fused(); const int32_t* labels_fused = c.labels_fused();
     PrepArgs pa{params, ws + lay.wpack, reinterpret_cast<float*>(ws + lay.bias), p->d_packs, p->d_biases, (int)hp.packs.size(), (int)hp.biases.size()};
+    if (sizeof(T) == 2 && training && p->fuse_fin) { pa.fin_cnt = reinterpret_cast<unsigned*>(ws + fin_counters_off(hp, lay)); pa.n_fin_cnt = hp.n_targets; }
     int enc_pack0 = (int)hp.packs.size();
     for (int t = 0; t < hp.NT; ++t) if (hp.pack_enc_base[t] >= 0) enc_pack0 = std::min(enc_pack0, hp.pack_enc_base[t]);
     static const bool embed_off = TUNE_ENV("MSHGNN_PREP_EMBED") && atoi(TUNE_ENV("MSHGNN_PREP_EMBED")) == 0;
@@ -2060,6 +2130,7 @@
         hipLaunchKernelGGL(k_layer_bwd<T>, dim3(tiles), dim3(LAYER_THREADS), hp.n_blk * Prec<T>::BLK, st, a);
     }
     const int gw_parts = gw_parts_for(hp.n_parts, hp.n_lanes, hp.gw_ipl, B, sizeof(T) == 4 ? GW_KW : GWB_KW, p->n_cu);
+    int fuse_lanes = -1;
     if (c.grad_params) {
         GradwArgs a{};
         a.ws = ws;
@@ -2078,22 +2149,29 @@
         a.signs = p->d_signs; a.slabs = reinterpret_cast<float*>(ws + lay.slabs); a.B = B; a.n_lanes = hp.n_lanes; a.n_parts = gw_parts;
         a.dbg = p->dbg_gw;
         a.stamps = stamp_ptr("MSHGNN_STAMPS_GW");
+        [[maybe_unused]] static const bool gw_general = TUNE_ENV("MSHGNN_GRADW") && std::string(TUNE_ENV("MSHGNN_GRADW")) == "general";
+        if (sizeof(T) == 2 && p->fuse_fin && gw_phase < 0 && c.chunk.total_windows == 0 && !gw_general && a.n_pad > 0) {
+            fuse_lanes = p->fuse_max_slabs / gw_parts;
+            a.fin = finalize_args(p, c, lay, gw_parts);
+            a.fin_cnt = reinterpret_cast<unsigned*>(ws + fin_counters_off(hp, lay));
+            a.tail_ops = p->d_tables + hp.fin_tail_off; a.n_tail_ops = hp.n_fin_tail; a.n_tail_wg = FIN_TAIL_WGS; a.fuse_lanes = fuse_lanes;
+        }
+        const unsigned gw_grid = (unsigned)(a.n_pad * gw_parts + a.n_tail_wg);
         ProfScope ps(p, hp.ks_gradw, st);
         auto launch_gradw = [&](const GradwArgs& ga, hipStream_t s_) {
-            [[maybe_unused]] static const bool gw_general = TUNE_ENV("MSHGNN_GRADW") && std::string(TUNE_ENV("MSHGNN_GRADW")) == "general";
             if (ga.n_pad <= 0) return;
             if constexpr (sizeof(T) == 4) hipLaunchKernelGGL(k_gradw_f32, dim3(ga.n_pad * gw_parts), dim3(256), 0, s_, ga);
 #ifdef MSHGNN_TUNING
             else if (gw_general && hp.gw_ipl == 1) hipLaunchKernelGGL(k_gradw_bf16<1>, dim3(ga.n_pad * gw_parts), dim3(256), 0, s_, ga);
             else if (gw_general && hp.gw_ipl == 2) hipLaunchKernelGGL(k_gradw_bf16<2>, dim3(ga.n_pad * gw_parts), dim3(256), 0, s_, ga);
 #endif
-            else if (series) hipLaunchKernelGGL((k_gradw_bf16_lean<true, true>), dim3(ga.n_pad * gw_parts), dim3(256), 0, s_, ga);
-            else if (ga.aligned) hipLaunchKernelGGL(k_gradw_bf16_lean<true>, dim3(ga.n_pad * gw_parts), dim3(256), 0, s_, ga);
-            else hipLaunchKernelGGL(k_gradw_bf16_lean<false>, dim3(ga.n_pad * gw_parts), dim3(256), 0, s_, ga);
+            else if (series) hipLaunchKernelGGL((k_gradw_bf16_lean<true, true>), dim3(gw_grid), dim3(256), 0, s_, ga);
+            else if (ga.aligned) hipLaunchKernelGGL(k_gradw_bf16_lean<true>, dim3(gw_grid), dim3(256), 0, s_, ga);
+            else hipLaunchKernelGGL(k_gradw_bf16_lean<false>, dim3(gw_grid), dim3(256), 0, s_, ga);
         };
         launch_gradw(a, st);
     }
-    return run_finalize(p, c, lay, gw_parts);
+    return run_finalize(p, c, lay, gw_parts, fuse_lanes);
 }
 
 static int run_forward(const mshgnn_plan* p, StepCall& c) {
diff --git a/morphsym_hgnn_amd/csrc/mshgnn_device.hpp b/morphsym_hgnn_amd/csrc/mshgnn_device.hpp
--- a/morphsym_hgnn_amd/csrc/mshgnn_device.hpp
+++ b/morphsym_hgnn_amd/csrc/mshgnn_device.hpp
@@ -305,7 +305,11 @@
 struct PrepArgs {
     const float* params; void* wpack; float* bias; const PackDesc* packs; const BiasDesc* biases; int n_packs; int n_biases;
     int pack0 = 0, pack_n = -1;
-};
+    unsigned* fin_cnt = nullptr; int n_fin_cnt = 0;
+};
+__device__ __forceinline__ void prep_zero_counters(const PrepArgs& a) {
+    if (a.fin_cnt && blockIdx.x == 0) for (int i = threadIdx.x; i < a.n_fin_cnt; i += blockDim.x) a.fin_cnt[i] = 0u;
+}
 
 struct EncArgs {
     const void* x[MSHGNN_MAX_TYPES]; int64_t pitch[MSHGNN_MAX_TYPES]; int vb[MSHGNN_MAX_TYPES];
@@ -674,6 +678,7 @@
 template <typename T, bool SPLIT_OUT> __global__ __launch_bounds__(256) void k_prep_tiled(PrepArgs a) {
     __shared__ __attribute__((aligned(16))) float tile[PREP_TILE_FLOATS];
     const int tid = threadIdx.x;
+    prep_zero_counters(a);
     if ((int)blockIdx.x < 2 * a.n_packs) { prep_pack_half<T, SPLIT_OUT>(a, blockIdx.x >> 1, blockIdx.x & 1, tile, tid); return; }
     const int b = ((int)blockIdx.x - 2 * a.n_packs) * 256 + tid;
     if (b < a.n_biases * H) {
@@ -1150,6 +1155,10 @@
 };
 
 
+struct FinArgs { const int* fin; const int* fin0; const int* targets; const float* slabs; const float* dec_slabs; float* grad; int n_lanes, n_parts; float* loss; float inv_n;
+                 int n_dec; int accumulate;
+                 const int* ops; };
+
 struct GradwArgs {
     const char* ws; size_t buf_off[BUF_COUNT];
     const void* x[MSHGNN_MAX_TYPES]; int64_t pitch[MSHGNN_MAX_TYPES]; int nodes[MSHGNN_MAX_TYPES]; int vb[MSHGNN_MAX_TYPES];
@@ -1158,6 +1167,7 @@
     int dbg;
     long long* stamps;
     SeriesSrc ser;
+    FinArgs fin; unsigned* fin_cnt; const int* tail_ops; int n_tail_ops, n_tail_wg, fuse_lanes;
 };
 
 constexpr int GWB_KW = 64;
@@ -1176,8 +1186,9 @@
 }
 
 
-struct FinArgs { const int* fin; const int* fin0; const int* targets; const float* slabs; const float* dec_slabs; float* grad; int n_lanes, n_parts; float* loss; float inv_n;
-                 int n_dec; int accumulate; };
+
+constexpr int FUSE_MAX_SLABS = 0;
+constexpr int FIN_TAIL_WGS = 32;
 
 struct mshgnn_gen_state;
 struct ProfRec { int slot; hipEvent_t a, b; };
@@ -1196,6 +1207,8 @@
     int stash_nt_force = -1;
     int64_t step_chunk = 32768;
     bool use_step = false;
+    bool fuse_fin = false;
+    int fuse_max_slabs = FUSE_MAX_SLABS;
     bool use_spec = true;
     const char* spec_name = "";
     std::string spec_name_buf;
@@ -1291,7 +1304,7 @@
 #define SPEC_CAT2(a, b) a##b
 #define SPEC_CAT(a, b) SPEC_CAT2(a, b)
 
-int run_finalize(const mshgnn_plan* p, const StepCall& c, const mshgnn_ws_layout& lay, int gw_parts);
+int run_finalize(const mshgnn_plan* p, const StepCall& c, const mshgnn_ws_layout& lay, int gw_parts, int fuse_lanes = -1);
 int x3_set_attrs(mshgnn_plan* p);
 int x3_attach_program(mshgnn_plan* p, void* selector);
 int x3_forward(const mshgnn_plan* p, StepCall& c);
diff --git a/morphsym_hgnn_amd/csrc/mshgnn_plan.hpp b/morphsym_hgnn_amd/csrc/mshgnn_plan.hpp
--- a/morphsym_hgnn_amd/csrc/mshgnn_plan.hpp
+++ b/morphsym_hgnn_amd/csrc/mshgnn_plan.hpp
@@ -134,6 +134,8 @@
     int order_ph_off[2]{}, npad_ph[2]{}, n_fin_ph0 = 0;
     int64_t grad_split = -1;
     int fin_off = 0, n_fin = 0;
+    int fin_tail_off = 0, n_fin_tail = 0, fin_rem_off = 0; bool fin_fusable = false;
+    std::vector<int> fin_rem_lanes;
     int enc_tile_mb = 4;
     int n_slabs = 0;
     std::vector<float> out_mask_f;
@@ -1007,6 +1009,24 @@
         }
         T.insert(T.end(), extra.begin(), extra.end());
         if (p.grad_split < 0) p.n_fin_ph0 = p.n_fin;
+        p.fin_fusable = true;
+        std::vector<int> tail, rem;
+        for (int i = 0; i < p.n_fin; ++i) {
+            const FinRec& f = fins[i];
+            if (f.kind != FIN_MATRIX && f.kind != FIN_BIAS) { tail.push_back(i); continue; }
+            int32_t* tt = &T[p.tgt_off + (size_t)f.target * TGT_INTS];
+            if (tt[3] >= TGT_INTS - 4) { p.fin_fusable = false; break; }
+            tt[4 + tt[3]++] = i;
+            rem.push_back(i);
+        }
+        auto lanes_of = [&](int i) { return tgt_lane_end[fins[i].target] - tgt_lane_begin[fins[i].target]; };
+        std::stable_sort(rem.begin(), rem.end(), [&](int x, int y) { return lanes_of(x) > lanes_of(y); });
+        p.fin_tail_off = (int)T.size(); p.n_fin_tail = (int)tail.size();
+        T.insert(T.end(), tail.begin(), tail.end());
+        p.fin_rem_off = (int)T.size();
+        T.insert(T.end(), rem.begin(), rem.end());
+        p.fin_rem_lanes.clear();
+        for (int i : rem) p.fin_rem_lanes.push_back(lanes_of(i));
     }
 
     p.info.rows_per_tile = p.rows; p.info.total_nodes = p.NN; p.info.lds_bytes = (int64_t)p.n_blk * p.blk_bytes;
@@ -1059,6 +1079,7 @@
 
 inline size_t align_up(size_t v, size_t a) { return (v + a - 1) / a * a; }
 
+inline size_t fin_counters_off(const HostPlan& p, const mshgnn_ws_layout& o) { return o.slabs + (size_t)p.n_slabs * SLAB_FLOATS * 4; }
 inline void layout_workspace(const HostPlan& p, int64_t B, int training, mshgnn_ws_layout* o) {
     std::memset(o, 0, sizeof(*o));
     size_t off = 0;
@@ -1070,7 +1091,7 @@
         o->dd[0] = take((size_t)((B + 15) / 16 * 16) * p.NN * 4 * 4);
         for (int l = 0; l <= p.L; ++l) o->dx[l] = take(act);
         for (int l = 0; l < p.L; ++l) { o->dh[l] = take(act); o->du[l] = take(mlp); }
-        o->slabs = take((size_t)p.n_slabs * SLAB_FLOATS * 4);
+        o->slabs = take((size_t)p.n_slabs * SLAB_FLOATS * 4 + (size_t)p.n_targets * 4);
         o->dec_slabs = take((size_t)std::max<int64_t>(NWG_DEC, (B + TILE_ROWS - 1) / TILE_ROWS) * DEC_SLAB_FLOATS * 4);
     }
     o->wpack = take(p.packs.size() * (size_t)H * H * p.esize * p.planes);
```

After: 43.49 million windows/s. -4.3%, worse.
